# bluecher31/mlff-preconditioner

Hardware: AMD Instinct MI355X
Metric: CG iters/sec + GB/s on N×N fp64 kernel mat-vec; iters-to-1e-6 vs CPU ref (higher is better)
Workload: dtype f64

## Files before the change

### include/mlffpcg.h

```cpp
#ifndef MLFFPCG_H
#define MLFFPCG_H

#include <stdint.h>

#ifdef __cplusplus
extern "C" {
#endif

#define MLFF_OK 0
#define MLFF_ERR_ARG (-1)
#define MLFF_ERR_HIP (-2)
#define MLFF_ERR_NOT_PSD (-3)
#define MLFF_ERR_LINALG (-4)
#define MLFF_ERR_STATE (-5)
#define MLFF_ERR_COMM (-6)
#define MLFF_ERR_NOMEM (-7)

#define MLFF_PRECON_NONE 0
#define MLFF_PRECON_PIVCHOL 1
#define MLFF_PRECON_NYSTROM 2
#define MLFF_PRECON_NYSTROM_SB 3
#define MLFF_PRECON_LOWRANK 4
#define MLFF_PRECON_EIG 5

#define MLFF_STORAGE_DENSE 0
#define MLFF_STORAGE_SYMTILE 1
#define MLFF_STORAGE_AUTO 2
#define MLFF_STORAGE_MATFREE 3

#define MLFF_PCG_RUNNING 0
#define MLFF_PCG_CONVERGED 2
#define MLFF_PCG_MAXITER 3

typedef struct mlff_ctx mlff_ctx;

int mlff_version(void);
const char *mlff_build_hash(void);
int mlff_device_count(int *n_out);
int mlff_comm_unique_id(unsigned char id_out[128]);
int mlff_comm_selftest(int device, int64_t count, double *max_err_out);

int mlff_ctx_create(int device, int rank, int world, const unsigned char *comm_id,
                    int64_t n_global, mlff_ctx **ctx_out);
int mlff_ctx_destroy(mlff_ctx *ctx);
const char *mlff_last_error(mlff_ctx *ctx);
int mlff_shard_range(mlff_ctx *ctx, int64_t *row0_out, int64_t *nrows_out);
int mlff_comm_abort(mlff_ctx *ctx);
int mlff_matrix_ld(mlff_ctx *ctx, int64_t *ld_out);
int mlff_synchronize(mlff_ctx *ctx);
int mlff_stream(mlff_ctx *ctx, void **stream_out);

int mlff_set_matrix_host(mlff_ctx *ctx, const double *K_local, int64_t ld_host);
int mlff_get_matrix_rows(mlff_ctx *ctx, int64_t r0, int64_t nr, double *out, int64_t ld_out);
int mlff_gen_rbf(mlff_ctx *ctx, const double *X, int d, double length_scale, double jitter);
int mlff_assemble_sgdml(mlff_ctx *ctx, const double *R_desc, const double *R_d_desc,
                        int64_t M, int n_atoms, const int32_t *perms, int n_perms, double sig);
int mlff_sgdml_operator(mlff_ctx *ctx, const double *R_desc, const double *R_d_desc, int64_t M,
                        int n_atoms, const int32_t *perms, int n_perms, double sig);

int mlff_set_energy_constraints(mlff_ctx *ctx, int use_E_cstr);

int mlff_spectrum(mlff_ctx *ctx, int preconditioned, double *eig_out);

int mlff_test_gemm(mlff_ctx *ctx, int ta, int tb, int64_t M, int64_t N, int64_t K, double alpha,
                   const double *A, int64_t lda, const double *B, int64_t ldb, double beta,
                   double *C, int64_t ldc, int splits);
int mlff_dense_cho_solve(mlff_ctx *ctx, double sigma_K, double shift, const double *b,
                         double *x_out, double *seconds_out);
int mlff_test_potrf(mlff_ctx *ctx, const double *A, int64_t n, int variant, double *L_out,
                    double *seconds_out);
int mlff_test_gram(mlff_ctx *ctx, const double *W, int64_t k, int64_t ncols, int mode,
                   double *G_out);
int mlff_cho_factor_stable(mlff_ctx *ctx, const double *M, int64_t m, double *L_out,
                           double *lo_eig_out);
int mlff_sym_min_eig(mlff_ctx *ctx, const double *M, int64_t m, double *lo_eig_out,
                     double *d_out, double *e_out);
int mlff_sgdml_descriptors(const double *R, int64_t M, int n_atoms, double *R_desc_out,
                           double *R_d_desc_out);

int mlff_sgdml_energies(mlff_ctx *ctx, const double *alphas, double *E_out, int64_t *i0_out,
                        int64_t *ni_out);

int mlff_predict_set_model(mlff_ctx *ctx, const double *R_desc, const double *R_d_desc_alpha,
                           int64_t M, int n_atoms, const int32_t *perms, int n_perms, double sig,
                           double std, double c);
int mlff_predict(mlff_ctx *ctx, const double *R, int64_t Q, double *E_out, double *F_out);
int mlff_predict_info(mlff_ctx *ctx, int *form_out, int64_t *slab_out, double *flops_per_query_out,
                      double *bytes_per_query_out);

int mlff_set_operator(mlff_ctx *ctx, double sigma_K, double lam);
int mlff_matvec(mlff_ctx *ctx, const double *v_global, double *y_local);
int mlff_set_storage(mlff_ctx *ctx, int mode);
int mlff_storage_info(mlff_ctx *ctx, int *mode_out, double *bytes_per_matvec_out);
#define MLFF_MF_FORM_PAIR 0
#define MLFF_MF_FORM_REC 1
#define MLFF_MF_FORM_PTILE 2
int mlff_operator_form(mlff_ctx *ctx, int *form_out);
int mlff_get_diag(mlff_ctx *ctx, double *diag_local);

int mlff_precon_none(mlff_ctx *ctx);
int mlff_precon_pivchol(mlff_ctx *ctx, int64_t k, int build_woodbury, int64_t *index_columns_out,
                        double *seconds_out);
int mlff_pivchol_times(mlff_ctx *ctx, double *col_seconds_out, int64_t k,
                       double *woodbury_seconds_out);
int mlff_precon_nystrom(mlff_ctx *ctx, const int64_t *idx, int64_t k, int variant, double *seconds_out);
int mlff_precon_lowrank(mlff_ctx *ctx, const double *Lt_local, int64_t k);
int mlff_precon_eig(mlff_ctx *ctx, int64_t k, int mask_mode, int64_t dim_i, int build_woodbury,
                    double *evals_out, double *rowlev_out);
int mlff_precon_info(mlff_ctx *ctx, int *kind_out, int64_t *k_out);
int mlff_eig_info(mlff_ctx *ctx, int *converged_out, double *rel_resid_out);
int mlff_precon_apply(mlff_ctx *ctx, const double *r_local, double *z_local);
int mlff_precon_apply_traffic(mlff_ctx *ctx, int *one_pass_out, double *bytes_out);
int mlff_precon_get_panel(mlff_ctx *ctx, double *T_local, int64_t ld_out);

int mlff_lev_scores(mlff_ctx *ctx, const int64_t *idx, int64_t k, double lam, double *scores_out);

int mlff_pcg_start(mlff_ctx *ctx, const double *b_local, const double *x0_local, double tol,
                   int64_t maxiter, int *early_exit_out);
int mlff_pcg_run(mlff_ctx *ctx, int64_t n_iter, int64_t chunk, int *status_out);
int mlff_pcg_result(mlff_ctx *ctx, int64_t *iters_out, int *status_out, double *resid_out,
                    int *info_out);
int mlff_pcg_get_x(mlff_ctx *ctx, double *x_local);
int mlff_pcg_get_trace(mlff_ctx *ctx, double *trace_out, int64_t n);

int mlff_timing_enable(mlff_ctx *ctx, int on);
int mlff_timing_read(mlff_ctx *ctx, double *gemv_ms, int64_t *gemv_count, double *iter_ms,
                     int64_t *iter_count);
int mlff_timing_read_precon(mlff_ctx *ctx, double *ms, int64_t *count);
int mlff_timing_read_comm(mlff_ctx *ctx, double *ms, int64_t *count);
int mlff_timing_reset(mlff_ctx *ctx);
int mlff_device_memory(mlff_ctx *ctx, int64_t *free_out, int64_t *total_out);

#ifdef __cplusplus
}
#endif
#endif
```

### mlff-preconditioner_amd/csrc/api.hip

```cpp
#include "common.h"

#include <cstdlib>

#include <algorithm>
#include <chrono>
#include <cmath>
#include <condition_variable>
#include <cstring>
#include <limits>
#include <map>
#include <mutex>

using namespace mlff;

static thread_local std::string g_last_error;

namespace mlff {

int set_error(mlff_ctx *ctx, int code, const std::string &msg) {
  if (ctx != nullptr) ctx->err = msg;
  g_last_error = msg;
  return code;
}

// ... 1124 lines not shown
  if (hipDeviceSynchronize() != hipSuccess) return fail(set_error(nullptr, MLFF_ERR_HIP, "init sync failed"));
  *ctx_out = ctx;
  return MLFF_OK;
  MLFF_API_END(nullptr)
}

int mlff_ctx_destroy(mlff_ctx *ctx) {
  MLFF_API_BEGIN
  if (ctx == nullptr) return MLFF_OK;
  hipSetDevice(ctx->device);
  if (ctx->stream) hipStreamSynchronize(ctx->stream);
  for (void *p : {(void *)ctx->K, (void *)ctx->x, (void *)ctx->r, (void *)ctx->z, (void *)ctx->q,
                  (void *)ctx->b, (void *)ctx->p_full, (void *)ctx->xg, (void *)ctx->part,
                  (void *)ctx->st, (void *)ctx->trace, (void *)ctx->T, (void *)ctx->tpart_base,
                  (void *)ctx->perm, (void *)ctx->dwork, (void *)ctx->pivflag, (void *)ctx->prow, (void *)ctx->zpart, (void *)ctx->lr_zpart, (void *)ctx->lr_slots, (void *)ctx->lr_fault, (void *)ctx->gb})
    dev_free(p);
  for (const auto &c : ctx->scratch_chunks) dev_free(c.p);
  ctx->scratch_chunks.clear();
  sym_free(ctx->sym);
  mf_free(ctx->mf);
  pred_free(ctx->pred);
  rbf_free(ctx);
  if (ctx->h_st) hipHostFree(ctx->h_st);
  for (hipEvent_t e : ctx->timing.ev) hipEventDestroy(e);
  if (ctx->comm) ncclCommDestroy(ctx->comm);
  ctx->local.reset();
  if (ctx->stream) hipStreamDestroy(ctx->stream);
  delete ctx;
  return MLFF_OK;
  MLFF_API_END(ctx)
}

int mlff_comm_abort(mlff_ctx *ctx) {
  MLFF_API_BEGIN
  if (ctx == nullptr) return set_error(nullptr, MLFF_ERR_ARG, "null ctx");
  ctx->aborted = true;
  if (ctx->local) ctx->local->abort();
  if (ctx->comm != nullptr) {
    (void)hipSetDevice(ctx->device);
    ncclCommAbort(ctx->comm);
    ctx->comm = nullptr;
  }
  return MLFF_OK;
  MLFF_API_END(ctx)
}

int mlff_shard_range(mlff_ctx *ctx, int64_t *row0_out, int64_t *nrows_out) {
  MLFF_API_BEGIN
  MLFF_ENTER(ctx);
  if (row0_out) *row0_out = ctx->row0;
  if (nrows_out) *nrows_out = ctx->nrows;
  return MLFF_OK;
  MLFF_API_END(ctx)
}

int mlff_matrix_ld(mlff_ctx *ctx, int64_t *ld_out) {
  MLFF_API_BEGIN
  if (ctx == nullptr || ld_out == nullptr) return set_error(ctx, MLFF_ERR_ARG, "null pointer");
  *ld_out = ctx->ld;
  return MLFF_OK;
  MLFF_API_END(ctx)
}

int mlff_synchronize(mlff_ctx *ctx) {
  MLFF_API_BEGIN
  MLFF_ENTER(ctx);
  MLFF_HIP(ctx, hipStreamSynchronize(ctx->stream));
  return MLFF_OK;
  MLFF_API_END(ctx)
}

int mlff_stream(mlff_ctx *ctx, void **stream_out) {
  MLFF_API_BEGIN
  if (ctx == nullptr || stream_out == nullptr) return set_error(ctx, MLFF_ERR_ARG, "null pointer");
  *stream_out = (void *)ctx->stream;
  return MLFF_OK;
  MLFF_API_END(ctx)
}

int mlff_set_matrix_host(mlff_ctx *ctx, const double *K_local, int64_t ld_host) {
  MLFF_API_BEGIN
  MLFF_ENTER(ctx);
  if (K_local == nullptr && ctx->nrows > 0) return set_error(ctx, MLFF_ERR_ARG, "null K");
  if (ld_host < ctx->N) return set_error(ctx, MLFF_ERR_ARG, "ld_host < N");
  MLFF_TRY(ensure_matrix(ctx));
  MLFF_HIP(ctx, hipMemsetAsync(ctx->K, 0, sizeof(double) * ctx->blk * ctx->ld, ctx->stream));
  for (int r = 0; r < ctx->world && ctx->nrows > 0; ++r) {
    const int64_t g0 = (int64_t)r * ctx->rows_per;
    if (g0 >= ctx->N) break;
    const int64_t cnt = std::min<int64_t>(ctx->rows_per, ctx->N - g0);
    MLFF_HIP(ctx, hipMemcpy2DAsync(ctx->K + (int64_t)r * ctx->blk, sizeof(double) * ctx->ld,
                                   K_local + g0, sizeof(double) * ld_host, sizeof(double) * cnt,
                                   ctx->nrows, hipMemcpyHostToDevice, ctx->stream));
  }
  MLFF_HIP(ctx, hipStreamSynchronize(ctx->stream));
  ctx->has_matrix = true;
  ctx->K_symmetric = false;
  ctx->sym.ready = false;
  mf_free(ctx->mf);
  rbf_free(ctx);
  return MLFF_OK;
  MLFF_API_END(ctx)
}

int mlff_get_matrix_rows(mlff_ctx *ctx, int64_t r0, int64_t nr, double *out, int64_t ld_out) {
  MLFF_API_BEGIN
  MLFF_ENTER(ctx);
  if (out == nullptr) return set_error(ctx, MLFF_ERR_ARG, "null pointer");
  if (!ctx->has_matrix && !ctx->rbf.ready) return set_error(ctx, MLFF_ERR_STATE, "no kernel matrix set");
  if (r0 < 0 || nr < 0 || r0 + nr > ctx->nrows || ld_out < ctx->N)
    return set_error(ctx, MLFF_ERR_ARG, "row range / ld_out");
  ScratchScope scope(ctx);
  const int64_t chunk = ctx->has_matrix ? nr : std::max<int64_t>(1, std::min<int64_t>(nr, (int64_t)(256e6 / (8.0 * ctx->ld))));
  double *tmp = nullptr;
  if (!ctx->has_matrix) MLFF_TRY(scratch_alloc(ctx, &tmp, (size_t)chunk * ctx->ld));
  for (int64_t c0 = 0; c0 < nr; c0 += chunk) {
    const int64_t cn = std::min<int64_t>(chunk, nr - c0);
    const double *src = ctx->K + (r0 + c0) * ctx->ld;
    if (!ctx->has_matrix) {
      launch_gen_rbf(tmp, ctx->ld, cn, ctx->row0 + r0 + c0, ctx->rows_per, ctx->blk, ctx->N,
                     ctx->rbf.Xs, ctx->rbf.d, ctx->rbf.jitter, ctx->stream);
      MLFF_HIP(ctx, hipGetLastError());
      src = tmp;
    }
    for (int r = 0; r < ctx->world; ++r) {
      const int64_t g0 = (int64_t)r * ctx->rows_per;
      if (g0 >= ctx->N) break;
      const int64_t cnt = std::min<int64_t>(ctx->rows_per, ctx->N - g0);
      MLFF_HIP(ctx, hipMemcpy2DAsync(out + c0 * ld_out + g0, sizeof(double) * ld_out,
                                     src + (int64_t)r * ctx->blk, sizeof(double) * ctx->ld,
                                     sizeof(double) * cnt, cn, hipMemcpyDeviceToHost, ctx->stream));
    }
    MLFF_HIP(ctx, hipStreamSynchronize(ctx->stream));
  }
  return MLFF_OK;
  MLFF_API_END(ctx)
}

int mlff_gen_rbf(mlff_ctx *ctx, const double *X, int d, double length_scale, double jitter) {
  MLFF_API_BEGIN
  MLFF_ENTER(ctx);
  if (X == nullptr || d < 1 || d > 8 || !(length_scale > 0.0))
    return set_error(ctx, MLFF_ERR_ARG, "gen_rbf: need X, 1 <= d <= 8, length_scale > 0");
  std::vector<double> Xs((size_t)ctx->N * d);
  for (size_t i = 0; i < Xs.size(); ++i) Xs[i] = X[i] / length_scale;
  sym_free(ctx->sym);
  mf_free(ctx->mf);
  rbf_free(ctx);
  if (ctx->K != nullptr) {
    (void)hipFree(ctx->K);
    ctx->K = nullptr;
  }
  ctx->has_matrix = false;
  MLFF_HIP(ctx, hipMalloc(&ctx->rbf.Xs, sizeof(double) * Xs.size()));
  MLFF_HIP(ctx, hipMemcpy(ctx->rbf.Xs, Xs.data(), sizeof(double) * Xs.size(), hipMemcpyHostToDevice));
  ctx->rbf.d = d;
  ctx->rbf.jitter = jitter;
  ctx->rbf.ready = true;
  ctx->K_symmetric = true;
  return MLFF_OK;
  MLFF_API_END(ctx)
}

int mlff_assemble_sgdml(mlff_ctx *ctx, const double *R_desc, const double *R_d_desc, int64_t M,
                        int n_atoms, const int32_t *perms, int n_perms, double sig) {
  MLFF_API_BEGIN
  MLFF_ENTER(ctx);
  if (R_desc == nullptr || R_d_desc == nullptr || perms == nullptr || !(sig > 0.0))
    return set_error(ctx, MLFF_ERR_ARG, "assemble_sgdml: null input or sig <= 0");
  rbf_free(ctx);
  MLFF_TRY(ensure_matrix(ctx));
  MLFF_TRY(assemble_sgdml(ctx, R_desc, R_d_desc, M, n_atoms, perms, n_perms, sig));
  MLFF_TRY(mf_setup(ctx, R_desc, R_d_desc, M, n_atoms, perms, n_perms, sig));
  ctx->has_matrix = true;
  ctx->K_symmetric = true;
  ctx->sym.ready = false;
  return MLFF_OK;
  MLFF_API_END(ctx)
}

int mlff_sgdml_operator(mlff_ctx *ctx, const double *R_desc, const double *R_d_desc, int64_t M,
                        int n_atoms, const int32_t *perms, int n_perms, double sig) {
  MLFF_API_BEGIN
  MLFF_ENTER(ctx);
  if (R_desc == nullptr || R_d_desc == nullptr || perms == nullptr || !(sig > 0.0))
    return set_error(ctx, MLFF_ERR_ARG, "sgdml_operator: null input or sig <= 0");
  rbf_free(ctx);
  MLFF_TRY(mf_setup(ctx, R_desc, R_d_desc, M, n_atoms, perms, n_perms, sig));
  ctx->use_mf = false;
  ctx->has_matrix = false;
  ctx->sym.ready = false;
  return MLFF_OK;
  MLFF_API_END(ctx)
}

int mlff_test_gemm(mlff_ctx *ctx, int ta, int tb, int64_t M, int64_t N, int64_t K, double alpha,
                   const double *A, int64_t lda, const double *B, int64_t ldb, double beta,
                   double *C, int64_t ldc, int splits) {
  MLFF_API_BEGIN
  MLFF_ENTER(ctx);
  if (A == nullptr || B == nullptr || C == nullptr || M < 0 || N < 0 || K < 0 || splits < 1 ||
      lda < (ta ? M : K) || ldb < (tb ? K : N) || ldc < N)
    return set_error(ctx, MLFF_ERR_ARG, "test_gemm: bad arguments");
  return test_gemm(ctx, ta, tb, M, N, K, alpha, A, lda, B, ldb, beta, C, ldc, splits);
  MLFF_API_END(ctx)
}

int mlff_test_potrf(mlff_ctx *ctx, const double *A, int64_t n, int variant, double *L_out,
                    double *seconds_out) {
  MLFF_API_BEGIN
  MLFF_ENTER(ctx);
  if (A == nullptr || L_out == nullptr || n < 1 || variant < 0 || variant > 1)
    return set_error(ctx, MLFF_ERR_ARG, "test_potrf: bad arguments");
  return test_potrf(ctx, A, n, variant, L_out, seconds_out);
  MLFF_API_END(ctx)
}

int mlff_dense_cho_solve(mlff_ctx *ctx, double sigma_K, double shift, const double *b,
                         double *x_out, double *seconds_out) {
  MLFF_API_BEGIN
  MLFF_ENTER(ctx);
  if (b == nullptr || x_out == nullptr) return set_error(ctx, MLFF_ERR_ARG, "null pointer");
  if (ctx->world > 1)
    return set_error(ctx, MLFF_ERR_ARG, "dense_cho_solve: the closed-form solve runs on one rank");
  if (!ctx->has_matrix)
    return set_error(ctx, MLFF_ERR_STATE,
                     "dense_cho_solve: no dense kernel matrix (mlff_set_matrix_host / "
                     "mlff_assemble_sgdml); a matrix-free operator alone cannot be factored");
  return dense_cho_solve(ctx, sigma_K, shift, b, x_out, seconds_out);
  MLFF_API_END(ctx)
}

int mlff_test_gram(mlff_ctx *ctx, const double *W, int64_t k, int64_t ncols, int mode,
                   double *G_out) {
  MLFF_API_BEGIN
  MLFF_ENTER(ctx);
  if (W == nullptr || G_out == nullptr || k < 1 || ncols < 1 || mode < 0 || mode > 2)
    return set_error(ctx, MLFF_ERR_ARG, "test_gram: bad arguments");
  ScratchScope scope(ctx);
  double *dW = nullptr, *dG = nullptr;
  MLFF_TRY(scratch_alloc(ctx, &dW, (size_t)(k * ncols)));
  MLFF_TRY(scratch_alloc(ctx, &dG, (size_t)(k * k)));
  MLFF_HIP(ctx, hipMemcpyAsync(dW, W, sizeof(double) * k * ncols, hipMemcpyHostToDevice, ctx->stream));
  if (mode == 0)
    MLFF_TRY(syrk_wide(ctx, dW, k, ncols, ncols, dG));
  else
    MLFF_TRY(gram_wide_dd(ctx, dW, k, ncols, ncols, dG, mode == 2));
  MLFF_HIP(ctx, hipMemcpyAsync(G_out, dG, sizeof(double) * k * k, hipMemcpyDeviceToHost, ctx->stream));
  MLFF_HIP(ctx, hipStreamSynchronize(ctx->stream));
  return MLFF_OK;
  MLFF_API_END(ctx)
}

int mlff_sym_min_eig(mlff_ctx *ctx, const double *M, int64_t m, double *lo_eig_out,
                     double *d_out, double *e_out) {
  MLFF_API_BEGIN
  MLFF_ENTER(ctx);
  if (M == nullptr || m < 1 || lo_eig_out == nullptr)
    return set_error(ctx, MLFF_ERR_ARG, "sym_min_eig: bad arguments");
  ScratchScope scope(ctx);
  double *dM = nullptr;
  MLFF_TRY(scratch_alloc(ctx, &dM, (size_t)(m * m)));
  MLFF_HIP(ctx, hipMemcpyAsync(dM, M, sizeof(double) * m * m, hipMemcpyHostToDevice, ctx->stream));
  return sym_min_eig(ctx, dM, m, lo_eig_out, d_out, e_out);
  MLFF_API_END(ctx)
}

int mlff_cho_factor_stable(mlff_ctx *ctx, const double *M, int64_t m, double *L_out,
                           double *lo_eig_out) {
  MLFF_API_BEGIN
  MLFF_ENTER(ctx);
  if (M == nullptr || m < 1 || L_out == nullptr)
    return set_error(ctx, MLFF_ERR_ARG, "cho_factor_stable: bad arguments");
  ScratchScope scope(ctx);
  double *dM = nullptr;
  MLFF_TRY(scratch_alloc(ctx, &dM, (size_t)(m * m)));
  MLFF_HIP(ctx, hipMemcpyAsync(dM, M, sizeof(double) * m * m, hipMemcpyHostToDevice, ctx->stream));
  MLFF_TRY(cho_factor_stable(ctx, dM, m, lo_eig_out));
  MLFF_HIP(ctx, hipMemcpyAsync(L_out, dM, sizeof(double) * m * m, hipMemcpyDeviceToHost, ctx->stream));
  MLFF_HIP(ctx, hipStreamSynchronize(ctx->stream));
  return MLFF_OK;
  MLFF_API_END(ctx)
}

int mlff_spectrum(mlff_ctx *ctx, int preconditioned, double *eig_out) {
  MLFF_API_BEGIN
  MLFF_ENTER(ctx);
  if (eig_out == nullptr) return set_error(ctx, MLFF_ERR_ARG, "null pointer");
  MLFF_TRY(require_operator(ctx));
  return spectrum(ctx, preconditioned != 0, eig_out);
  MLFF_API_END(ctx)
}

int mlff_set_energy_constraints(mlff_ctx *ctx, int use_E_cstr) {
  MLFF_API_BEGIN
  MLFF_ENTER(ctx);
  if (use_E_cstr && ctx->world > 1)
    return set_error(ctx, MLFF_ERR_ARG, "use_E_cstr: energy constraints run on one rank");
  ctx->use_E_cstr = use_E_cstr != 0;
  return MLFF_OK;
  MLFF_API_END(ctx)
}

int mlff_sgdml_descriptors(const double *R, int64_t M, int n_atoms, double *R_desc_out,
                           double *R_d_desc_out) {
  MLFF_API_BEGIN
  if (R == nullptr || R_desc_out == nullptr || R_d_desc_out == nullptr || M < 1 || n_atoms < 2)
    return set_error(nullptr, MLFF_ERR_ARG, "sgdml_descriptors: bad arguments");
  const int rc = sgdml_descriptors(R, M, n_atoms, R_desc_out, R_d_desc_out);
  if (rc != MLFF_OK) return set_error(nullptr, rc, "sgdml_descriptors: HIP failure");
  return MLFF_OK;
  MLFF_API_END(nullptr)
}

int mlff_sgdml_energies(mlff_ctx *ctx, const double *alphas, double *E_out, int64_t *i0_out,
                        int64_t *ni_out) {
  MLFF_API_BEGIN
  MLFF_ENTER(ctx);
  if (alphas == nullptr || E_out == nullptr) return set_error(ctx, MLFF_ERR_ARG, "null pointer");
  if (!ctx->mf.ready) return set_error(ctx, MLFF_ERR_STATE, "no sGDML operator set");
  const MfData &mf = ctx->mf;
  const int64_t MP = mf.M * mf.n_perms;
  std::vector<double> pairs((size_t)std::max<int64_t>(mf.ni, 1) * MP);
  MLFF_TRY(mf_energies(ctx, alphas, pairs.data()));
  for (int64_t i = 0; i < mf.ni; ++i) {
    double e = 0.0;
    for (int64_t jp = 0; jp < MP; ++jp) e += pairs[(size_t)i * MP + jp];
    E_out[i] = e;
  }
  if (i0_out) *i0_out = mf.i0;
  if (ni_out) *ni_out = mf.ni;
  return MLFF_OK;
  MLFF_API_END(ctx)
}

int mlff_predict_set_model(mlff_ctx *ctx, const double *R_desc, const double *R_d_desc_alpha,
                           int64_t M, int n_atoms, const int32_t *perms, int n_perms, double sig,
                           double std, double c) {
  MLFF_API_BEGIN
  MLFF_ENTER(ctx);
  if (ctx->world > 1) return set_error(ctx, MLFF_ERR_ARG, "predict: runs on a one-rank context");
  if (R_desc == nullptr || R_d_desc_alpha == nullptr || perms == nullptr)
    return set_error(ctx, MLFF_ERR_ARG, "predict: null pointer");
  if (n_atoms < 2 || M < 1 || n_perms < 1 || n_perms > 1024)
    return set_error(ctx, MLFF_ERR_ARG, "predict: bad sizes");
  if (3 * (int64_t)n_atoms * M != ctx->N)
    return set_error(ctx, MLFF_ERR_ARG, "predict: N != 3 * n_atoms * M");
  if (!(sig > 0.0)) return set_error(ctx, MLFF_ERR_ARG, "predict: sig must be > 0");
  return pred_set_model(ctx, R_desc, R_d_desc_alpha, M, n_atoms, perms, n_perms, sig, std, c);
  MLFF_API_END(ctx)
}

int mlff_predict(mlff_ctx *ctx, const double *R, int64_t Q, double *E_out, double *F_out) {
  MLFF_API_BEGIN
  MLFF_ENTER(ctx);
  if (ctx->world > 1) return set_error(ctx, MLFF_ERR_ARG, "predict: runs on a one-rank context");
  if (!ctx->pred.ready) return set_error(ctx, MLFF_ERR_STATE, "predict: no model set (mlff_predict_set_model)");
  if (Q < 0) return set_error(ctx, MLFF_ERR_ARG, "predict: Q < 0");
  if (Q == 0) return MLFF_OK;
  if (R == nullptr || E_out == nullptr || F_out == nullptr)
    return set_error(ctx, MLFF_ERR_ARG, "predict: null pointer");
  return pred_run(ctx, R, Q, E_out, F_out);
  MLFF_API_END(ctx)
}

int mlff_predict_info(mlff_ctx *ctx, int *form_out, int64_t *slab_out, double *flops_per_query_out,
                      double *bytes_per_query_out) {
  MLFF_API_BEGIN
  MLFF_ENTER(ctx);
  if (!ctx->pred.ready) return set_error(ctx, MLFF_ERR_STATE, "predict: no model set (mlff_predict_set_model)");
  double fl = 0.0, by = 0.0;
  pred_work(ctx->pred, &fl, &by);
  if (form_out) *form_out = ctx->pred.form;
  if (slab_out) *slab_out = ctx->pred.slab;
  if (flops_per_query_out) *flops_per_query_out = fl;
  if (bytes_per_query_out) *bytes_per_query_out = by;
  return MLFF_OK;
  MLFF_API_END(ctx)
}

int mlff_set_operator(mlff_ctx *ctx, double sigma_K, double lam) {
  MLFF_API_BEGIN
  MLFF_ENTER(ctx);
  if (!(lam > 0.0)) return set_error(ctx, MLFF_ERR_ARG, "lam must be > 0");
  if (sigma_K != 1.0 && sigma_K != -1.0) return set_error(ctx, MLFF_ERR_ARG, "sigma_K must be +-1");
  ctx->sigma_K = sigma_K;
  ctx->lam = lam;
  ctx->has_operator = true;
  return MLFF_OK;
  MLFF_API_END(ctx)
}

int mlff_set_storage(mlff_ctx *ctx, int mode) {
  MLFF_API_BEGIN
  MLFF_ENTER(ctx);
  if (mode != MLFF_STORAGE_DENSE && mode != MLFF_STORAGE_SYMTILE && mode != MLFF_STORAGE_AUTO &&
      mode != MLFF_STORAGE_MATFREE)
    return set_error(ctx, MLFF_ERR_ARG, "bad storage mode");
  if (mode != ctx->storage) {
    ctx->storage = mode;
    ctx->use_sym = false;
    ctx->use_mf = false;
    if (mode == MLFF_STORAGE_DENSE || mode == MLFF_STORAGE_MATFREE) sym_free(ctx->sym);
  }
  return MLFF_OK;
  MLFF_API_END(ctx)
}

int mlff_operator_form(mlff_ctx *ctx, int *form_out) {
  MLFF_API_BEGIN
  MLFF_ENTER(ctx);
  if (form_out == nullptr) return set_error(ctx, MLFF_ERR_ARG, "null form_out");
  *form_out = ctx->mf.ready ? mf_form(ctx) : -1;
  return MLFF_OK;
  MLFF_API_END(ctx)
}

int mlff_storage_info(mlff_ctx *ctx, int *mode_out, double *bytes_per_matvec_out) {
  MLFF_API_BEGIN
  MLFF_ENTER(ctx);
  MLFF_TRY(require_operator(ctx));
  MLFF_TRY(resolve_storage(ctx));
  if (mode_out)
    *mode_out = ctx->use_mf ? MLFF_STORAGE_MATFREE
                            : (ctx->use_sym ? MLFF_STORAGE_SYMTILE : MLFF_STORAGE_DENSE);
  if (bytes_per_matvec_out) *bytes_per_matvec_out = operator_bytes(ctx);
  return MLFF_OK;
  MLFF_API_END(ctx)
}

int mlff_matvec(mlff_ctx *ctx, const double *v_global, double *y_local) {
  MLFF_API_BEGIN
  MLFF_ENTER(ctx);
  MLFF_TRY(require_operator(ctx));
  if (v_global == nullptr || (y_local == nullptr && ctx->nrows > 0)) return set_error(ctx, MLFF_ERR_ARG, "null vector");
  MLFF_TRY(resolve_storage(ctx));
  MLFF_TRY(scatter_global(ctx, v_global, ctx->xg));
  MLFF_TRY(launch_operator(ctx, ctx->xg, ctx->q, ctx->xg + (int64_t)ctx->rank * ctx->blk, nullptr));
  MLFF_HIP(ctx, hipGetLastError());
  if (ctx->nrows > 0)
    MLFF_HIP(ctx, hipMemcpyAsync(y_local, ctx->q, sizeof(double) * ctx->nrows, hipMemcpyDeviceToHost, ctx->stream));
  MLFF_HIP(ctx, hipStreamSynchronize(ctx->stream));
  return MLFF_OK;
  MLFF_API_END(ctx)
}

int mlff_get_diag(mlff_ctx *ctx, double *diag_local) {
  MLFF_API_BEGIN
  MLFF_ENTER(ctx);
  if (!ctx->has_matrix && !ctx->mf.ready && !ctx->rbf.ready)
    return set_error(ctx, MLFF_ERR_STATE, "no kernel matrix set");
  MLFF_TRY(operator_diag(ctx, ctx->dwork));
  if (ctx->nrows > 0)
    MLFF_HIP(ctx, hipMemcpyAsync(diag_local, ctx->dwork, sizeof(double) * ctx->nrows, hipMemcpyDeviceToHost, ctx->stream));
  MLFF_HIP(ctx, hipStreamSynchronize(ctx->stream));
  return MLFF_OK;
  MLFF_API_END(ctx)
}

int mlff_precon_none(mlff_ctx *ctx) {
  MLFF_API_BEGIN
  MLFF_ENTER(ctx);
  ctx->precon_kind = MLFF_PRECON_NONE;
  ctx->k = 0;
  return MLFF_OK;
  MLFF_API_END(ctx)
}

int mlff_precon_pivchol(mlff_ctx *ctx, int64_t k, int build_woodbury, int64_t *index_columns_out,
                        double *seconds_out) {
  MLFF_API_BEGIN
  MLFF_ENTER(ctx);
  MLFF_TRY(require_operator(ctx));
  if (k < 1 || k > ctx->N || k > 65536)
    return set_error(ctx, MLFF_ERR_ARG, "pivoted Cholesky rank k must satisfy 1 <= k <= min(N, 65536)");
  const auto t0 = std::chrono::steady_clock::now();
  ctx->precon_kind = MLFF_PRECON_NONE;
  MLFF_TRY(alloc_panel(ctx, k));
  if (ctx->prow) hipFree(ctx->prow);
  ctx->prow = nullptr;
  MLFF_HIP(ctx, hipMalloc(&ctx->prow, sizeof(double) * (k + 1)));
  MLFF_TRY(pivoted_cholesky(ctx, k, index_columns_out));
  ctx->k = k;
  ctx->piv_woodbury_s = 0.0;
  if (build_woodbury) {
    const auto tw = std::chrono::steady_clock::now();
    MLFF_TRY(woodbury_inplace(ctx, ctx->T, k));
    ctx->piv_woodbury_s = std::chrono::duration<double>(std::chrono::steady_clock::now() - tw).count();
    ctx->precon_kind = MLFF_PRECON_PIVCHOL;
    ctx->sigma_p = 1.0;
  }
  MLFF_HIP(ctx, hipStreamSynchronize(ctx->stream));
  if (seconds_out)
    *seconds_out = std::chrono::duration<double>(std::chrono::steady_clock::now() - t0).count();
  return MLFF_OK;
  MLFF_API_END(ctx)
}

int mlff_pivchol_times(mlff_ctx *ctx, double *col_seconds_out, int64_t k,
                       double *woodbury_seconds_out) {
  MLFF_API_BEGIN
  MLFF_ENTER(ctx);
  if (k < 0 || (k > 0 && col_seconds_out == nullptr)) return set_error(ctx, MLFF_ERR_ARG, "bad output");
  const int64_t n = std::min<int64_t>(k, (int64_t)ctx->piv_col_s.size());
  for (int64_t c = 0; c < n; ++c) col_seconds_out[c] = ctx->piv_col_s[c];
  for (int64_t c = n; c < k; ++c) col_seconds_out[c] = 0.0;
  if (woodbury_seconds_out) *woodbury_seconds_out = ctx->piv_woodbury_s;
  return MLFF_OK;
  MLFF_API_END(ctx)
}

int mlff_precon_nystrom(mlff_ctx *ctx, const int64_t *idx, int64_t k, int variant,
                        double *seconds_out) {
  MLFF_API_BEGIN
  MLFF_ENTER(ctx);
  MLFF_TRY(require_operator(ctx));
  if (variant != 0 && variant != 1) return set_error(ctx, MLFF_ERR_ARG, "variant must be 0 or 1");
  MLFF_TRY(check_idx(ctx, idx, k));
  const auto t0 = std::chrono::steady_clock::now();
  ctx->precon_kind = MLFF_PRECON_NONE;
  MLFF_TRY(alloc_panel(ctx, k));
  MLFF_TRY(nystrom_panel(ctx, idx, k, variant, ctx->lam, ctx->T));
  ctx->precon_kind = variant == 0 ? MLFF_PRECON_NYSTROM : MLFF_PRECON_NYSTROM_SB;
  ctx->k = k;
  ctx->sigma_p = -1.0;
  if (seconds_out)
    *seconds_out = std::chrono::duration<double>(std::chrono::steady_clock::now() - t0).count();
  return MLFF_OK;
  MLFF_API_END(ctx)
}

int mlff_precon_lowrank(mlff_ctx *ctx, const double *Lt_local, int64_t k) {
  MLFF_API_BEGIN
  MLFF_ENTER(ctx);
  MLFF_TRY(require_operator(ctx));
  if (k < 1 || k > ctx->N || (Lt_local == nullptr && ctx->nrows > 0))
    return set_error(ctx, MLFF_ERR_ARG, "lowrank: bad factor");
  ctx->precon_kind = MLFF_PRECON_NONE;
  MLFF_TRY(alloc_panel(ctx, k));
  if (ctx->nrows > 0)
    MLFF_HIP(ctx, hipMemcpy2DAsync(ctx->T, sizeof(double) * ctx->blk, Lt_local,
                                   sizeof(double) * ctx->nrows, sizeof(double) * ctx->nrows, k,
                                   hipMemcpyHostToDevice, ctx->stream));
  MLFF_TRY(woodbury_inplace(ctx, ctx->T, k));
  ctx->precon_kind = MLFF_PRECON_LOWRANK;
  ctx->k = k;
  ctx->sigma_p = 1.0;
  return MLFF_OK;
  MLFF_API_END(ctx)
}

int mlff_precon_eig(mlff_ctx *ctx, int64_t k, int mask_mode, int64_t dim_i, int build_woodbury,
                    double *evals_out, double *rowlev_out) {
  MLFF_API_BEGIN
  MLFF_ENTER(ctx);
  if (mask_mode < 0 || mask_mode > 2 || (mask_mode == 2 && (dim_i < 3 || dim_i % 3 != 0)))
    return set_error(ctx, MLFF_ERR_ARG, "eig: bad mask_mode / dim_i");
  if (mask_mode == 2) {
    MLFF_TRY(require_matrix(ctx));
  } else {
    MLFF_TRY(require_operator(ctx));
  }
  if (k < 1 || k > ctx->N) return set_error(ctx, MLFF_ERR_ARG, "eig: need 1 <= k <= N");
  ctx->precon_kind = MLFF_PRECON_NONE;
  MLFF_TRY(alloc_panel(ctx, k));
  MLFF_TRY(eig_lowrank(ctx, k, mask_mode, dim_i, ctx->T, evals_out, rowlev_out));
  if (build_woodbury) {
    MLFF_TRY(woodbury_inplace(ctx, ctx->T, k));
    ctx->precon_kind = MLFF_PRECON_EIG;
    ctx->k = k;
    ctx->sigma_p = 1.0;
  }
  return MLFF_OK;
  MLFF_API_END(ctx)
}

int mlff_eig_info(mlff_ctx *ctx, int *converged_out, double *rel_resid_out) {
  MLFF_API_BEGIN
  MLFF_ENTER(ctx);
  if (converged_out) *converged_out = ctx->eig_converged ? 1 : 0;
  if (rel_resid_out) *rel_resid_out = ctx->eig_rel_resid;
  return MLFF_OK;
  MLFF_API_END(ctx)
}

int mlff_precon_info(mlff_ctx *ctx, int *kind_out, int64_t *k_out) {
  MLFF_API_BEGIN
  MLFF_ENTER(ctx);
  if (kind_out) *kind_out = ctx->precon_kind;
  if (k_out) *k_out = ctx->k;
  return MLFF_OK;
  MLFF_API_END(ctx)
}

int mlff_precon_apply_traffic(mlff_ctx *ctx, int *one_pass_out, double *bytes_out) {
  MLFF_API_BEGIN
  MLFF_ENTER(ctx);
  const double N = (double)ctx->blk, n = (double)ctx->nrows, k = (double)ctx->k;
  const bool one = ctx->precon_kind != MLFF_PRECON_NONE && (ctx->lr_rows || ctx->lr_cluster);
  if (one_pass_out) *one_pass_out = one ? (ctx->lr_cluster ? 2 : 1) : 0;
  if (bytes_out) {
    if (ctx->precon_kind == MLFF_PRECON_NONE)
      *bytes_out = 0.0;
    else if (one)
      *bytes_out = 8.0 * k * N +
                   16.0 * (double)(ctx->lr_cluster ? ctx->lr_q : lr_rows_groups(ctx->k)) * N +
                   24.0 * n;
    else
      *bytes_out = 16.0 * k * N + 24.0 * n;
  }
  return MLFF_OK;
  MLFF_API_END(ctx)
}

int mlff_precon_apply(mlff_ctx *ctx, const double *r_local, double *z_local) {
  MLFF_API_BEGIN
  MLFF_ENTER(ctx);
  MLFF_TRY(require_operator(ctx));
  hipStream_t s = ctx->stream;
  ScratchScope scope(ctx);
  double *rd = nullptr, *zd = nullptr;
  MLFF_TRY(scratch_alloc(ctx, &rd, ctx->blk));
  MLFF_TRY(scratch_alloc(ctx, &zd, ctx->blk));
  MLFF_HIP(ctx, hipMemsetAsync(rd, 0, sizeof(double) * ctx->blk, s));
  if (ctx->nrows > 0)
    MLFF_HIP(ctx, hipMemcpyAsync(rd, r_local, sizeof(double) * ctx->nrows, hipMemcpyHostToDevice, s));
  if (ctx->precon_kind == MLFF_PRECON_NONE) {
    MLFF_HIP(ctx, hipMemcpyAsync(zd, rd, sizeof(double) * ctx->blk, hipMemcpyDeviceToDevice, s));
  } else {
    ctx->spec_t = false;
    if (ctx->exact_sums) {
      launch_dd_lowrank(ctx->T, ctx->blk, ctx->k, rd, zd, ctx->nrows, ctx->sigma_p, 1.0 / ctx->lam,
                        ctx->tpart, nullptr, s);
      MLFF_HIP(ctx, hipGetLastError());
      if (ctx->nrows > 0)
        MLFF_HIP(ctx, hipMemcpyAsync(z_local, zd, sizeof(double) * ctx->nrows, hipMemcpyDeviceToHost, s));
      MLFF_HIP(ctx, hipStreamSynchronize(s));
      return MLFF_OK;
    }
    if (ctx->lr_rows || ctx->lr_cluster) {
      if (ctx->lr_rows) {
        launch_lr_apply_rows(ctx->T, ctx->blk, ctx->k, rd, zd, ctx->nrows, ctx->sigma_p,
                             1.0 / ctx->lam, nullptr, nullptr, s, ctx->lr_zpart);
      } else {
        MLFF_HIP(ctx, hipMemsetAsync(ctx->lr_fault, 0, sizeof(int), s));
        launch_lr_apply_cluster(ctx->T, ctx->blk, ctx->k, ctx->lr_q, rd, zd, ctx->nrows,
                                ctx->sigma_p, 1.0 / ctx->lam, nullptr, nullptr, s, ctx->lr_zpart,
                                ctx->lr_slots, next_lr_epoch(ctx), ctx->lr_fault);
      }
      MLFF_HIP(ctx, hipGetLastError());
      if (ctx->lr_cluster) {
        int fault = 0;
        MLFF_HIP(ctx, hipMemcpyAsync(&fault, ctx->lr_fault, sizeof(int), hipMemcpyDeviceToHost, s));
        MLFF_HIP(ctx, hipStreamSynchronize(s));
        if (fault != 0) {
          ctx->lr_cluster = false;
          ctx->lr_fallbacks += 1;
          launch_gemv_split(ctx->T, ctx->blk, ctx->k, ctx->blk, ctx->tsplit, rd, ctx->tpart, nullptr, s);
          launch_precon_z(ctx->T, ctx->blk, ctx->k, ctx->tsplit, ctx->tpart, rd, zd, ctx->nrows,
                          ctx->sigma_p, 1.0 / ctx->lam, nullptr, nullptr, s, ctx->zpart, ctx->zsplit);
          MLFF_HIP(ctx, hipGetLastError());
        }
      }
      if (ctx->nrows > 0)
        MLFF_HIP(ctx, hipMemcpyAsync(z_local, zd, sizeof(double) * ctx->nrows, hipMemcpyDeviceToHost, s));
      MLFF_HIP(ctx, hipStreamSynchronize(s));
      return MLFF_OK;
    }
    launch_gemv_split(ctx->T, ctx->blk, ctx->k, ctx->blk, ctx->tsplit, rd, ctx->tpart, nullptr, s);
    MLFF_TRY(allreduce(ctx, ctx->tpart, (size_t)(ctx->k * ctx->tsplit)));
    launch_precon_z(ctx->T, ctx->blk, ctx->k, ctx->tsplit, ctx->tpart, rd, zd, ctx->nrows,
                    ctx->sigma_p, 1.0 / ctx->lam, nullptr, nullptr, s, ctx->zpart, ctx->zsplit);
  }
  MLFF_HIP(ctx, hipGetLastError());
  if (ctx->nrows > 0)
    MLFF_HIP(ctx, hipMemcpyAsync(z_local, zd, sizeof(double) * ctx->nrows, hipMemcpyDeviceToHost, s));
  MLFF_HIP(ctx, hipStreamSynchronize(s));
  return MLFF_OK;
  MLFF_API_END(ctx)
}

int mlff_precon_get_panel(mlff_ctx *ctx, double *T_local, int64_t ld_out) {
  MLFF_API_BEGIN
  MLFF_ENTER(ctx);
  if (ctx->T == nullptr || ctx->k < 1) return set_error(ctx, MLFF_ERR_STATE, "no low-rank panel");
  if (T_local == nullptr || ld_out < ctx->nrows) return set_error(ctx, MLFF_ERR_ARG, "bad output");
  if (ctx->nrows > 0)
    MLFF_HIP(ctx, hipMemcpy2DAsync(T_local, sizeof(double) * ld_out, ctx->T, sizeof(double) * ctx->blk,
                                   sizeof(double) * ctx->nrows, ctx->k, hipMemcpyDeviceToHost, ctx->stream));
  MLFF_HIP(ctx, hipStreamSynchronize(ctx->stream));
  return MLFF_OK;
  MLFF_API_END(ctx)
}

int mlff_lev_scores(mlff_ctx *ctx, const int64_t *idx, int64_t k, double lam, double *scores_out) {
  MLFF_API_BEGIN
  MLFF_ENTER(ctx);
  if (!ctx->has_matrix && !ctx->mf.ready && !ctx->rbf.ready)
    return set_error(ctx, MLFF_ERR_STATE, "no kernel matrix set");
  if (!(lam > 0.0) || scores_out == nullptr) return set_error(ctx, MLFF_ERR_ARG, "lev_scores: bad args");
  MLFF_TRY(check_idx(ctx, idx, k));
  hipStream_t s = ctx->stream;
  double *W = nullptr;
  MLFF_HIP(ctx, hipMalloc(&W, sizeof(double) * round_up(k, 8) * ctx->blk));
  MLFF_HIP(ctx, hipMemsetAsync(W, 0, sizeof(double) * round_up(k, 8) * ctx->blk, s));
  int rc = nystrom_panel(ctx, idx, k, 0, lam, W);
  if (rc != MLFF_OK) {
    hipFree(W);
    return rc;
  }
  MLFF_HIP(ctx, hipMemsetAsync(ctx->xg, 0, sizeof(double) * ctx->ld, s));
  launch_colsumsq(W, k, ctx->nrows, ctx->blk, ctx->xg + (int64_t)ctx->rank * ctx->blk, s);
  MLFF_TRY(allgather_blocks(ctx, ctx->xg));
  for (int r = 0; r < ctx->world; ++r) {
    const int64_t g0 = (int64_t)r * ctx->rows_per;
    if (g0 >= ctx->N) break;
    const int64_t cnt = std::min<int64_t>(ctx->rows_per, ctx->N - g0);
    MLFF_HIP(ctx, hipMemcpyAsync(scores_out + g0, ctx->xg + (int64_t)r * ctx->blk,
                                 sizeof(double) * cnt, hipMemcpyDeviceToHost, s));
  }
  MLFF_HIP(ctx, hipStreamSynchronize(s));
  hipFree(W);
  return MLFF_OK;
  MLFF_API_END(ctx)
}

int mlff_pcg_start(mlff_ctx *ctx, const double *b_local, const double *x0_local, double tol,
                   int64_t maxiter, int *early_exit_out) {
  MLFF_API_BEGIN
// ... 249 lines not shown
```

### mlff-preconditioner_amd/csrc/common.h

```cpp
#pragma once

#include <hip/hip_runtime.h>
#include <rccl/rccl.h>

#include <cstdint>
#include <memory>
#include <string>
#include <cstdlib>
#include <vector>

#include "../../include/mlffpcg.h"

namespace mlff {

constexpr int kWave = 64;
constexpr int kBlock = 256;
constexpr int kPad = 64;
constexpr int kMaxPart = 1024;
constexpr int kVecGrid = 512;
constexpr int kSymTile = 512;

__host__ __device__ inline int64_t round_up(int64_t a, int64_t b) { return (a + b - 1) / b * b; }

enum : int { ST_RUNNING = 0, ST_RECHECK = 1, ST_CONVERGED = 2, ST_MAXITER = 3, ST_FAULT = 4 };

struct DevState {
  double rho, rho1, alpha, pq, rr, resid, atol, pad0;
  long long iters;
  long long maxiter;
  int status;
  int linalg_err;
  int pivot_err;
  int pad1;
  long long m_pi;
  double sqrt_piv;
  double best_val;
  long long best_pos;
  double rho_new;
};

constexpr int kSymGenMaxD = 3;
constexpr double kSymStreamRate = 4990.0;
constexpr double kSymGenRate = 4990.0;
struct SymGen {
  const double *Xs = nullptr;
  int d = 0;
  double jitter = 0.0;
  int64_t N = 0, rows_per = 0, blk = 0;
  int n_s = 0;
  int qmode = 0;
  int roles = 0;
  int pool_first = 0;
};
enum SymRoles : int { kSymRolesCu = 0, kSymRolesIndex = 1, kSymRolesStream = 2, kSymRolesGen = 3 };
constexpr int kSymCuWords = 4096;

struct SymPack {
  bool ready = false;
  double *tiles = nullptr;
  int2 *list = nullptr;
  int64_t ntiles = 0;
  int64_t Np = 0;
  int64_t nb = 0;
  int64_t tiles_per_rank = 0;
  double *P = nullptr;
  int64_t nwhole = 0;
  int lsub = 2;
  int64_t pq_planes = 0;
  double *Pq = nullptr;
  unsigned char *split = nullptr;
  int *own = nullptr;
  int *plist = nullptr;
  int64_t pstride = 0;
  int pmax = 0;
  bool pq_ordered = false;
  int64_t t_split = 0;
  int64_t dyn = 0;
  unsigned long long *ticket = nullptr;
  bool gen = false;
  SymGen gsrc;
  double *yg = nullptr;
  double *yr = nullptr;
  int64_t ystride = 0;
};

constexpr int kSymOwnSplit = 1 << 24;
constexpr int kSymPlistSlotBits = 16;
constexpr int kSymPlistMaxSlots = (1 << kSymPlistSlotBits) - 1;
__host__ __device__ inline int sym_own_entry(int slot, bool split) {
  return slot | (split ? kSymOwnSplit : 0);
}
__host__ __device__ inline int sym_own_slot(int e) { return e & (kSymOwnSplit - 1); }
__host__ __device__ inline bool sym_own_split(int e) { return (e & kSymOwnSplit) != 0; }
__host__ __device__ inline int sym_plist_entry(int slot, int plane) {
  return slot | (plane << kSymPlistSlotBits);
}
__host__ __device__ inline int sym_plist_slot(int e) { return e & kSymPlistMaxSlots; }
__host__ __device__ inline int sym_plist_plane(int e) { return e >> kSymPlistSlotBits; }

struct MfData {
  bool ready = false;
  int64_t M = 0, D = 0;
  int n = 0, n_perms = 0;
  double sig = 0.0;
  int64_t i0 = 0, ni = 0;
  double *Rd = nullptr, *Rdd = nullptr;
  double *Rt = nullptr, *Zt = nullptr;
  int32_t *Pt = nullptr, *ps = nullptr, *pt = nullptr;
  bool ident = false;
  double *m5 = nullptr, *w = nullptr;
  double *c = nullptr, *F = nullptr;
  double *part = nullptr;
  double *ypart = nullptr;
  double *xc = nullptr;
  int nz = 1;
  int64_t dslice = 0;
  std::vector<int32_t> perms, piinv;
  double *uvk = nullptr;
  int32_t *pi_d = nullptr, *piinv_d = nullptr;
  bool rec = false;
  int rec_rg = 8;
  bool rec_wc16 = true;
  int rblk = 0;
  int64_t ldw = 0;
  double *wt = nullptr, *sv = nullptr, *rpart = nullptr;
  bool ptile = false;
  int pt_S = 1;
  double *ptpart = nullptr;
  bool E = false;
  int64_t nF = 0;
  double *kee = nullptr;
  double *eterm = nullptr;
};

struct PredData {
  bool ready = false;
  int64_t M = 0, D = 0, MP = 0;
  int n = 0, n_perms = 0;
  double sig = 0.0, std = 1.0, c = 0.0;
  int form = 0;
  int S = 1;
  int G = 1;
  int64_t slab = 0;
  int64_t PS = 0, ecol = 0;
  double *Rt = nullptr, *Zt = nullptr;
  double *Rq = nullptr;
  double *Rdq = nullptr, *Rddq = nullptr;
  double *part = nullptr;
  double *Fd = nullptr;
  double *EF = nullptr;
  double *h_in = nullptr, *h_out = nullptr;
};

struct RbfData {
  bool ready = false;
  double *Xs = nullptr;
  int d = 0;
  double jitter = 0.0;
};

__device__ __forceinline__ double rbf_sqdist_step(double s, double df, bool first) {
  return first ? __dmul_rn(df, df) : fma(df, df, s);
}
__device__ __forceinline__ double rbf_of_sqdist(double s) { return exp(-0.5 * s); }
__device__ __forceinline__ double rbf_value(const double (&xi)[8], const double *__restrict__ Xs,
                                            int64_t g, int d) {
  double s = 0.0;
#pragma unroll
  for (int t = 0; t < 8; ++t)
    if (t < d) s = rbf_sqdist_step(s, __dsub_rn(xi[t], Xs[g * d + t]), t == 0);
  return rbf_of_sqdist(s);
}

struct StopFold {
  const double *rr_part = nullptr;
  DevState *st = nullptr;
  double *trace = nullptr;
  long long it = 0;
};

struct XrFold {
  double *x = nullptr;
  double *r = nullptr;
  const double *p = nullptr;
  const double *q = nullptr;
  const double *pq_part = nullptr;
  double *rr_part = nullptr;
  DevState *st = nullptr;
};

inline unsigned timing_event_flags() {
  static const unsigned f = std::getenv("MLFF_EVENT_FENCE") ? hipEventDefault
                                                            : hipEventDisableSystemFence;
  return f;
}

struct Timing {
  bool on = false;
  int every = 1;
  bool sample = true;
  std::vector<hipEvent_t> ev;
  size_t used = 0;
  double gemv_ms = 0.0;
  int64_t gemv_count = 0;
  double pre_ms = 0.0;
  int64_t pre_count = 0;
  double iter_ms = 0.0;
  int64_t iter_count = 0;
  double comm_ms = 0.0;
  int64_t comm_count = 0;
};


__device__ __forceinline__ double fused_p(double pold, double z, double beta, bool first) {
  return first ? z : fma(beta, pold, z);
}

__device__ __forceinline__ double wave_sum(double v) {
#pragma unroll
  for (int o = 32; o > 0; o >>= 1) v += __shfl_down(v, o, 64);
  return v;
}

template <int CTRL>
__device__ __forceinline__ double dpp_f64(double v) {
  const int lo = __builtin_amdgcn_update_dpp(0, __double2loint(v), CTRL, 0xF, 0xF, false);
  const int hi = __builtin_amdgcn_update_dpp(0, __double2hiint(v), CTRL, 0xF, 0xF, false);
  return __hiloint2double(hi, lo);
}
template <int L>
__device__ __forceinline__ double group_sum(double v) {
  static_assert(L == 1 || L == 2 || L == 4 || L == 8, "DPP butterfly for L <= 8");
  if (L >= 2) v += dpp_f64<0xB1>(v);
  if (L >= 4) v += dpp_f64<0x4E>(v);
  if (L >= 8) v += dpp_f64<0x141>(v);
  return v;
}

__device__ __forceinline__ double block_sum256(double v, double *sh) {
  v = wave_sum(v);
  const int lane = threadIdx.x & 63, w = threadIdx.x >> 6;
  __syncthreads();
  if (lane == 0) sh[w] = v;
  __syncthreads();
  double t = 0.0;
  if (threadIdx.x == 0) t = (sh[0] + sh[1]) + (sh[2] + sh[3]);
  return t;
}

__device__ __forceinline__ void block_sum256_pair(double &a, double &b, double *sh) {
  a = wave_sum(a);
  b = wave_sum(b);
  const int lane = threadIdx.x & 63, w = threadIdx.x >> 6;
  __syncthreads();
  if (lane == 0) {
    sh[w] = a;
    sh[4 + w] = b;
  }
  __syncthreads();
  a = (sh[0] + sh[1]) + (sh[2] + sh[3]);
  b = (sh[4] + sh[5]) + (sh[6] + sh[7]);
}

__device__ __forceinline__ double reduce_parts_bcast(const double *__restrict__ part, int np,
                                                     double *sh) {
  double v = 0.0;
  for (int i = threadIdx.x; i < np; i += 256) v += part[i];
  v = block_sum256(v, sh);
  __syncthreads();
  if (threadIdx.x == 0) sh[4] = v;
  __syncthreads();
  return sh[4];
}

__device__ __forceinline__ bool stop_decide(const StopFold &f, double rr) {
  const double resid = sqrt(rr);
  DevState *st = f.st;
  int dec = ST_RUNNING;
  if (resid <= st->atol)
    dec = f.it > 1 ? ST_RECHECK : ST_CONVERGED;
  else if (f.it >= st->maxiter)
    dec = ST_MAXITER;
  if (blockIdx.x == 0 && blockIdx.y == 0 && threadIdx.x == 0) {
    st->rr = rr;
    st->resid = resid;
    st->iters = f.it;
    f.trace[f.it] = resid;
    if (dec != ST_RUNNING)
      st->status = dec;
    else
      st->rho1 = st->rho;
  }
  return dec == ST_RUNNING;
}

__device__ __forceinline__ double reduce_parts_bcast_wide(const double *__restrict__ part, int np,
                                                          double *sh) {
  double v = 0.0;
  if (threadIdx.x < 256)
    for (int i = threadIdx.x; i < np; i += 256) v += part[i];
  v = wave_sum(v);
  const int lane = threadIdx.x & 63, w = threadIdx.x >> 6;
  __syncthreads();
  if (lane == 0 && w < 4) sh[w] = v;
  __syncthreads();
  const double t = (sh[0] + sh[1]) + (sh[2] + sh[3]);
  __syncthreads();
  return t;
}

__device__ __forceinline__ double parts_thread_sum(const double *__restrict__ part, int np) {
  double v = 0.0;
  for (int i = threadIdx.x; i < np; i += 256) v += part[i];
  return v;
}
__device__ __forceinline__ double parts_bcast(double v, double *sh) {
  v = block_sum256(v, sh);
  __syncthreads();
  if (threadIdx.x == 0) sh[4] = v;
  __syncthreads();
  return sh[4];
}

}

namespace mlff {
struct LocalGroup;
}

struct mlff_ctx {
  int device = 0, rank = 0, world = 1;
  int64_t N = 0;
  int64_t rows_per = 0;
  int64_t row0 = 0, nrows = 0;
  int64_t blk = 0;
  int64_t ld = 0;
  hipStream_t stream = nullptr;
  ncclComm_t comm = nullptr;
  std::shared_ptr<mlff::LocalGroup> local;
  bool solo = false;

  double *K = nullptr;
  bool has_matrix = false;
  double sigma_K = 1.0, lam = 0.0;
  bool has_operator = false;
  bool K_symmetric = false;
  bool use_E_cstr = false;
  int storage = MLFF_STORAGE_AUTO;
  bool use_sym = false;
  bool use_mf = false;
  mlff::SymPack sym;
  mlff::MfData mf;
  mlff::RbfData rbf;
  mlff::PredData pred;

  double *x = nullptr, *r = nullptr, *z = nullptr, *q = nullptr, *b = nullptr;
  double *p_full = nullptr, *xg = nullptr;
  double *gb = nullptr;
  int64_t gstride = 0;
  double *part = nullptr;
  mlff::DevState *st = nullptr;
  mlff::DevState *h_st = nullptr;
  double *trace = nullptr;
  int64_t trace_cap = 0;
  bool pcg_active = false;
  int64_t pcg_done = 0;
  double tol = 0.0, bnorm = 0.0;

  int precon_kind = MLFF_PRECON_NONE;
  int64_t k = 0;
  double *T = nullptr;
  double sigma_p = 1.0;
  int tsplit = 1;
  int zsplit = 1;
  double *zpart = nullptr;
  bool lr_rows = false;
  bool fuse_p = true, fuse_xr = true;
  bool cho_fast = true;
  bool fuse_xr_ranks = false;
  bool pq_publish = false;
  bool piv_persist_off = false;
  int wb_refine = 0;
  int wb_gram_dd = 1;
  bool nys_refine = false;
  bool exact_sums = false;
  bool lr_cluster = false;
  int lr_q = 0;
  double *lr_zpart = nullptr;
  unsigned long long *lr_slots = nullptr;
  unsigned lr_epoch = 0;
  int *lr_fault = nullptr;
  int lr_fallbacks = 0;
  double last_lo_eig = 0.0;
  bool cho_flipped = false;
  bool eig_converged = true;
  double eig_rel_resid = 0.0;
  double *tpart = nullptr;
  double *tpart_base = nullptr;
  bool spec_t = false;

  int64_t *perm = nullptr;
  double *dwork = nullptr;
  int *pivflag = nullptr;
  double *prow = nullptr;
  std::vector<double> piv_col_s;
  double piv_woodbury_s = 0.0;

  mlff::Timing timing;
  std::string err;
  bool aborted = false;

  struct ScratchChunk {
    char *p;
    size_t size;
  };
  std::vector<ScratchChunk> scratch_chunks;
  size_t scratch_cur = 0, scratch_off = 0;
  int scratch_depth = 0;
};

namespace mlff {

int set_error(mlff_ctx *ctx, int code, const std::string &msg);
int hip_check(mlff_ctx *ctx, hipError_t e, const char *what);
int nccl_check(mlff_ctx *ctx, ncclResult_t e, const char *what);

#define MLFF_HIP(ctx, call)                                   \
  do {                                                        \
    hipError_t e__ = (call);                                  \
    if (e__ != hipSuccess) return mlff::hip_check(ctx, e__, #call); \
  } while (0)
#define MLFF_NCCL(ctx, call)                                  \
  do {                                                        \
    ncclResult_t e__ = (call);                                \
    if (e__ != ncclSuccess) return mlff::nccl_check(ctx, e__, #call); \
  } while (0)
#define MLFF_ENTER(ctx)                                                        \
  do {                                                                         \
    if ((ctx) == nullptr) return mlff::set_error(nullptr, MLFF_ERR_ARG, "null ctx"); \
    if ((ctx)->aborted)                                                        \
      return mlff::set_error((ctx), MLFF_ERR_COMM, "communicator aborted (mlff_comm_abort)"); \
    (void)hipSetDevice((ctx)->device);                                         \
  } while (0)
#define MLFF_TRY(x)             \
  do {                          \
    int rc__ = (x);             \
    if (rc__ != MLFF_OK) return rc__; \
  } while (0)

int api_exception(mlff_ctx *ctx, int code, const char *what);
#define MLFF_API_BEGIN try {
#define MLFF_API_END(ctx)                                                             \
  }                                                                                   \
  catch (const std::bad_alloc &) {                                                    \
    return mlff::api_exception((ctx), MLFF_ERR_NOMEM, "host allocation failed");      \
  }                                                                                   \
  catch (const std::exception &e__) {                                                 \
    return mlff::api_exception((ctx), MLFF_ERR_HIP, e__.what());                      \
  }                                                                                   \
  catch (...) {                                                                       \
    return mlff::api_exception((ctx), MLFF_ERR_HIP, "unknown C++ exception");         \
  }

struct ScratchScope {
  mlff_ctx *ctx;
  size_t chunk, off;
  explicit ScratchScope(mlff_ctx *c);
  ~ScratchScope();
  ScratchScope(const ScratchScope &) = delete;
  ScratchScope &operator=(const ScratchScope &) = delete;
};
int scratch_get(mlff_ctx *ctx, size_t bytes, void **out);
template <typename T>
int scratch_alloc(mlff_ctx *ctx, T **out, size_t count) {
  return scratch_get(ctx, sizeof(T) * (count > 0 ? count : 1), reinterpret_cast<void **>(out));
}

int comm_allreduce(mlff_ctx *ctx, double *buf, size_t n);
int comm_allgather(mlff_ctx *ctx, const double *send, double *recv, size_t count);

void launch_gemv_rows(const double *M, int64_t ld, int64_t rows, const double *v, double *y,
                      double sigma, double lam, const double *vloc, const int *status,
                      hipStream_t s);
void launch_gemv_split(const double *T, int64_t ldt, int64_t k, int64_t ncols, int splits,
                       const double *r, double *tpart, const int *status, hipStream_t s,
                       StopFold fold = StopFold{});
int choose_tsplit(int64_t k, int64_t ncols);
int choose_zsplit(int64_t k, int64_t ncols);
void launch_precon_z(const double *T, int64_t ldt, int64_t k, int splits, const double *tpart,
                     const double *r, double *z, int64_t n, double sigma_p, double lam_inv,
                     double *rho_part, const int *status, hipStream_t s, double *zpart,
                     int zsplit, StopFold fold = StopFold{});
bool lr_rows_fits(int64_t ldt);
int lr_rows_groups(int64_t k);
void launch_lr_apply_rows(const double *T, int64_t ldt, int64_t k, const double *r, double *z,
                          int64_t n, double sigma_p, double lam_inv, double *rho_part,
                          const int *status, hipStream_t s, double *zpart,
                          StopFold fold = StopFold{}, XrFold xf = XrFold{});
bool lr_cluster_fits(int64_t ldt);
int lr_cluster_members(int64_t ldt);
int lr_cluster_count(int64_t ldt, int device);
void launch_lr_apply_cluster(const double *T, int64_t ldt, int64_t k, int Q, const double *r,
                             double *z, int64_t n, double sigma_p, double lam_inv,
                             double *rho_part, const int *status, hipStream_t s, double *zpart,
                             unsigned long long *slots, unsigned epoch, int *fault,
                             StopFold fold = StopFold{});
void launch_colgemv_part(const double *W, int64_t ldw, int64_t k, const double *tsrc,
                         int tsplits, int64_t tstride, int ksplit, double *part,
                         const int *status, hipStream_t s, StopFold fold = StopFold{},
                         int64_t cached_rows = 0, const long long *tcol = nullptr,
                         const int *spec_hit = nullptr, int64_t spec_m0 = 0);
int gemm_splitk(mlff_ctx *ctx, bool ta, bool tb, int64_t M, int64_t N, int64_t K, const double *A,
                int64_t lda, const double *B, int64_t ldb, double *C, int64_t ldc);
int choose_ksplit(int64_t k, int64_t ncols);
int64_t panel_cached_rows(int64_t k, int64_t ldt);
void launch_dot_part(const double *a, const double *b, int64_t n, double *part,
                     const int *status, hipStream_t s, StopFold fold = StopFold{});
void launch_update_p(const double *z, double *p, int64_t n, const double *rho_part,
                     DevState *st, long long it, const int *status, hipStream_t s);
void launch_copy_dot(const double *r, int64_t n, double *dst, double *part, const int *status,
                     hipStream_t s, StopFold fold = StopFold{});
void launch_update_p_gathered(const double *gb, int64_t gstride, int64_t blk, int world,
                              double *p_full, DevState *st, long long it, const int *status,
                              hipStream_t s);
void launch_update_xr_shares(double *x, double *r, const double *p, const double *y,
                             const double *shares, int world, int64_t n, double sigma, double lam,
                             double *rr_part, DevState *st, const int *status, hipStream_t s);
bool xr_fold_fits(int64_t ncols, int splits, int64_t n);
void launch_dd_gemv_rows(const double *M, int64_t ld, int64_t rows, int64_t ncols, const double *v,
                         double *y, double sigma, double lam, const double *vloc, const int *status,
                         hipStream_t s);
void launch_dd_lowrank(const double *T, int64_t ldt, int64_t k, const double *r, double *z, int64_t n,
                       double sigma_p, double lam_inv, double *t, const int *status, hipStream_t s);
int gram_wide_dd(mlff_ctx *ctx, const double *W, int64_t k, int64_t ncols, int64_t ldw, double *G,
                 bool exact_products);
void launch_gemv_xr(const double *T, int64_t ldt, int64_t k, int64_t ncols, int splits,
                    const double *r, double *r_out, double *x, const double *p, const double *y,
                    const double *shares, int world, int64_t n, double sigma, double lam,
                    double *rr_part, DevState *st, double *tpart, const int *status,
                    hipStream_t s);
void launch_update_xr(double *x, double *r, const double *p, const double *q, int64_t n,
                      const double *pq_part, double *rr_part, DevState *st, const int *status,
                      hipStream_t s);
void launch_stoptest(const double *rr_part, DevState *st, double *trace, long long it,
                     hipStream_t s);
void launch_residual(const double *b, const double *q, double *r, int64_t n, double *rr_part,
                     hipStream_t s);
void launch_recheck_finish(const double *rr_part, DevState *st, double *trace, hipStream_t s);
void launch_reduce_to(const double *part, int np, double *out, hipStream_t s);
void launch_scale_copy(const double *a, double *y, int64_t n, double alpha, hipStream_t s);

void launch_gemm(bool ta, bool tb, int64_t M, int64_t Nc, int64_t Kd, double alpha,
                 const double *A, int64_t lda, const double *B, int64_t ldb, double beta,
                 double *C, int64_t ldc, hipStream_t s);
int syrk_wide(mlff_ctx *ctx, const double *W, int64_t k, int64_t ncols, int64_t ldw, double *G);
int gram_wide(mlff_ctx *ctx, const double *A, const double *B, int64_t k, int64_t ncols,
              int64_t ldw, double *G);
int potrf_lower(mlff_ctx *ctx, double *A, int64_t k, bool *ok_out = nullptr);
int sym_min_eig(mlff_ctx *ctx, const double *M, int64_t m, double *lo_eig, double *d_host,
                double *e_host);
int trsm_lower_wide(mlff_ctx *ctx, const double *L, int64_t k, double *W, int64_t ncols,
                    int64_t ldw);
void launch_add_diag(double *A, int64_t k, double v, hipStream_t s);
void launch_zero_upper(double *A, int64_t k, hipStream_t s);
void launch_potrf_diag_wave(double *A, int64_t lda, int64_t j0, int jb, int *err, hipStream_t s);
void launch_trsm_panel(double *A, int64_t lda, int64_t k, int64_t j0, int jb, hipStream_t s);
void launch_gemm_tri(bool ta, bool tb, int64_t M, int64_t Nc, int64_t Kd, double alpha,
                     const double *A, int64_t lda, const double *B, int64_t ldb, double beta,
                     double *C, int64_t ldc, hipStream_t s);

int potrf_lower_blocked(mlff_ctx *ctx, double *A, int64_t n, bool *ok_out = nullptr);
int trsv_lower_fwd(mlff_ctx *ctx, const double *L, int64_t n, double *x);
int trsv_lower_bwd(mlff_ctx *ctx, const double *L, int64_t n, double *x);
int dense_cho_solve(mlff_ctx *ctx, double sigma_K, double shift, const double *b_host,
                    double *x_host, double *seconds_out);
int test_potrf(mlff_ctx *ctx, const double *A_host, int64_t n, int variant, double *L_host,
               double *seconds_out);
void launch_colsumsq(const double *W, int64_t k, int64_t ncols, int64_t ldw, double *out,
                     hipStream_t s);

void launch_gen_rbf(double *K, int64_t ld, int64_t nrows, int64_t row0, int64_t rows_per,
                    int64_t blk, int64_t N, const double *Xs, int d, double jitter,
                    hipStream_t s);
void launch_diag_of(const double *K, int64_t ld, int64_t nrows, int64_t row0, int64_t rows_per,
                    int64_t blk, double sigma, double *out, hipStream_t s);
void launch_gather_cols(const double *K, int64_t ld, int64_t nrows, const int64_t *idx,
                        int64_t k, int64_t rows_per, int64_t blk, double sigma, double *W,
                        int64_t ldw, hipStream_t s);
void launch_gather_mm(const double *W, int64_t ldw, const int64_t *idx, int64_t k,
                      int64_t row0, int64_t nrows, double *Smm, hipStream_t s);
void launch_rbf_cols(const RbfData &rbf, int64_t N, int64_t row0, int64_t nrows,
                     const int64_t *cols, int64_t ncols, const DevState *st, double sigma,
                     double *out, int64_t ldo, hipStream_t s);
void launch_fill(double *y, int64_t n, double v, hipStream_t s);
int assemble_sgdml(mlff_ctx *ctx, const double *R_desc, const double *R_d_desc, int64_t M,
                   int n_atoms, const int32_t *perms, int n_perms, double sig);
int sgdml_descriptors(const double *R, int64_t M, int n_atoms, double *R_desc,
                      double *R_d_desc);
void launch_sgdml_kee(const double *Rd, int64_t M, int64_t D, int64_t i0, int64_t ni,
                      const int32_t *Pt, int n_perms, double sig, double *kee, hipStream_t s);
void launch_sgdml_records(const double *Rd, const double *Rdd, int64_t M, int n, int64_t D,
                          int64_t i0, int64_t ni, const int32_t *Pt, const int32_t *piinv,
                          int n_perms, double sig, double *uvk, hipStream_t s);
void launch_sgdml_columns(const double *Rdd, int64_t M, int n, int64_t D, int64_t i0,
                          const int32_t *pi, const int32_t *piinv, int n_perms,
                          const double *uvk, int64_t row0, int64_t nrows, const int64_t *cols,
                          int64_t ncols, const DevState *st, double sigma, double *out,
                          int64_t ldo, hipStream_t s);

int sym_build(mlff_ctx *ctx, bool check_symmetry, bool *symmetric_out);
void sym_free(SymPack &sp);
struct PGather {
  const double *gb = nullptr;
  int64_t gstride = 0, blk = 0;
  int world = 1;
  DevState *st = nullptr;
  long long it = 0;
};
void launch_symv(const SymPack &sp, const double *v_full, double *P, const int *status,
                 hipStream_t s, PGather pg = PGather{});
void launch_sym_reduce(const SymPack &sp, int64_t n_out, double *y, bool epilogue, double sigma,
                       double lam, const double *vloc, const int *status, hipStream_t s);
void launch_sym_reduce_pq(const SymPack &sp, int64_t n_out, double *y, double sigma, double lam,
                          const double *p, double *pq_part, const int *status, hipStream_t s,
                          PGather pg = PGather{});
void launch_sym_reduce_ranks(const SymPack &sp, int rank, int world, int64_t blk,
                             const double *p_full, double *pq_part, double *pp_part,
                             double sigma, double lam, const int *status, hipStream_t s,
                             PGather pg = PGather{}, bool separate_publish = false);
void launch_axpby_loc(const double *src, double *y, int64_t n, double sigma, double lam,
                      const double *vloc, const int *status, hipStream_t s);
int comm_reduce_scatter(mlff_ctx *ctx, const double *send, double *recv, size_t count);

int mf_setup(mlff_ctx *ctx, const double *R_desc, const double *R_d_desc, int64_t M, int n_atoms,
             const int32_t *perms, int n_perms, double sig);
struct PFuse {
  const double *z;
  const double *rho_part;
  DevState *st;
  long long it;
  StopFold sf;
};
bool mf_can_fuse_p(const mlff_ctx *ctx);
void launch_mf_operator(const mlff_ctx *ctx, const double *x_full, double *y_loc,
                        const double *x_loc, const int *status, double sigma, double lam,
                        double *pq_part = nullptr, const PFuse *pf = nullptr);
int mf_diag(mlff_ctx *ctx, double *out);
void launch_mf_zt(const MfData &mf, const double *xc, const int *status, hipStream_t s,
                  const PFuse *pf = nullptr);
bool pt_supported(int64_t D);
int pt_chunks(int64_t D, int64_t ni, int64_t MP);
int64_t pt_padded_d(int64_t D);
void launch_pt_operator(const MfData &mf, const double *Rt, const double *xc, int64_t row0,
                        int64_t nrows, const double *x_loc, double *y_loc, const int *status,
                        double sigma, double lam, double *pq_part, hipStream_t s,
                        const PFuse *pf = nullptr);
int mf_form(const mlff_ctx *ctx);
bool mf_columns(const mlff_ctx *ctx, const int64_t *cols, int64_t ncols, double sigma,
                double *out, int64_t ldo);
int mf_energies(mlff_ctx *ctx, const double *alphas, double *E_pairs_host);
int operator_diag(mlff_ctx *ctx, double *out);
int sgdml_diag(mlff_ctx *ctx, const double *dRd, const double *dRdd, int64_t M, int n,
               const int32_t *dP, const int32_t *perms_host, const int32_t *piinv_host,
               int n_perms, double sig, double *diag_out);
double mf_bytes(const mlff_ctx *ctx);
double mf_seconds(const mlff_ctx *ctx);
void mf_free(MfData &mf);
int desc_perm_tables(mlff_ctx *ctx, const int32_t *perms, int n, int n_perms,
                     std::vector<int32_t> &Pt, std::vector<int32_t> &piinv);

int pred_set_model(mlff_ctx *ctx, const double *R_desc, const double *R_d_desc_alpha, int64_t M,
                   int n_atoms, const int32_t *perms, int n_perms, double sig, double std, double c);
int pred_run(mlff_ctx *ctx, const double *R, int64_t Q, double *E_out, double *F_out);
bool pred_tile_supported(int64_t D);
void pred_work(const PredData &pd, double *flops_per_query, double *bytes_per_query);
void pred_free(PredData &pd);

int operator_prepare(mlff_ctx *ctx);
int operator_apply_local(mlff_ctx *ctx, const double *x_loc, double *y_loc);

int eig_lowrank(mlff_ctx *ctx, int64_t k, int mask_mode, int64_t dim_i, double *Lt_out,
                double *evals_out, double *rowlev_out);
int spectrum(mlff_ctx *ctx, bool preconditioned, double *eig_out);
int test_gemm(mlff_ctx *ctx, int ta, int tb, int64_t M, int64_t Nc, int64_t Kd, double alpha,
              const double *A, int64_t lda, const double *B, int64_t ldb, double beta, double *C,
              int64_t ldc, int splits);

int pivoted_cholesky(mlff_ctx *ctx, int64_t k, int64_t *index_columns_out);

}
```

### mlff-preconditioner_amd/csrc/kernels_sym.hip

```cpp
#include "common.h"

#include <algorithm>
#include <cstdlib>
#include <cstring>

namespace mlff {

typedef double d2 __attribute__((ext_vector_type(2)));

namespace {

constexpr int B = kSymTile;
constexpr int kRB = 8;
constexpr int kBatches = B / kRB;
constexpr int kTileRed = 6 * B;
constexpr int kTileLds = kTileRed + 4 * kRB * 64;

__device__ __forceinline__ void decode_unit(long long u, int nwhole, int lsub, int &tile, int &h,
                                            int &gb0, int &gb1) {
  if (u < nwhole) {
    tile = (int)u;
    h = 0;
    gb0 = 0;
    gb1 = kBatches;
  } else {
    const long long q = u - nwhole;
    tile = nwhole + (int)(q >> lsub);
    h = (int)(q & ((1 << lsub) - 1));
    gb0 = h * (kBatches >> lsub);
    gb1 = gb0 + (kBatches >> lsub);
  }
}

__device__ __forceinline__ double gathered_rho(const PGather &pg, double *sh) {
  double v = 0.0;
  const int np = pg.world * kVecGrid;
  int f = threadIdx.x;
  for (; f + 7 * 256 < np; f += 8 * 256) {
    double t[8];
#pragma unroll
    for (int u = 0; u < 8; ++u) {
      const int g = f + u * 256;
      t[u] = pg.gb[(int64_t)(g / kVecGrid) * pg.gstride + pg.blk + (g % kVecGrid)];
    }
#pragma unroll
    for (int u = 0; u < 8; ++u) v += t[u];
  }
  for (; f < np; f += 256) v += pg.gb[(int64_t)(f / kVecGrid) * pg.gstride + pg.blk + (f % kVecGrid)];
  v = block_sum256(v, sh);
  __syncthreads();
  if (threadIdx.x == 0) sh[4] = v;
  __syncthreads();
  const double rho = sh[4];
  __syncthreads();
  return rho;
}

__device__ __forceinline__ double pg_z(const PGather &pg, int64_t i) {
  const int64_t rk = i / pg.blk;
  return rk < pg.world ? pg.gb[rk * pg.gstride + i % pg.blk] : 0.0;
}
__device__ __forceinline__ double pg_val(const PGather &pg, const double *v, int64_t i, double beta) {
  return pg.it > 1 ? fma(beta, v[i], pg_z(pg, i)) : pg_z(pg, i);
}
__device__ __forceinline__ d2 pg_val2(const PGather &pg, const double *v, int64_t i, double beta) {
  if (pg.gb == nullptr) return *reinterpret_cast<const d2 *>(v + i);
  const int64_t rk = i / pg.blk;
  const d2 z = rk < pg.world ? *reinterpret_cast<const d2 *>(pg.gb + rk * pg.gstride + i % pg.blk)
                             : d2{0.0, 0.0};
  if (pg.it <= 1) return z;
  const d2 po = *reinterpret_cast<const d2 *>(v + i);
  return d2{fma(beta, po.x, z.x), fma(beta, po.y, z.y)};
}

__device__ __forceinline__ double fused_p_beta(const PGather &pg, double rho, double *publish) {
  const double beta = pg.it > 1 ? rho / pg.st->rho1 : 0.0;
  if (blockIdx.x == 0 && threadIdx.x == 0) *publish = rho;
  return beta;
}

constexpr int kTicketWords = 4;
__device__ __forceinline__ void reset_work_counters(unsigned long long *ticket) {
  ticket[0] = 0ull;
  ticket[2] = 0ull;
  ticket[3] = 0ull;
}

struct UnitQueue {
  unsigned long long *c0, *c1, *c2;
  long long base0, hi0, base1, hi1, base2, hi2;
  int stage;
};
__device__ __forceinline__ bool take_unit(unsigned long long *c, long long base, long long hi,
                                          long long &u) {
  if (base >= hi) return false;
  u = base + (long long)atomicAdd(c, 1ull);
  return u < hi;
}
__device__ __forceinline__ long long next_unit(UnitQueue &q, long long nunits) {
  long long u;
  if (q.stage == 0) {
    if (take_unit(q.c0, q.base0, q.hi0, u)) return u;
    q.stage = 1;
  }
  if (q.stage == 1) {
    if (take_unit(q.c1, q.base1, q.hi1, u)) return u;
    q.stage = 2;
  }
  if (q.stage == 2) {
    if (take_unit(q.c2, q.base2, q.hi2, u)) return u;
    q.stage = 3;
  }
  return nunits;
}

__device__ __forceinline__ bool gen_index(const SymGen &gs, int64_t pos, int64_t &g) {
  const int64_t off = pos % gs.blk;
  g = (pos / gs.blk) * gs.rows_per + off;
  return off < gs.rows_per && g < gs.N;
}

struct GenCols {
  double x[8][kSymGenMaxD];
  unsigned valid;
};
__device__ __forceinline__ void gen_load_cols(const SymGen &gs, int J, int lane, GenCols &gc) {
  gc.valid = 0u;
#pragma unroll
  for (int j = 0; j < 8; ++j) {
    int64_t g;
    const bool ok = gen_index(gs, (int64_t)J * B + 2 * (lane + 64 * (j >> 1)) + (j & 1), g);
    if (ok) gc.valid |= 1u << j;
#pragma unroll
    for (int t = 0; t < kSymGenMaxD; ++t) gc.x[j][t] = (ok && t < gs.d) ? gs.Xs[g * gs.d + t] : 0.0;
  }
}
__device__ __forceinline__ void gen_stage_rows(const SymGen &gs, int I, int r0, int nr,
                                               double *__restrict__ xrow) {
  for (int i = threadIdx.x; i < nr; i += 256) {
    int64_t g;
    const bool ok = gen_index(gs, (int64_t)I * B + r0 + i, g);
#pragma unroll
    for (int t = 0; t < kSymGenMaxD; ++t)
      xrow[4 * (r0 + i) + t] = (ok && t < gs.d) ? gs.Xs[g * gs.d + t] : 0.0;
    xrow[4 * (r0 + i) + 3] = ok ? 1.0 : 0.0;
  }
}
__device__ __forceinline__ bool gen_block_full(const SymGen &gs, int Jb) {
  int64_t g;
  const int64_t p0 = (int64_t)Jb * B, p1 = p0 + B - 1;
  return p0 / gs.blk == p1 / gs.blk && gen_index(gs, p0, g) && gen_index(gs, p1, g);
}
__device__ __forceinline__ void gen_row(const SymGen &gs, const GenCols &gc,
                                        const double *__restrict__ xrow, int r, int lane, bool plain,
                                        bool diag, d2 (&ar)[4]) {
  const double *xr = xrow + 4 * r;
  double x[kSymGenMaxD];
#pragma unroll
  for (int t = 0; t < kSymGenMaxD; ++t) x[t] = xr[t];
  double v[8];
#pragma unroll
  for (int j = 0; j < 8; ++j) {
    double s = 0.0;
#pragma unroll
    for (int t = 0; t < kSymGenMaxD; ++t) s = rbf_sqdist_step(s, __dsub_rn(gc.x[j][t], x[t]), t == 0);
    v[j] = rbf_of_sqdist(s);
  }
  if (!plain) {
    const bool rv = xr[3] != 0.0;
#pragma unroll
    for (int j = 0; j < 8; ++j) {
      const int c = 2 * (lane + 64 * (j >> 1)) + (j & 1);
      if (diag && c == r) v[j] = 1.0 + gs.jitter;
      if (!(rv && ((gc.valid >> j) & 1u))) v[j] = 0.0;
    }
  }
#pragma unroll
  for (int q = 0; q < 4; ++q) ar[q] = d2{v[2 * q], v[2 * q + 1]};
}


__device__ __forceinline__ void tile_load_batch(const double *A, int64_t rbase, int lane,
                                                d2 (&a)[kRB][4]) {
  const d2 *rowp = reinterpret_cast<const d2 *>(A + rbase * B) + lane;
#pragma unroll
  for (int rr = 0; rr < kRB; ++rr)
#pragma unroll
    for (int q = 0; q < 4; ++q) a[rr][q] = __builtin_nontemporal_load(rowp + rr * (B / 2) + 64 * q);
}

template <bool GEN>
__device__ __forceinline__ void tile_batch(const d2 (&a)[GEN ? 1 : kRB][4], const SymGen &gs,
                                           const GenCols &gc, const double *xrow,
                                           bool plain, bool diag, const d2 (&pc)[4],
                                           const double *vrow, int rbase, int lane,
                                           double *red, double *rows,
                                           d2 (&acc)[4]) {
#pragma unroll(GEN ? 2 : kRB)
  for (int rr = 0; rr < kRB; ++rr) {
    d2 ar[4];
    if constexpr (GEN) {
      gen_row(gs, gc, xrow, rbase + rr, lane, plain, diag, ar);
    } else {
#pragma unroll
      for (int q = 0; q < 4; ++q) ar[q] = a[rr][q];
    }
    double s0 = ar[0].x * pc[0].x;
    double s1 = ar[0].y * pc[0].y;
#pragma unroll
    for (int q = 1; q < 4; ++q) {
      s0 = fma(ar[q].x, pc[q].x, s0);
      s1 = fma(ar[q].y, pc[q].y, s1);
    }
    red[rr * 64 + lane] = s0 + s1;
    if (!diag) {
      const double pr = vrow[rbase + rr];
#pragma unroll
      for (int q = 0; q < 4; ++q) {
        acc[q].x = fma(ar[q].x, pr, acc[q].x);
        acc[q].y = fma(ar[q].y, pr, acc[q].y);
      }
    }
  }
  __builtin_amdgcn_fence(__ATOMIC_RELEASE, "wavefront");
  __builtin_amdgcn_wave_barrier();
  __builtin_amdgcn_fence(__ATOMIC_ACQUIRE, "wavefront");
  const d2 *rp = reinterpret_cast<const d2 *>(red + (lane >> 3) * 64 + (lane & 7) * 8);
  const d2 t0 = rp[0], t1 = rp[1], t2 = rp[2], t3 = rp[3];
  double tt = ((t0.x + t0.y) + (t1.x + t1.y)) + ((t2.x + t2.y) + (t3.x + t3.y));
  tt += __shfl_xor(tt, 1, 64);
  tt += __shfl_xor(tt, 2, 64);
  tt += __shfl_xor(tt, 4, 64);
  if ((lane & 7) == 0) rows[rbase + (lane >> 3)] = tt;
  __builtin_amdgcn_fence(__ATOMIC_RELEASE, "wavefront");
  __builtin_amdgcn_wave_barrier();
  __builtin_amdgcn_fence(__ATOMIC_ACQUIRE, "wavefront");
}

__device__ __forceinline__ void tile_stage_cols(const d2 (&acc)[4], double *cs, int w, int lane) {
  d2 *cs2 = reinterpret_cast<d2 *>(cs);
#pragma unroll
  for (int q = 0; q < 4; ++q) cs2[w * (B / 2) + lane + 64 * q] = acc[q];
}

__device__ __forceinline__ void tile_store_slots(double *P, double *Pq,
                                                 int64_t Np, int nb, int2 t, int h, int gb0, int gb1,
                                                 bool diag, const double *sh) {
  const double *rows = sh + B, *cs = sh + 2 * B;
  const int row0 = gb0 * kRB, nr = (gb1 - gb0) * kRB;
  double *Prow = P + (int64_t)t.y * Np + (int64_t)t.x * B + row0;
  for (int c = threadIdx.x; c < nr; c += 256) __builtin_nontemporal_store(rows[row0 + c], Prow + c);
  if (!diag) {
    double *Pc = h == 0 ? P : Pq + (int64_t)(h - 1) * nb * Np;
    double *Pcol = Pc + (int64_t)t.x * Np + (int64_t)t.y * B;
    for (int c = threadIdx.x; c < B; c += 256)
      __builtin_nontemporal_store((cs[c] + cs[B + c]) + (cs[2 * B + c] + cs[3 * B + c]), Pcol + c);
  }
}

__global__ __launch_bounds__(256) void k_symv_tiles(const double *__restrict__ tiles,
                                                    const int2 *__restrict__ list,
                                                    const double *__restrict__ v,
                                                    double *__restrict__ P,
                                                    double *__restrict__ Pq, int64_t Np,
                                                    int nwhole, int nb, int lsub,
                                                    const int *__restrict__ status) {
  if (status != nullptr && *status != ST_RUNNING) return;
  __shared__ double sh[kTileLds];
  const int lane = threadIdx.x & 63, w = threadIdx.x >> 6;
  int tile, h, gb0, gb1;
  decode_unit(blockIdx.x, nwhole, lsub, tile, h, gb0, gb1);
  const int2 t = list[tile];
  const double *A = tiles + (int64_t)tile * B * B;
  d2 pc[4], a[kRB][4];
#pragma unroll
  for (int q = 0; q < 4; ++q)
    pc[q] = *reinterpret_cast<const d2 *>(v + (int64_t)t.y * B + 2 * (lane + 64 * q));
  tile_load_batch(A, (int64_t)(gb0 + w) * kRB, lane, a);
  for (int i = gb0 * kRB + threadIdx.x; i < gb1 * kRB; i += 256) sh[i] = v[(int64_t)t.x * B + i];
  __syncthreads();
  const bool diag = t.x == t.y;
  const GenCols none{};
  d2 acc[4];
#pragma unroll
  for (int q = 0; q < 4; ++q) acc[q] = d2{0.0, 0.0};
#pragma unroll 1
  for (int g = gb0 + w; g < gb1; g += 4) {
    if (g != gb0 + w) tile_load_batch(A, g * kRB, lane, a);
    tile_batch<false>(a, SymGen{}, none, nullptr, false, diag, pc, sh, g * kRB, lane,
                      sh + kTileRed + w * kRB * 64, sh + B, acc);
  }
  if (!diag) tile_stage_cols(acc, sh + 2 * B, w, lane);
  __syncthreads();
  tile_store_slots(P, Pq, Np, nb, t, h, gb0, gb1, diag, sh);
}

struct SymvArgs {
  const double *tiles;
  const int2 *list;
  const double *v;
  double *P, *Pq;
  int64_t Np;
  int nwhole;
  long long nunits;
  int nb, lsub;
  PGather pg;
  double beta;
};

template <bool GEN>
__device__ __forceinline__ long long symv_units(const SymvArgs &k, const SymGen &gs, long long u,
                                                UnitQueue q, double *__restrict__ sh,
                                                long long *s_next) {
  const int lane = threadIdx.x & 63, w = threadIdx.x >> 6;
  double *vrow = sh, *rows = sh + B, *cs = sh + 2 * B;
  double *red = sh + kTileRed + w * kRB * 64;
  double *xrow = sh + kTileLds;
  const PGather &pg = k.pg;
  const double *v = k.v;
  const double beta = k.beta;
  long long units_done = 0;
  int tile, h, gb0, gb1;
  decode_unit(u, k.nwhole, k.lsub, tile, h, gb0, gb1);
  int2 t = k.list[tile];
  const double *A = k.tiles + (int64_t)tile * B * B;
  d2 pc[4], a[GEN ? 1 : kRB][4];
  GenCols gc;
#pragma unroll
  for (int q = 0; q < 4; ++q) pc[q] = pg_val2(pg, v, (int64_t)t.y * B + 2 * (lane + 64 * q), beta);
  if constexpr (!GEN) tile_load_batch(A, (int64_t)(gb0 + w) * kRB, lane, a);
  if (threadIdx.x == 0) *s_next = next_unit(q, k.nunits);
  for (int i = threadIdx.x; i < (gb1 - gb0) * kRB; i += 256) {
    const int64_t gi = (int64_t)t.x * B + gb0 * kRB + i;
    vrow[gb0 * kRB + i] = pg.gb != nullptr ? pg_val(pg, v, gi, beta) : v[gi];
  }
  if (GEN) {
    gen_stage_rows(gs, t.x, gb0 * kRB, (gb1 - gb0) * kRB, xrow);
    gen_load_cols(gs, t.y, lane, gc);
  }
  __syncthreads();
  while (true) {
    const bool diag = t.x == t.y;
    const bool plain = GEN && !diag && gen_block_full(gs, t.x) && gen_block_full(gs, t.y);
    d2 acc[4];
#pragma unroll
    for (int q = 0; q < 4; ++q) acc[q] = d2{0.0, 0.0};
#pragma unroll 1
    for (int g = gb0 + w; g < gb1; g += 4) {
      if constexpr (!GEN)
        if (g != gb0 + w) tile_load_batch(A, g * kRB, lane, a);
      tile_batch<GEN>(a, gs, gc, xrow, plain, diag, pc, vrow, g * kRB, lane, red, rows, acc);
    }
    if (!diag) tile_stage_cols(acc, cs, w, lane);
    __syncthreads();
    const long long un = *s_next;
    int tile2 = 0, h2 = 0, gb02 = 0, gb12 = 0;
    int2 t2 = t;
    const double *A2 = A;
    if (un < k.nunits) {
      decode_unit(un, k.nwhole, k.lsub, tile2, h2, gb02, gb12);
      t2 = k.list[tile2];
      A2 = k.tiles + (int64_t)tile2 * B * B;
#pragma unroll
      for (int q = 0; q < 4; ++q)
        pc[q] = pg_val2(pg, v, (int64_t)t2.y * B + 2 * (lane + 64 * q), beta);
      if constexpr (GEN)
        gen_load_cols(gs, t2.y, lane, gc);
      else
        tile_load_batch(A2, (int64_t)(gb02 + w) * kRB, lane, a);
    }
    tile_store_slots(k.P, k.Pq, k.Np, k.nb, t, h, gb0, gb1, diag, sh);
    __syncthreads();
    ++units_done;
    if (un >= k.nunits) break;
    if (threadIdx.x == 0) *s_next = next_unit(q, k.nunits);
    tile = tile2;
    h = h2;
    gb0 = gb02;
    gb1 = gb12;
    t = t2;
    A = A2;
    for (int i = threadIdx.x; i < (gb1 - gb0) * kRB; i += 256) {
      const int64_t gi = (int64_t)t.x * B + gb0 * kRB + i;
      vrow[gb0 * kRB + i] = pg.gb != nullptr ? pg_val(pg, v, gi, beta) : v[gi];
    }
    if (GEN) gen_stage_rows(gs, t.x, gb0 * kRB, (gb1 - gb0) * kRB, xrow);
    __syncthreads();
  }
  return units_done;
}

__device__ __forceinline__ unsigned cu_key() {
  unsigned xcc = 0, hw = 0;
  asm volatile("s_getreg_b32 %0, hwreg(HW_REG_XCC_ID)" : "=s"(xcc));
  asm volatile("s_getreg_b32 %0, hwreg(HW_REG_HW_ID)" : "=s"(hw));
  return ((xcc & 0xfu) << 8) | ((hw >> 8) & 0xffu);
}

constexpr int kTraceWords = 4;

template <bool ROLES>
__global__ __launch_bounds__(256) void k_symv_dyn(const double *__restrict__ tiles,
                                                  const int2 *__restrict__ list,
                                                  const double *__restrict__ v,
                                                  double *__restrict__ P,
                                                  double *__restrict__ Pq, int64_t Np,
                                                  int nwhole, long long nunits, int nb,
                                                  int lsub,
                                                  unsigned long long *__restrict__ ticket,
                                                  const int *__restrict__ status, PGather pg,
                                                  SymGen gs,
                                                  unsigned long long *wgtrace = nullptr) {
  if (status != nullptr && *status != ST_RUNNING) return;
  unsigned long long *tr = wgtrace != nullptr ? wgtrace + kTraceWords * blockIdx.x : nullptr;
  if (tr != nullptr && threadIdx.x == 0) tr[0] = wall_clock64();
  __shared__ double sh[kTileLds + (ROLES ? 4 * B : 0)];
  __shared__ long long s_next;
  __shared__ int s_role;
  if (!ROLES && (long long)blockIdx.x >= nunits) return;
  if (ROLES && threadIdx.x == 0) {
    int r = gs.roles == kSymRolesGen ? 1 : 0;
    if (gs.roles == kSymRolesIndex) r = (int)(blockIdx.x & 1u);
    if (gs.roles == kSymRolesCu) r = (int)(atomicAdd(ticket + kTicketWords + cu_key(), 1ull) & 1ull);
    s_role = r;
  }
  if (!ROLES && tr != nullptr && threadIdx.x == 0) tr[3] = 1ull | (unsigned long long)cu_key() << 2;
  const double beta = pg.gb != nullptr ? fused_p_beta(pg, gathered_rho(pg, sh), &pg.st->rho_new) : 0.0;
  UnitQueue q{ticket, ticket, ticket, (long long)gridDim.x, nunits, 0, 0, 0, 0, 0};
  long long u = blockIdx.x;
  bool gen = false;
  if (ROLES) {
    __syncthreads();
    gen = __builtin_amdgcn_readfirstlane(s_role) != 0;
    const bool pool_first = gs.pool_first != 0 && gs.qmode != (gen ? 1 : 2);
    unsigned long long *cs = ticket, *cg = ticket + 2, *cq = ticket + 3;
    const long long ns = gs.n_s;
    q.c0 = gen ? cg : cs;
    q.base0 = gen ? ns : 0;
    q.hi0 = gen ? nwhole : ns;
    unsigned long long *co = gen ? cs : cg;
    const long long olo = gen ? 0 : ns, ohi = gen ? ns : nwhole;
    q.c1 = pool_first ? cq : co;
    q.base1 = pool_first ? nwhole : olo;
    q.hi1 = pool_first ? nunits : ohi;
    q.c2 = pool_first ? co : cq;
    q.base2 = pool_first ? olo : nwhole;
    q.hi2 = pool_first ? ohi : nunits;
    if (threadIdx.x == 0) {
      s_next = next_unit(q, nunits);
      if (tr != nullptr) tr[3] = 1ull | (gen ? 2ull : 0ull) | (unsigned long long)cu_key() << 2;
    }
    __syncthreads();
    u = s_next;
    __syncthreads();
    if (u >= nunits) {
      if (tr != nullptr && threadIdx.x == 0) tr[1] = wall_clock64();
      return;
    }
  }
  const SymvArgs k{tiles, list, v, P, Pq, Np, nwhole, nunits, nb, lsub, pg, beta};
  long long units_done;
  if constexpr (ROLES) {
    if (gen)
      units_done = symv_units<true>(k, gs, u, q, sh, &s_next);
    else
      units_done = symv_units<false>(k, gs, u, q, sh, &s_next);
  } else {
    units_done = symv_units<false>(k, gs, u, q, sh, &s_next);
  }
  if (tr != nullptr && threadIdx.x == 0) {
    tr[1] = wall_clock64();
    tr[2] = (unsigned long long)units_done;
  }
}

template <bool EPI, bool PQ>
__global__ __launch_bounds__(256) void k_sym_reduce(const double *__restrict__ P,
                                                    const double *__restrict__ Pq,
                                                    const unsigned char *__restrict__ split,
                                                    int t_split, int64_t Np, int nb, int nq,
                                                    int64_t n_out, double *__restrict__ y,
                                                    double sigma, double lam,
                                                    const double *__restrict__ vloc,
                                                    double *__restrict__ pq_part,
                                                    unsigned long long *__restrict__ ticket,
                                                    const int *__restrict__ status,
                                                    PGather pg = PGather{},
                                                    double *pw = nullptr) {
  if (status != nullptr && *status != ST_RUNNING) return;
  if (blockIdx.x == 0 && threadIdx.x == 0) reset_work_counters(ticket);
  double apq = 0.0;
  const double beta = PQ && pg.gb != nullptr ? fused_p_beta(pg, pg.st->rho_new, &pg.st->rho) : 0.0;
  const int64_t pl = (int64_t)nb * Np;
  for (int64_t i = (int64_t)blockIdx.x * 256 + threadIdx.x; i < n_out;
       i += (int64_t)gridDim.x * 256) {
    const int bi = (int)(i / B);
    double s = 0.0;
    const int tend = t_split > bi ? t_split : bi + 1;
    const int t8 = tend < nb ? tend : nb;
    int t = 0;
    for (; t + 15 < t8; t += 16) {
      double v[16];
#pragma unroll
      for (int u = 0; u < 16; ++u) v[u] = __builtin_nontemporal_load(P + (int64_t)(t + u) * Np + i);
#pragma unroll
      for (int u = 0; u < 16; ++u) s += v[u];
    }
    for (; t + 7 < t8; t += 8) {
      double v[8];
#pragma unroll
      for (int u = 0; u < 8; ++u) v[u] = __builtin_nontemporal_load(P + (int64_t)(t + u) * Np + i);
#pragma unroll
      for (int u = 0; u < 8; ++u) s += v[u];
    }
    for (; t < nb; t += 8) {
      double v[8];
#pragma unroll
      for (int u = 0; u < 8; ++u) {
        v[u] = 0.0;
        const int tu = t + u;
        if (tu < nb) {
          v[u] = P[(int64_t)tu * Np + i];
          if (tu > bi && split[(int64_t)tu * nb + bi])
            for (int hq = 0; hq < nq; ++hq) v[u] += Pq[hq * pl + (int64_t)tu * Np + i];
        }
      }
#pragma unroll
      for (int u = 0; u < 8; ++u)
        if (t + u < nb) s += v[u];
    }
    if (EPI) {
      double pv = 0.0;
      if (PQ && pg.gb != nullptr) {
        pv = pg_val(pg, pw, i, beta);
        pw[i] = pv;
      } else if (vloc != nullptr) {
        pv = vloc[i];
      }
      double yv = sigma * s;
      if (vloc != nullptr) yv += lam * pv;
      y[i] = yv;
      if (PQ) apq = fma(pv, yv, apq);
    } else {
      y[i] = s;
    }
  }
  if (PQ) {
    __shared__ double sh[4];
    apq = block_sum256(apq, sh);
    if (threadIdx.x == 0) pq_part[blockIdx.x] = apq;
  }
}

struct PqPublish {
  double sigma = 0.0, lam = 0.0;
  int world = 0;
  bool ordered = true;
};

template <bool ORDERED>
__device__ __forceinline__ void pq_put(double *p, double v) {
  if (ORDERED)
    *p = v;
  else
    __hip_atomic_store(reinterpret_cast<unsigned long long *>(p), __builtin_bit_cast(unsigned long long, v),
                       __ATOMIC_RELAXED, __HIP_MEMORY_SCOPE_AGENT);
}
template <bool ORDERED>
__device__ __forceinline__ double pq_get(const double *p) {
  if (ORDERED) return *p;
  return __builtin_bit_cast(double, __hip_atomic_load(reinterpret_cast<const unsigned long long *>(p),
                                                      __ATOMIC_RELAXED, __HIP_MEMORY_SCOPE_AGENT));
}

template <bool ORDERED = true>
__device__ __forceinline__ void pq_publish_share(const double *pq_part, const double *pp_part, int np,
                                                 double sigma, double lam, int rank, int world,
                                                 int64_t blk, int64_t bstride, double *yg, double *sh) {
  double a = 0.0, b = 0.0;
  for (int i = threadIdx.x; i < np; i += 256) {
    a += pq_get<ORDERED>(pq_part + i);
    b += pq_get<ORDERED>(pp_part + i);
  }
  block_sum256_pair(a, b, sh);
  const double share = sigma * a + lam * b;
  for (int g = threadIdx.x; g < world; g += 256) yg[(int64_t)g * bstride + blk + rank] = share;
}

template <bool ORDERED>
__device__ __forceinline__ bool pq_arrive(double a, double b, double *pq_part, double *pp_part,
                                          unsigned long long *ticket, int *s_last) {
  if (threadIdx.x == 0) {
    pq_put<ORDERED>(pq_part + blockIdx.x, a);
    pq_put<ORDERED>(pp_part + blockIdx.x, b);
    if (ORDERED)
      __builtin_amdgcn_fence(__ATOMIC_RELEASE, "agent");
    else
      asm volatile("s_waitcnt vmcnt(0)" ::: "memory");
    const bool last = __hip_atomic_fetch_add(ticket + 1, 1ull, __ATOMIC_RELAXED, __HIP_MEMORY_SCOPE_AGENT) ==
                      (unsigned long long)(gridDim.x - 1);
    if (last) __hip_atomic_store(ticket + 1, 0ull, __ATOMIC_RELAXED, __HIP_MEMORY_SCOPE_AGENT);
    *s_last = last;
  }
  __syncthreads();
  if (!*s_last) return false;
  if (ORDERED)
    __builtin_amdgcn_fence(__ATOMIC_ACQUIRE, "agent");
  else
    __builtin_amdgcn_fence(__ATOMIC_ACQUIRE, "wavefront");
  return true;
}

template <bool ORDERED>
__device__ __forceinline__ void pq_tail(double apq, double app, double *pq_part, double *pp_part,
                                        unsigned long long *ticket, const PqPublish &pub, int rank,
                                        int64_t blk, int64_t bstride, double *yg, double *sh,
                                        int *s_last) {
  block_sum256_pair(apq, app, sh);
  if (pub.world == 0) {
    if (threadIdx.x == 0) {
      pq_part[blockIdx.x] = apq;
      pp_part[blockIdx.x] = app;
    }
    return;
  }
  if (!pq_arrive<ORDERED>(apq, app, pq_part, pp_part, ticket, s_last)) return;
  pq_publish_share<ORDERED>(pq_part, pp_part, (int)gridDim.x, pub.sigma, pub.lam, rank, pub.world, blk,
                            bstride, yg, sh);
}

template <bool PQ>
__global__ __launch_bounds__(256) void k_sym_reduce_w(const double *__restrict__ P,
                                                      const double *__restrict__ Pq,
                                                      const unsigned char *__restrict__ split,
                                                      int64_t Np, int nq,
                                                      int nb, int rank,
                                                      const int *__restrict__ own,
                                                      int64_t ld, int64_t blk, int64_t bstride,
                                                      double *__restrict__ yg,
                                                      double *p,
                                                      double *__restrict__ pq_part,
                                                      double *__restrict__ pp_part,
                                                      unsigned long long *__restrict__ ticket,
                                                      const int *__restrict__ status,
                                                      PGather pg, PqPublish pub) {
  if (status != nullptr && *status != ST_RUNNING) return;
  if (blockIdx.x == 0 && threadIdx.x == 0) reset_work_counters(ticket);
  __shared__ double sh[8];
  __shared__ int s_last;
  double apq = 0.0, app = 0.0;
  const double beta = PQ && pg.gb != nullptr ? fused_p_beta(pg, pg.st->rho_new, &pg.st->rho) : 0.0;
  const int64_t lo = (int64_t)rank * blk, hi = lo + blk;
  for (int64_t i = (int64_t)blockIdx.x * 256 + threadIdx.x; i < ld;
       i += (int64_t)gridDim.x * 256) {
    const int bi = __builtin_amdgcn_readfirstlane((int)(i / B));
    double s = 0.0;
    const int *ol = own + (int64_t)bi * nb;
    const int cnt = own[(int64_t)nb * nb + bi];
    const int64_t pl = (int64_t)nb * Np;
    for (int c = 0; c < cnt; c += 16) {
      double v[16];
#pragma unroll
      for (int u = 0; u < 16; ++u) {
        v[u] = 0.0;
        if (c + u < cnt) {
          const int e = ol[c + u];
          const int64_t at = (int64_t)sym_own_slot(e) * Np + i;
          v[u] = P[at];
          if (sym_own_split(e))
            for (int hq = 0; hq < nq; ++hq) v[u] += Pq[hq * pl + at];
        }
      }
#pragma unroll
      for (int u = 0; u < 16; ++u)
        if (c + u < cnt) s += v[u];
    }
    yg[(i / blk) * bstride + i % blk] = s;
    if (PQ) {
      double pv;
      if (pg.gb != nullptr) {
        pv = pg_val(pg, p, i, beta);
        p[i] = pv;
      } else {
        pv = p[i];
      }
      apq = fma(pv, s, apq);
      if (i >= lo && i < hi) app = fma(pv, pv, app);
    }
  }
  if (PQ) pq_tail<true>(apq, app, pq_part, pp_part, ticket, pub, rank, blk, bstride, yg, sh, &s_last);
}

constexpr int kRwBatch = 32;
constexpr int kRwMaxList = 2048;

template <bool PQ>
__global__ __launch_bounds__(256) void k_sym_reduce_wl(const double *__restrict__ P,
                                                       const double *__restrict__ Pq,
                                                       int64_t Np, int nb,
                                                       const int *__restrict__ plist,
                                                       int64_t pstride, int rank,
                                                       int64_t ld, int64_t blk, int64_t bstride,
                                                       double *__restrict__ yg, double *p,
                                                       double *__restrict__ pq_part,
                                                       double *__restrict__ pp_part,
                                                       unsigned long long *__restrict__ ticket,
                                                       const int *__restrict__ status,
                                                       PGather pg, PqPublish pub) {
  if (status != nullptr && *status != ST_RUNNING) return;
  if (blockIdx.x == 0 && threadIdx.x == 0) reset_work_counters(ticket);
  __shared__ double sh[8];
  __shared__ int s_last;
  __shared__ int sl[kRwMaxList];
  double apq = 0.0, app = 0.0;
  const double beta = PQ && pg.gb != nullptr ? fused_p_beta(pg, pg.st->rho_new, &pg.st->rho) : 0.0;
  const int64_t lo = (int64_t)rank * blk, hi = lo + blk;
  const int64_t plane = (int64_t)nb * Np;
  for (int64_t c0 = (int64_t)blockIdx.x * 256; c0 < ld; c0 += (int64_t)gridDim.x * 256) {
    const int64_t i = c0 + threadIdx.x;
    const int bi = (int)(c0 / B);
    const int cnt = plist[(int64_t)nb * pstride + bi];
    int le[kRwMaxList / 256];
#pragma unroll
    for (int q = 0; q < kRwMaxList / 256; ++q) {
      const int e = threadIdx.x + 256 * q;
      le[q] = e < pstride ? plist[(int64_t)bi * pstride + e] : 0;
    }
    double pz = 0.0, pold = 0.0;
    if (PQ && i < ld) {
      if (pg.gb != nullptr) {
        pz = pg_z(pg, i);
        if (pg.it > 1) pold = p[i];
      } else {
        pold = p[i];
      }
    }
    __syncthreads();
#pragma unroll
    for (int q = 0; q < kRwMaxList / 256; ++q)
      if (threadIdx.x + 256 * q < pstride) sl[threadIdx.x + 256 * q] = le[q];
    __syncthreads();
    const int lane32 = (int)(threadIdx.x & 31);
    auto entries = [&](int e0) { return sl[e0 + lane32 < cnt ? e0 + lane32 : cnt - 1]; };
    auto load = [&](int ent, int u) {
      const int x = __builtin_amdgcn_readlane(ent, u);
      const int h = sym_plist_plane(x);
      const double *base = h == 0 ? P : Pq + (int64_t)(h - 1) * plane;
      return base[(int64_t)sym_plist_slot(x) * Np + i];
    };
    double s = 0.0, cur = 0.0;
    if (cnt > 0 && i < ld) {
      double v[kRwBatch];
      int ev = entries(0);
#pragma unroll
      for (int u = 0; u < kRwBatch; ++u) v[u] = load(ev, u);
      for (int e0 = 0; e0 < cnt; e0 += kRwBatch) {
        double w[kRwBatch];
        const int ew = entries(e0 + kRwBatch < cnt ? e0 + kRwBatch : e0);
        if (e0 + kRwBatch < cnt) {
#pragma unroll
          for (int u = 0; u < kRwBatch; ++u) w[u] = load(ew, u);
        } else {
#pragma unroll
          for (int u = 0; u < kRwBatch; ++u) w[u] = 0.0;
        }
#pragma unroll
        for (int u = 0; u < kRwBatch; ++u) {
          if (e0 + u < cnt) {
            if (sym_plist_plane(__builtin_amdgcn_readlane(ev, u))) {
              cur += v[u];
            } else {
              s += cur;
              cur = v[u];
            }
          }
        }
#pragma unroll
        for (int u = 0; u < kRwBatch; ++u) v[u] = w[u];
        ev = ew;
      }
    }
    s += cur;
    if (i >= ld) continue;
    yg[(i / blk) * bstride + i % blk] = s;
    if (PQ) {
      double pv;
      if (pg.gb != nullptr) {
        pv = pg.it > 1 ? fma(beta, pold, pz) : pz;
        p[i] = pv;
      } else {
        pv = pold;
      }
      apq = fma(pv, s, apq);
      if (i >= lo && i < hi) app = fma(pv, pv, app);
    }
  }
  if (PQ) {
    if (pub.ordered)
      pq_tail<true>(apq, app, pq_part, pp_part, ticket, pub, rank, blk, bstride, yg, sh, &s_last);
    else
      pq_tail<false>(apq, app, pq_part, pp_part, ticket, pub, rank, blk, bstride, yg, sh, &s_last);
  }
}

__global__ __launch_bounds__(256) void k_pq_publish(const double *__restrict__ pq_part,
                                                    const double *__restrict__ pp_part, int np,
                                                    double sigma, double lam, int rank, int world,
                                                    int64_t blk, int64_t bstride,
                                                    double *__restrict__ yg,
                                                    const int *__restrict__ status) {
  if (status != nullptr && *status != ST_RUNNING) return;
  __shared__ double sh[8];
  pq_publish_share(pq_part, pp_part, np, sigma, lam, rank, world, blk, bstride, yg, sh);
}

__global__ __launch_bounds__(256) void k_axpby_loc(const double *__restrict__ src, double *y,
                                                   int64_t n, double sigma, double lam,
                                                   const double *__restrict__ vloc,
                                                   const int *__restrict__ status) {
  if (status != nullptr && *status != ST_RUNNING) return;
  const int64_t i = (int64_t)blockIdx.x * 256 + threadIdx.x;
  if (i >= n) return;
  double yv = sigma * src[i];
  if (vloc != nullptr) yv += lam * vloc[i];
  y[i] = yv;
}

template <bool COMPARE>
__global__ __launch_bounds__(256) void k_sym_pack(const double *__restrict__ K, int64_t ld,
                                                  int64_t rowbase, int64_t nloc, const int2 *__restrict__ list,
                                                  const unsigned char *__restrict__ trans,
                                                  double *__restrict__ tiles,
                                                  int *__restrict__ mismatch) {
  __shared__ double S[64][65];
  const int2 t = list[blockIdx.x];
  const bool tr = trans[blockIdx.x] != 0;
  double *T = tiles + (int64_t)blockIdx.x * B * B;
  const int tx = threadIdx.x & 63, ty = threadIdx.x >> 6;
  int bad = 0;
  for (int sb = 0; sb < (B / 64) * (B / 64); ++sb) {
    const int br = (sb / (B / 64)) * 64, bc = (sb % (B / 64)) * 64;
    const int64_t srow = tr ? (int64_t)t.y * B + bc : (int64_t)t.x * B + br;
    const int64_t scol = tr ? (int64_t)t.x * B + br : (int64_t)t.y * B + bc;
    __syncthreads();
    for (int a = ty; a < 64; a += 4) {
      const int64_t lr = srow + a - rowbase, c = scol + tx;
      S[a][tx] = (lr >= 0 && lr < nloc && c < ld) ? K[lr * ld + c] : 0.0;
    }
    __syncthreads();
    for (int a = ty; a < 64; a += 4) {
      const double val = tr ? S[tx][a] : S[a][tx];
      double *dst = T + (int64_t)(br + a) * B + bc + tx;
      if (COMPARE) {
        if (*dst != val) bad = 1;
      } else {
        *dst = val;
      }
    }
  }
  if (COMPARE && bad) atomicOr(mismatch, 1);
}

__global__ __launch_bounds__(256) void k_sym_gen_rbf(const int2 *__restrict__ list,
                                                     const double *__restrict__ Xs, int d,
                                                     double jitter, int64_t N, int64_t rows_per,
                                                     int64_t blk, double *__restrict__ tiles) {
  const int2 t = list[blockIdx.x];
  double *T = tiles + (int64_t)blockIdx.x * B * B;
  double xc[2][8];
  int64_t gc[2];
  bool vc[2];
#pragma unroll
  for (int h = 0; h < 2; ++h) {
    const int64_t pos = (int64_t)t.y * B + threadIdx.x + 256 * h;
    const int64_t off = pos % blk;
    gc[h] = (pos / blk) * rows_per + off;
    vc[h] = off < rows_per && gc[h] < N;
#pragma unroll
    for (int u = 0; u < 8; ++u) xc[h][u] = (vc[h] && u < d) ? Xs[gc[h] * d + u] : 0.0;
  }
  for (int r = 0; r < B; ++r) {
    const int64_t pos = (int64_t)t.x * B + r;
    const int64_t off = pos % blk;
    const int64_t gr = (pos / blk) * rows_per + off;
    const bool vr = off < rows_per && gr < N;
#pragma unroll
    for (int h = 0; h < 2; ++h) {
      double val = 0.0;
      if (vr && vc[h]) val = (gr == gc[h]) ? 1.0 + jitter : rbf_value(xc[h], Xs, gr, d);
      __builtin_nontemporal_store(val, T + (int64_t)r * B + threadIdx.x + 256 * h);
    }
  }
}

}

struct SymKnobs {
  int64_t whole_rounds = -1;
  int lsub = 2;
  bool dynamic = true;
  bool gen = true;
  int64_t gen_tiles = -1;
  int gen_quarters = 0;
  int roles = kSymRolesCu;
  int pool_first = 0;
  bool reduce_list = true;
  bool pq_ordered = false;
  long long trace_at = 0;
};

static SymKnobs sym_knobs() {
  SymKnobs k;
  if (const char *e = std::getenv("MLFF_SYM_WHOLE_ROUNDS")) k.whole_rounds = std::max<int64_t>(0, std::atoll(e));
  if (const char *e = std::getenv("MLFF_SYM_LSUB")) {
    const int v = std::atoi(e);
    if (v >= 1 && v <= 4) k.lsub = v;
  }
  if (const char *e = std::getenv("MLFF_SYM_SCHED")) k.dynamic = std::strcmp(e, "static") != 0;
  if (const char *e = std::getenv("MLFF_SYM_GEN")) k.gen = std::atoi(e) != 0;
  if (const char *e = std::getenv("MLFF_SYM_GEN_TILES")) k.gen_tiles = std::max<int64_t>(0, std::atoll(e));
  if (const char *e = std::getenv("MLFF_SYM_GEN_QUARTERS")) {
    const int v = std::atoi(e);
    if (v >= 0 && v <= 2) k.gen_quarters = v;
  }
  if (const char *e = std::getenv("MLFF_SYM_ROLES")) {
    if (std::strcmp(e, "index") == 0) k.roles = kSymRolesIndex;
    if (std::strcmp(e, "stream") == 0) k.roles = kSymRolesStream;
    if (std::strcmp(e, "gen") == 0) k.roles = kSymRolesGen;
  }
  if (const char *e = std::getenv("MLFF_SYM_STEAL")) k.pool_first = std::strcmp(e, "pool") == 0;
  if (const char *e = std::getenv("MLFF_SYM_REDUCE_LIST")) k.reduce_list = std::atoi(e) != 0;
  if (const char *e = std::getenv("MLFF_SYM_PQ_ORDERED")) k.pq_ordered = std::atoi(e) != 0;
  if (const char *e = std::getenv("MLFF_SYM_TRACE")) k.trace_at = std::atoll(e);
  return k;
}

static void print_symv_trace(const unsigned long long *tr, unsigned G, int64_t units, hipStream_t s) {
  std::vector<unsigned long long> h((size_t)kTraceWords * G);
  if (hipStreamSynchronize(s) != hipSuccess ||
      hipMemcpy(h.data(), tr, sizeof(unsigned long long) * h.size(), hipMemcpyDeviceToHost) != hipSuccess)
    return;
  unsigned long long t0 = ~0ull, t1 = 0;
  std::vector<double> st, en, un;
  for (unsigned g = 0; g < G; ++g) {
    const unsigned long long *r = &h[(size_t)kTraceWords * g];
    if (r[0] == 0) continue;
    t0 = std::min(t0, r[0]);
    t1 = std::max(t1, r[1]);
  }
  double idle = 0.0;
  std::vector<int> cu_s(kSymCuWords, 0), cu_g(kSymCuWords, 0);
  int xs[16] = {0}, xg[16] = {0};
  double un_s = 0.0, un_g = 0.0;
  for (unsigned g = 0; g < G; ++g) {
    const unsigned long long *r = &h[(size_t)kTraceWords * g];
    if (r[0] == 0) continue;
    st.push_back(10.0 * (double)(r[0] - t0));
    en.push_back(10.0 * (double)(r[1] - t0));
    un.push_back((double)r[2]);
    idle += 10.0 * (double)(t1 - r[1]) + 10.0 * (double)(r[0] - t0);
    if (!(r[3] & 1ull)) continue;
    const bool gen = (r[3] & 2ull) != 0;
    const unsigned key = (unsigned)(r[3] >> 2) & (kSymCuWords - 1);
    ++(gen ? cu_g : cu_s)[key];
    ++(gen ? xg : xs)[key >> 8];
    (gen ? un_g : un_s) += (double)r[2];
  }
  auto q = [](std::vector<double> v, double f) {
    std::sort(v.begin(), v.end());
    return v.empty() ? 0.0 : v[(size_t)(f * (double)(v.size() - 1))];
  };
  const double span = 10.0 * (double)(t1 - t0);
  std::fprintf(stderr,
               "[sym trace] units %lld on %zu workgroups (units per wg p0/p50/p100 %.0f/%.0f/%.0f); "
               "span %.1f us; starts p50/p100 %.1f/%.1f us; ends p0/p10/p50/p90/p100 "
               "%.1f/%.1f/%.1f/%.1f/%.1f us; idle (ramp + tail) %.1f %% of wg-time\n",
               (long long)units, st.size(), q(un, 0.0), q(un, 0.5), q(un, 1.0), 1e-3 * span,
               1e-3 * q(st, 0.5), 1e-3 * q(st, 1.0), 1e-3 * q(en, 0.0), 1e-3 * q(en, 0.1),
               1e-3 * q(en, 0.5), 1e-3 * q(en, 0.9), 1e-3 * q(en, 1.0),
               100.0 * idle / (span * (double)st.size()));
  int cus = 0, paired = 0, two_s = 0, two_g = 0, other = 0;
  for (int k = 0; k < kSymCuWords; ++k) {
    if (cu_s[k] + cu_g[k] == 0) continue;
    ++cus;
    if (cu_s[k] == 1 && cu_g[k] == 1)
      ++paired;
    else if (cu_s[k] == 2 && cu_g[k] == 0)
      ++two_s;
    else if (cu_s[k] == 0 && cu_g[k] == 2)
      ++two_g;
    else
      ++other;
  }
  std::string per_xcc;
  for (int x = 0; x < 16; ++x)
    if (xs[x] + xg[x] > 0)
      per_xcc += " " + std::to_string(x) + ":" + std::to_string(xs[x]) + "s+" + std::to_string(xg[x]) + "g";
  std::fprintf(stderr,
               "[sym trace] roles: %d distinct CU keys; CUs holding {stream + gen} %d, {2 stream} %d, "
               "{2 gen} %d, other %d; units taken stream / gen %.0f / %.0f; per XCC id%s\n",
               cus, paired, two_s, two_g, other, un_s, un_g, per_xcc.c_str());
}

void launch_symv(const SymPack &sp, const double *v_full, double *P, const int *status,
                 hipStream_t s, PGather pg) {
  if (sp.ntiles == 0) return;
  const int64_t grid = sp.nwhole + ((sp.ntiles - sp.nwhole) << sp.lsub);
  if (sp.dyn == 0) {
    hipLaunchKernelGGL(k_symv_tiles, dim3((unsigned)grid), dim3(256), 0, s, sp.tiles, sp.list, v_full,
                       P, sp.Pq, sp.Np, (int)sp.nwhole, (int)sp.nb, sp.lsub, status);
    return;
  }
  const unsigned G = (unsigned)std::min<int64_t>(sp.dyn, grid);
  static const long long trace_at = sym_knobs().trace_at;
  static long long launches = 0;
  unsigned long long *tr = nullptr;
  if (trace_at > 0 && ++launches == trace_at &&
      hipMalloc(&tr, sizeof(unsigned long long) * kTraceWords * G) == hipSuccess)
    (void)hipMemsetAsync(tr, 0, sizeof(unsigned long long) * kTraceWords * G, s);
  if (sp.gen)
    hipLaunchKernelGGL(k_symv_dyn<true>, dim3(G), dim3(256), 0, s,
                       sp.tiles, sp.list, v_full, P, sp.Pq, sp.Np, (int)sp.nwhole, (long long)grid,
                       (int)sp.nb, sp.lsub, sp.ticket, status, pg, sp.gsrc, tr);
  else
    hipLaunchKernelGGL(k_symv_dyn<false>, dim3(G), dim3(256), 0, s,
                       sp.tiles, sp.list, v_full, P, sp.Pq, sp.Np, (int)sp.nwhole, (long long)grid,
                       (int)sp.nb, sp.lsub, sp.ticket, status, pg, SymGen{}, tr);
  if (tr != nullptr) {
    print_symv_trace(tr, G, grid, s);
    (void)hipFree(tr);
  }
}

void launch_sym_reduce(const SymPack &sp, int64_t n_out, double *y, bool epilogue, double sigma,
                       double lam, const double *vloc, const int *status, hipStream_t s) {
  if (n_out <= 0) return;
  const dim3 grid((unsigned)((n_out + 255) / 256));
  if (epilogue)
    hipLaunchKernelGGL((k_sym_reduce<true, false>), grid, dim3(256), 0, s, sp.P, sp.Pq, sp.split,
                       (int)sp.t_split, sp.Np, (int)sp.nb, (1 << sp.lsub) - 1, n_out, y, sigma, lam, vloc,
                       (double *)nullptr, sp.ticket, status);
  else
    hipLaunchKernelGGL((k_sym_reduce<false, false>), grid, dim3(256), 0, s, sp.P, sp.Pq, sp.split,
                       (int)sp.t_split, sp.Np, (int)sp.nb, (1 << sp.lsub) - 1, n_out, y, sigma, lam, vloc,
                       (double *)nullptr, sp.ticket, status);
}

void launch_sym_reduce_pq(const SymPack &sp, int64_t n_out, double *y, double sigma, double lam,
                          const double *p, double *pq_part, const int *status, hipStream_t s,
                          PGather pg) {
  hipLaunchKernelGGL((k_sym_reduce<true, true>), dim3(kVecGrid), dim3(256), 0, s, sp.P, sp.Pq,
                     sp.split, (int)sp.t_split, sp.Np, (int)sp.nb, (1 << sp.lsub) - 1, n_out, y, sigma,
                     lam, p, pq_part,
                     sp.ticket, status, pg, pg.gb != nullptr ? const_cast<double *>(p) : nullptr);
}

static bool sym_reduce_list(const SymPack &sp) {
  return sp.plist != nullptr && sp.pstride <= kRwMaxList && sp.nb <= kSymPlistMaxSlots;
}

void launch_sym_reduce_ranks(const SymPack &sp, int rank, int world, int64_t blk,
                             const double *p_full, double *pq_part, double *pp_part,
                             double sigma, double lam, const int *status, hipStream_t s,
                             PGather pg, bool separate_publish) {
  const int64_t ld = (int64_t)world * blk;
  const dim3 grid(kVecGrid);
  double *pw = const_cast<double *>(p_full);
  const PqPublish pub = p_full == nullptr
                            ? PqPublish{}
                            : PqPublish{sigma, lam, separate_publish ? 0 : world, sp.pq_ordered};
  const PGather pgu = p_full == nullptr ? PGather{} : pg;
  if (sym_reduce_list(sp)) {
    if (p_full == nullptr)
      hipLaunchKernelGGL((k_sym_reduce_wl<false>), grid, dim3(256), 0, s, sp.P, sp.Pq, sp.Np,
                         (int)sp.nb, sp.plist, sp.pstride, rank, ld, blk, sp.ystride, sp.yg, pw,
                         pq_part, pp_part, sp.ticket, status, pgu, pub);
    else
      hipLaunchKernelGGL((k_sym_reduce_wl<true>), grid, dim3(256), 0, s, sp.P, sp.Pq, sp.Np,
                         (int)sp.nb, sp.plist, sp.pstride, rank, ld, blk, sp.ystride, sp.yg, pw,
                         pq_part, pp_part, sp.ticket, status, pgu, pub);
  } else if (p_full == nullptr) {
    hipLaunchKernelGGL((k_sym_reduce_w<false>), grid, dim3(256), 0, s, sp.P, sp.Pq, sp.split, sp.Np,
                       (1 << sp.lsub) - 1, (int)sp.nb, rank,
                       sp.own, ld, blk, sp.ystride, sp.yg, pw, pq_part, pp_part,
                       sp.ticket, status, pgu, pub);
  } else {
    hipLaunchKernelGGL((k_sym_reduce_w<true>), grid, dim3(256), 0, s, sp.P, sp.Pq, sp.split, sp.Np,
                       (1 << sp.lsub) - 1, (int)sp.nb, rank,
                       sp.own, ld, blk, sp.ystride, sp.yg, pw, pq_part, pp_part,
                       sp.ticket, status, pgu, pub);
  }
  if (p_full != nullptr && separate_publish)
    hipLaunchKernelGGL(k_pq_publish, dim3(1), dim3(256), 0, s, pq_part, pp_part, kVecGrid, sigma, lam,
                       rank, world, blk, sp.ystride, sp.yg, status);
}

void launch_axpby_loc(const double *src, double *y, int64_t n, double sigma, double lam,
                      const double *vloc, const int *status, hipStream_t s) {
  if (n <= 0) return;
  hipLaunchKernelGGL(k_axpby_loc, dim3((unsigned)((n + 255) / 256)), dim3(256), 0, s, src, y, n,
                     sigma, lam, vloc, status);
}

static int owner_host(int I, int J, int tpr) {
  const int a = I / tpr, c = J / tpr;
  if (a == c) return a;
  return ((I + J) & 1) ? a : c;
}


struct SymPlan {
  int64_t Np = 0;
  int nb = 0, tpr = 0;
  std::vector<int2> list;
  std::vector<unsigned char> trans;
  int64_t nt = 0, nwhole = 0;
  int lsub = 2;
  int64_t nq = 3;
  int64_t dyn = 0;
  bool gen = false;
  SymGen gsrc;
};

static SymPlan sym_plan(const mlff_ctx *ctx, const SymKnobs &kn) {
  SymPlan pl;
  pl.Np = round_up(ctx->ld, B);
  pl.nb = (int)(pl.Np / B);
  pl.tpr = ctx->world > 1 ? (int)(ctx->blk / B) : pl.nb;
  for (int I = 0; I < pl.nb; ++I)
    for (int J = 0; J <= I; ++J) {
      if (owner_host(I, J, pl.tpr) != ctx->rank) continue;
      pl.list.push_back(make_int2(I, J));
      pl.trans.push_back(ctx->world > 1 && (I / pl.tpr) != ctx->rank ? 1 : 0);
    }
  pl.nt = (int64_t)pl.list.size();
  int cus = 0;
  if (hipDeviceGetAttribute(&cus, hipDeviceAttributeMultiprocessorCount, ctx->device) != hipSuccess ||
      cus < 1)
    cus = 256;
  const int64_t C = 2 * (int64_t)cus;
  pl.nwhole = (pl.nt / C) * C;
  if (kn.whole_rounds >= 0) pl.nwhole = std::min<int64_t>(pl.nwhole, kn.whole_rounds * C);
  pl.lsub = kn.lsub;
  pl.nq = ((int64_t)1 << pl.lsub) - 1;
  pl.dyn = kn.dynamic ? C : 0;
  if (pl.dyn > 0 && pl.nt > 0 && !ctx->has_matrix && ctx->rbf.ready && ctx->rbf.d >= 1 &&
      ctx->rbf.d <= kSymGenMaxD) {
    int64_t n_s = (int64_t)((double)pl.nwhole * kSymStreamRate / (kSymStreamRate + kSymGenRate) + 0.5);
    if (kn.gen_tiles >= 0) n_s = pl.nwhole - std::min<int64_t>(pl.nwhole, kn.gen_tiles);
    const int qmode = kn.gen_quarters;
    bool on = kn.gen;
    if (pl.nwhole == pl.nt && n_s == pl.nwhole) on = false;
    if (n_s == pl.nwhole && qmode == 1) on = false;
    if (on) {
      pl.gen = true;
      pl.gsrc = SymGen{ctx->rbf.Xs, ctx->rbf.d, ctx->rbf.jitter, ctx->N, ctx->rows_per, ctx->blk,
                       (int)n_s, qmode, kn.roles, kn.pool_first};
    }
  }
  return pl;
}

static int sym_alloc(mlff_ctx *ctx, const SymPlan &pl, const SymKnobs &kn) {
  SymPack &sp = ctx->sym;
  hipStream_t s = ctx->stream;
  const int64_t nt = pl.nt, nb = pl.nb, Np = pl.Np, nq = pl.nq;
  if (sp.tiles == nullptr || sp.ntiles != nt || sp.Np != Np || sp.pq_planes != nq) {
    sym_free(sp);
    if (nt > 0) {
      MLFF_HIP(ctx, hipMalloc(&sp.tiles, sizeof(double) * nt * B * B));
      MLFF_HIP(ctx, hipMalloc(&sp.list, sizeof(int2) * nt));
    }
    MLFF_HIP(ctx, hipMalloc(&sp.P, sizeof(double) * nb * Np));
    MLFF_HIP(ctx, hipMemsetAsync(sp.P, 0, sizeof(double) * nb * Np, s));
    MLFF_HIP(ctx, hipMalloc(&sp.Pq, sizeof(double) * nq * nb * Np));
    MLFF_HIP(ctx, hipMemsetAsync(sp.Pq, 0, sizeof(double) * nq * nb * Np, s));
    sp.pq_planes = nq;
    MLFF_HIP(ctx, hipMalloc(&sp.split, (size_t)nb * nb));
    MLFF_HIP(ctx, hipMalloc(&sp.own, sizeof(int) * (size_t)nb * (nb + 1)));
    const size_t tw = (kTicketWords + kSymCuWords) * sizeof(unsigned long long);
    MLFF_HIP(ctx, hipMalloc(&sp.ticket, tw));
    MLFF_HIP(ctx, hipMemsetAsync(sp.ticket, 0, tw, s));
    if (ctx->world > 1) {
      sp.ystride = ctx->blk + round_up(ctx->world, kPad);
      const int64_t ny = (int64_t)ctx->world * sp.ystride;
      MLFF_HIP(ctx, hipMalloc(&sp.yg, sizeof(double) * ny));
      MLFF_HIP(ctx, hipMalloc(&sp.yr, sizeof(double) * sp.ystride));
      MLFF_HIP(ctx, hipMemsetAsync(sp.yg, 0, sizeof(double) * ny, s));
      MLFF_HIP(ctx, hipMemsetAsync(sp.yr, 0, sizeof(double) * sp.ystride, s));
    }
  }
  sp.ntiles = nt;
  sp.Np = Np;
  sp.nb = nb;
  sp.tiles_per_rank = pl.tpr;
  sp.nwhole = pl.nwhole;
  sp.lsub = pl.lsub;
  sp.dyn = pl.dyn;
  sp.gen = pl.gen;
  sp.gsrc = pl.gsrc;
  sp.pq_ordered = kn.pq_ordered;
  return MLFF_OK;
}

static int sym_slot_tables(mlff_ctx *ctx, const SymPlan &pl, const SymKnobs &kn) {
  SymPack &sp = ctx->sym;
  hipStream_t s = ctx->stream;
  const int nb = pl.nb;
  std::vector<unsigned char> split((size_t)nb * nb, 0);
  sp.t_split = nb;
  for (int64_t t = pl.nwhole; t < pl.nt; ++t) {
    split[(size_t)pl.list[t].x * nb + pl.list[t].y] = 1;
    sp.t_split = std::min<int64_t>(sp.t_split, pl.list[t].x);
  }
  MLFF_HIP(ctx, hipMemcpyAsync(sp.split, split.data(), split.size(), hipMemcpyHostToDevice, s));
  std::vector<int> own((size_t)nb * (nb + 1), 0);
  for (int bi = 0; bi < nb; ++bi) {
    int c = 0;
    for (int t = 0; t < nb; ++t)
      if (owner_host(std::max(bi, t), std::min(bi, t), pl.tpr) == ctx->rank)
        own[(size_t)bi * nb + c++] = sym_own_entry(t, t > bi && split[(size_t)t * nb + bi]);
    own[(size_t)nb * nb + bi] = c;
  }
  MLFF_HIP(ctx, hipMemcpyAsync(sp.own, own.data(), sizeof(int) * own.size(), hipMemcpyHostToDevice, s));
  std::vector<std::vector<int>> lists((size_t)nb);
  sp.pmax = 0;
  for (int bi = 0; bi < nb; ++bi) {
    for (int j = 0; j < own[(size_t)nb * nb + bi]; ++j) {
      const int e = own[(size_t)bi * nb + j];
      for (int h = 0; h <= (sym_own_split(e) ? pl.nq : 0); ++h)
        lists[bi].push_back(sym_plist_entry(sym_own_slot(e), h));
    }
    sp.pmax = std::max(sp.pmax, (int)lists[bi].size());
  }
  sp.pstride = round_up(std::max(sp.pmax, 1), 64);
  std::vector<int> plist((size_t)nb * (sp.pstride + 1), 0);
  for (int bi = 0; bi < nb; ++bi) {
    std::copy(lists[bi].begin(), lists[bi].end(), plist.begin() + (size_t)bi * sp.pstride);
    plist[(size_t)nb * sp.pstride + bi] = (int)lists[bi].size();
  }
  if (sp.plist != nullptr) (void)hipFree(sp.plist);
  sp.plist = nullptr;
  if (ctx->world > 1 && kn.reduce_list) {
    MLFF_HIP(ctx, hipMalloc(&sp.plist, sizeof(int) * plist.size()));
    MLFF_HIP(ctx, hipMemcpyAsync(sp.plist, plist.data(), sizeof(int) * plist.size(),
                                 hipMemcpyHostToDevice, s));
  }
  MLFF_HIP(ctx, hipStreamSynchronize(s));
  return MLFF_OK;
}

static int sym_fill(mlff_ctx *ctx, const SymPlan &pl, bool check_symmetry, bool *symmetric_out) {
  SymPack &sp = ctx->sym;
  hipStream_t s = ctx->stream;
  const int64_t nt = pl.nt;
  if (symmetric_out) *symmetric_out = true;
  if (nt == 0) return MLFF_OK;
  MLFF_HIP(ctx, hipMemcpyAsync(sp.list, pl.list.data(), sizeof(int2) * nt, hipMemcpyHostToDevice, s));
  if (!ctx->has_matrix && ctx->rbf.ready) {
    hipLaunchKernelGGL(k_sym_gen_rbf, dim3((unsigned)nt), dim3(256), 0, s, sp.list, ctx->rbf.Xs,
                       ctx->rbf.d, ctx->rbf.jitter, ctx->N, ctx->rows_per, ctx->blk, sp.tiles);
    MLFF_HIP(ctx, hipGetLastError());
    MLFF_HIP(ctx, hipStreamSynchronize(s));
    return MLFF_OK;
  }
  unsigned char *dtrans = nullptr;
  int *dflag = nullptr;
  MLFF_HIP(ctx, hipMalloc(&dtrans, nt));
  MLFF_HIP(ctx, hipMalloc(&dflag, sizeof(int)));
  MLFF_HIP(ctx, hipMemcpyAsync(dtrans, pl.trans.data(), nt, hipMemcpyHostToDevice, s));
  MLFF_HIP(ctx, hipMemsetAsync(dflag, 0, sizeof(int), s));
  const int64_t rowbase = (int64_t)ctx->rank * ctx->blk;
  hipLaunchKernelGGL(k_sym_pack<false>, dim3((unsigned)nt), dim3(256), 0, s, ctx->K, ctx->ld, rowbase,
                     ctx->blk, sp.list, dtrans, sp.tiles, dflag);
  int mism = 0;
  if (check_symmetry) {
    MLFF_HIP(ctx, hipMemsetAsync(dtrans, 1, nt, s));
    hipLaunchKernelGGL(k_sym_pack<true>, dim3((unsigned)nt), dim3(256), 0, s, ctx->K, ctx->ld, rowbase,
                       ctx->blk, sp.list, dtrans, sp.tiles, dflag);
    MLFF_HIP(ctx, hipMemcpyAsync(&mism, dflag, sizeof(int), hipMemcpyDeviceToHost, s));
  }
  MLFF_HIP(ctx, hipGetLastError());
  MLFF_HIP(ctx, hipStreamSynchronize(s));
  (void)hipFree(dtrans);
  (void)hipFree(dflag);
  if (symmetric_out) *symmetric_out = (mism == 0);
  return MLFF_OK;
}

int sym_build(mlff_ctx *ctx, bool check_symmetry, bool *symmetric_out) {
  const SymKnobs kn = sym_knobs();
  const SymPlan pl = sym_plan(ctx, kn);
  if (int rc = sym_alloc(ctx, pl, kn); rc != MLFF_OK) return rc;
  if (int rc = sym_slot_tables(ctx, pl, kn); rc != MLFF_OK) return rc;
  if (int rc = sym_fill(ctx, pl, check_symmetry, symmetric_out); rc != MLFF_OK) return rc;
  ctx->sym.ready = true;
  return MLFF_OK;
}

void sym_free(SymPack &sp) {
  for (void *p : {(void *)sp.tiles, (void *)sp.list, (void *)sp.P, (void *)sp.yg, (void *)sp.yr,
                  (void *)sp.Pq, (void *)sp.split, (void *)sp.ticket, (void *)sp.own,
                  (void *)sp.plist})
    if (p) (void)hipFree(p);
  sp = SymPack{};
}

}
```

### mlff-preconditioner_amd/sgdml_amd/_native.py

```python
from __future__ import annotations

import ctypes
import os
from pathlib import Path

import numpy as np

PKG_ROOT = Path(__file__).resolve().parent.parent
LIB_PATH = Path(os.environ.get("MLFF_PCG_LIB", PKG_ROOT / "lib" / "libmlffpcg.so"))

MLFF_OK = 0
MLFF_ERR_ARG = -1
MLFF_ERR_HIP = -2
MLFF_ERR_NOT_PSD = -3
MLFF_ERR_LINALG = -4
MLFF_ERR_STATE = -5
MLFF_ERR_COMM = -6
MLFF_ERR_NOMEM = -7

PRECON_NONE, PRECON_PIVCHOL, PRECON_NYSTROM, PRECON_NYSTROM_SB, PRECON_LOWRANK, PRECON_EIG = range(6)
PCG_RUNNING, PCG_CONVERGED, PCG_MAXITER = 0, 2, 3
STORAGE_DENSE, STORAGE_SYMTILE, STORAGE_AUTO, STORAGE_MATFREE = 0, 1, 2, 3

_c_ctx = ctypes.c_void_p
_p_dbl = ctypes.POINTER(ctypes.c_double)
_p_i64 = ctypes.POINTER(ctypes.c_int64)
_p_i32 = ctypes.POINTER(ctypes.c_int32)
_p_int = ctypes.POINTER(ctypes.c_int)
_i64 = ctypes.c_int64
_int = ctypes.c_int
_dbl = ctypes.c_double

SIGNATURES = {
    "mlff_version": (_int, []),
    "mlff_build_hash": (ctypes.c_char_p, []),
    "mlff_device_count": (_int, [_p_int]),
    "mlff_comm_unique_id": (_int, [ctypes.c_char_p]),
    "mlff_comm_selftest": (_int, [_int, _i64, ctypes.POINTER(ctypes.c_double)]),
    "mlff_ctx_create": (_int, [_int, _int, _int, ctypes.c_char_p, _i64, ctypes.POINTER(_c_ctx)]),
    "mlff_ctx_destroy": (_int, [_c_ctx]),
    "mlff_last_error": (ctypes.c_char_p, [_c_ctx]),
    "mlff_shard_range": (_int, [_c_ctx, _p_i64, _p_i64]),
    "mlff_comm_abort": (_int, [_c_ctx]),
    "mlff_matrix_ld": (_int, [_c_ctx, _p_i64]),
    "mlff_synchronize": (_int, [_c_ctx]),
    "mlff_stream": (_int, [_c_ctx, ctypes.POINTER(ctypes.c_void_p)]),
    "mlff_set_matrix_host": (_int, [_c_ctx, _p_dbl, _i64]),
    "mlff_get_matrix_rows": (_int, [_c_ctx, _i64, _i64, _p_dbl, _i64]),
    "mlff_gen_rbf": (_int, [_c_ctx, _p_dbl, _int, _dbl, _dbl]),
    "mlff_assemble_sgdml": (_int, [_c_ctx, _p_dbl, _p_dbl, _i64, _int, _p_i32, _int, _dbl]),
    "mlff_sgdml_operator": (_int, [_c_ctx, _p_dbl, _p_dbl, _i64, _int, _p_i32, _int, _dbl]),
    "mlff_set_energy_constraints": (_int, [_c_ctx, _int]),
    "mlff_spectrum": (_int, [_c_ctx, _int, _p_dbl]),
    "mlff_test_gemm": (_int, [_c_ctx, _int, _int, _i64, _i64, _i64, _dbl, _p_dbl, _i64, _p_dbl,
                              _i64, _dbl, _p_dbl, _i64, _int]),
    "mlff_dense_cho_solve": (_int, [_c_ctx, _dbl, _dbl, _p_dbl, _p_dbl, _p_dbl]),
    "mlff_test_potrf": (_int, [_c_ctx, _p_dbl, _i64, _int, _p_dbl, _p_dbl]),
    "mlff_test_gram": (_int, [_c_ctx, _p_dbl, _i64, _i64, _int, _p_dbl]),
    "mlff_sgdml_energies": (_int, [_c_ctx, _p_dbl, _p_dbl, _p_i64, _p_i64]),
    "mlff_sgdml_descriptors": (_int, [_p_dbl, _i64, _int, _p_dbl, _p_dbl]),
    "mlff_predict_set_model": (_int, [_c_ctx, _p_dbl, _p_dbl, _i64, _int, _p_i32, _int, _dbl, _dbl,
                                      _dbl]),
    "mlff_predict": (_int, [_c_ctx, _p_dbl, _i64, _p_dbl, _p_dbl]),
    "mlff_predict_info": (_int, [_c_ctx, _p_int, _p_i64, _p_dbl, _p_dbl]),
    "mlff_set_operator": (_int, [_c_ctx, _dbl, _dbl]),
    "mlff_matvec": (_int, [_c_ctx, _p_dbl, _p_dbl]),
    "mlff_get_diag": (_int, [_c_ctx, _p_dbl]),
    "mlff_set_storage": (_int, [_c_ctx, _int]),
    "mlff_storage_info": (_int, [_c_ctx, _p_int, _p_dbl]),
    "mlff_operator_form": (_int, [_c_ctx, _p_int]),
    "mlff_precon_none": (_int, [_c_ctx]),
    "mlff_precon_pivchol": (_int, [_c_ctx, _i64, _int, _p_i64, _p_dbl]),
    "mlff_precon_nystrom": (_int, [_c_ctx, _p_i64, _i64, _int, _p_dbl]),
    "mlff_pivchol_times": (_int, [_c_ctx, _p_dbl, _i64, _p_dbl]),
    "mlff_precon_lowrank": (_int, [_c_ctx, _p_dbl, _i64]),
    "mlff_precon_eig": (_int, [_c_ctx, _i64, _int, _i64, _int, _p_dbl, _p_dbl]),
    "mlff_precon_info": (_int, [_c_ctx, _p_int, _p_i64]),
    "mlff_precon_apply_traffic": (_int, [_c_ctx, _p_int, _p_dbl]),
    "mlff_precon_apply": (_int, [_c_ctx, _p_dbl, _p_dbl]),
    "mlff_precon_get_panel": (_int, [_c_ctx, _p_dbl, _i64]),
    "mlff_lev_scores": (_int, [_c_ctx, _p_i64, _i64, _dbl, _p_dbl]),
    "mlff_eig_info": (_int, [_c_ctx, _p_int, _p_dbl]),
    "mlff_cho_factor_stable": (_int, [_c_ctx, _p_dbl, _i64, _p_dbl, _p_dbl]),
    "mlff_sym_min_eig": (_int, [_c_ctx, _p_dbl, _i64, _p_dbl, _p_dbl, _p_dbl]),
    "mlff_pcg_start": (_int, [_c_ctx, _p_dbl, _p_dbl, _dbl, _i64, _p_int]),
    "mlff_pcg_run": (_int, [_c_ctx, _i64, _i64, _p_int]),
    "mlff_pcg_result": (_int, [_c_ctx, _p_i64, _p_int, _p_dbl, _p_int]),
    "mlff_pcg_get_x": (_int, [_c_ctx, _p_dbl]),
    "mlff_pcg_get_trace": (_int, [_c_ctx, _p_dbl, _i64]),
    "mlff_timing_enable": (_int, [_c_ctx, _int]),
    "mlff_timing_read": (_int, [_c_ctx, _p_dbl, _p_i64, _p_dbl, _p_i64]),
    "mlff_timing_reset": (_int, [_c_ctx]),
    "mlff_timing_read_precon": (_int, [_c_ctx, _p_dbl, _p_i64]),
    "mlff_timing_read_comm": (_int, [_c_ctx, _p_dbl, _p_i64]),
    "mlff_device_memory": (_int, [_c_ctx, _p_i64, _p_i64]),
}

_lib = None


def load_library(path: str | os.PathLike | None = None):
    global _lib
    if _lib is not None:
        return _lib
    try:
        import torch
    except Exception:
        pass
    p = Path(path) if path is not None else Path(os.environ.get("MLFF_LIB") or LIB_PATH)
    if not p.exists():
        raise ImportError(
            f"libmlffpcg.so not found at {p}: build it with "
            "`python mlff-preconditioner_amd/build_native.py` (no CPU fallback exists)")
    lib = ctypes.CDLL(str(p))
    for name, (res, args) in SIGNATURES.items():
        fn = getattr(lib, name)
        fn.restype = res
        fn.argtypes = args
    _lib = lib
    return lib


def last_error(ctx=None) -> str:
    lib = load_library()
    msg = lib.mlff_last_error(ctx)
    return msg.decode() if msg else ""


def check(rc: int, ctx=None, what: str = ""):
    if rc == MLFF_OK:
        return
    msg = f"{what}: {last_error(ctx)}" if what else last_error(ctx)
    if rc == MLFF_ERR_NOT_PSD:
        raise AssertionError(msg)
    if rc == MLFF_ERR_LINALG:
        raise np.linalg.LinAlgError(msg)
    if rc == MLFF_ERR_ARG:
        raise ValueError(msg)
    raise RuntimeError(f"libmlffpcg error {rc}: {msg}")


def dptr(a: np.ndarray | None):
    if a is None:
        return None
    assert a.dtype == np.float64 and a.flags.c_contiguous
    return a.ctypes.data_as(_p_dbl)


def i64ptr(a: np.ndarray | None):
    if a is None:
        return None
    assert a.dtype == np.int64 and a.flags.c_contiguous
    return a.ctypes.data_as(_p_i64)


def i32ptr(a: np.ndarray):
    assert a.dtype == np.int32 and a.flags.c_contiguous
    return a.ctypes.data_as(_p_i32)


def build_hash() -> str:
    return load_library().mlff_build_hash().decode()


def device_count() -> int:
    lib = load_library()
    n = ctypes.c_int(0)
    rc = lib.mlff_device_count(ctypes.byref(n))
    return n.value if rc == MLFF_OK else 0


def comm_unique_id() -> bytes:
    lib = load_library()
    buf = ctypes.create_string_buffer(128)
    check(lib.mlff_comm_unique_id(buf), None, "mlff_comm_unique_id")
    return buf.raw


def comm_selftest(device: int = 0, count: int = 1 << 20) -> float:
    lib = load_library()
    err = ctypes.c_double(-1.0)
    check(lib.mlff_comm_selftest(int(device), int(count), ctypes.byref(err)), None, "mlff_comm_selftest")
    return err.value
```

### mlff-preconditioner_amd/sgdml_amd/solver.py

```python
from __future__ import annotations

import ctypes
import threading
from dataclasses import dataclass, field

import numpy as np

from . import _native as nat


@dataclass
class PCGResult:
    x: np.ndarray
    info: int
    iters: int
    resid: float
    trace: np.ndarray
    early_exit: bool = False
    callbacks: int = 0
    extra: dict = field(default_factory=dict)


class KernelSolver:
    def __init__(self, n: int, device: int | None = None, rank: int = 0, world: int = 1,
                 comm_id: bytes | None = None):
        self._lib = nat.load_library()
        self._close_lock = threading.Lock()
        self.n = int(n)
        self.rank, self.world = int(rank), int(world)
        if device is None:
            ndev = nat.device_count()
            device = rank % max(ndev, 1)
        self.device = int(device)
        ctx = ctypes.c_void_p()
        cid = None if comm_id is None else ctypes.c_char_p(bytes(comm_id))
        nat.check(self._lib.mlff_ctx_create(self.device, self.rank, self.world, cid, self.n,
                                            ctypes.byref(ctx)), None, "mlff_ctx_create")
        self._ctx = ctx
        r0, nr = ctypes.c_int64(), ctypes.c_int64()
        self._call("mlff_shard_range", ctypes.byref(r0), ctypes.byref(nr))
        self.row0, self.nrows = r0.value, nr.value

    def _call(self, name, *args):
        rc = getattr(self._lib, name)(self._ctx, *args)
        if rc != nat.MLFF_OK and self.world > 1 and rc not in (nat.MLFF_ERR_NOT_PSD,
                                                                nat.MLFF_ERR_LINALG):
            try:
                nat.check(rc, self._ctx, name)
            finally:
                self._lib.mlff_comm_abort(self._ctx)
        nat.check(rc, self._ctx, name)

    def close(self):
        lock = getattr(self, "_close_lock", None)
        if lock is None:
            return
        with lock:
            ctx = getattr(self, "_ctx", None)
            self._ctx = None
            if ctx is not None and ctx.value is not None:
                self._lib.mlff_ctx_destroy(ctx)

    def __del__(self):
        try:
            self.close()
        except Exception:
            pass

    def __enter__(self):
        return self

    def __exit__(self, *exc):
        self.close()

    def row_range(self) -> tuple[int, int]:
        return self.row0, self.row0 + self.nrows

    def synchronize(self):
        self._call("mlff_synchronize")

    def stream_handle(self) -> int:
        p = ctypes.c_void_p()
        self._call("mlff_stream", ctypes.byref(p))
        return p.value or 0

    def set_matrix(self, K_local: np.ndarray):
        K_local = np.ascontiguousarray(K_local, dtype=np.float64)
        if K_local.shape != (self.nrows, self.n):
            raise ValueError(f"K_local must have shape {(self.nrows, self.n)}, got {K_local.shape}")
        self._call("mlff_set_matrix_host", nat.dptr(K_local), self.n)

    def get_matrix_rows(self, r0: int = 0, nr: int | None = None) -> np.ndarray:
        nr = self.nrows - r0 if nr is None else nr
        out = np.empty((nr, self.n))
        self._call("mlff_get_matrix_rows", int(r0), int(nr), nat.dptr(out), self.n)
        return out

    def gen_rbf(self, X: np.ndarray, length_scale: float = 1.0, jitter: float = 0.0):
        X = np.ascontiguousarray(X, dtype=np.float64)
        if X.ndim != 2 or X.shape[0] != self.n:
            raise ValueError("X must be N x d")
        self._call("mlff_gen_rbf", nat.dptr(X), int(X.shape[1]), float(length_scale), float(jitter))

    def sgdml_operator(self, R_desc: np.ndarray, R_d_desc: np.ndarray, perms: np.ndarray,
                       sig: float, use_E_cstr: bool = False):
        self._call("mlff_set_energy_constraints", int(bool(use_E_cstr)))
        R_desc = np.ascontiguousarray(R_desc, dtype=np.float64)
        R_d_desc = np.ascontiguousarray(R_d_desc, dtype=np.float64)
        perms = np.ascontiguousarray(np.atleast_2d(perms), dtype=np.int32)
        M, D = R_desc.shape
        n_atoms = perms.shape[1]
        if R_d_desc.shape != (M, D, 3) or D != n_atoms * (n_atoms - 1) // 2:
            raise ValueError("R_desc / R_d_desc / perms shapes do not match")
        self._call("mlff_sgdml_operator", nat.dptr(R_desc), nat.dptr(R_d_desc), M, n_atoms,
                   nat.i32ptr(perms), perms.shape[0], float(sig))

    def assemble_sgdml(self, R_desc: np.ndarray, R_d_desc: np.ndarray, perms: np.ndarray,
                       sig: float, use_E_cstr: bool = False):
        self._call("mlff_set_energy_constraints", int(bool(use_E_cstr)))
        R_desc = np.ascontiguousarray(R_desc, dtype=np.float64)
        R_d_desc = np.ascontiguousarray(R_d_desc, dtype=np.float64)
        perms = np.ascontiguousarray(np.atleast_2d(perms), dtype=np.int32)
        M, D = R_desc.shape
        n_atoms = perms.shape[1]
        if R_d_desc.shape != (M, D, 3) or D != n_atoms * (n_atoms - 1) // 2:
            raise ValueError("R_desc / R_d_desc / perms shapes are inconsistent")
        self._call("mlff_assemble_sgdml", nat.dptr(R_desc), nat.dptr(R_d_desc), int(M),
                   int(n_atoms), nat.i32ptr(perms), int(perms.shape[0]), float(sig))

    def sgdml_energies(self, alphas: np.ndarray) -> tuple[int, np.ndarray]:
        alphas = np.ascontiguousarray(alphas, dtype=np.float64)
        if alphas.shape != (self.n,):
            raise ValueError("alphas must have N entries")
        E = np.empty(self.n)
        i0, ni = ctypes.c_int64(), ctypes.c_int64()
        self._call("mlff_sgdml_energies", nat.dptr(alphas), nat.dptr(E), ctypes.byref(i0),
                   ctypes.byref(ni))
        return i0.value, E[: ni.value].copy()

    def predict_set_model(self, R_desc: np.ndarray, R_d_desc_alpha: np.ndarray, perms: np.ndarray,
                          sig: float, std: float = 1.0, c: float = 0.0):
        R_desc = np.ascontiguousarray(R_desc, dtype=np.float64)
        Rda = np.ascontiguousarray(R_d_desc_alpha, dtype=np.float64)
        perms = np.ascontiguousarray(np.atleast_2d(perms), dtype=np.int32)
        if R_desc.ndim != 2:
            raise ValueError("R_desc must be M x D")
        M, D = R_desc.shape
        n_atoms = perms.shape[1]
        if Rda.shape != (M, D) or D != n_atoms * (n_atoms - 1) // 2:
            raise ValueError("R_desc / R_d_desc_alpha / perms shapes do not match")
        self._call("mlff_predict_set_model", nat.dptr(R_desc), nat.dptr(Rda), int(M), int(n_atoms),
                   nat.i32ptr(perms), int(perms.shape[0]), float(sig), float(std), float(c))
        self._pred_n_atoms = n_atoms

    def predict(self, R: np.ndarray) -> tuple[np.ndarray, np.ndarray]:
        R = np.ascontiguousarray(R, dtype=np.float64)
        n = getattr(self, "_pred_n_atoms", None)
        if n is not None and (R.ndim != 3 or R.shape[1:] != (n, 3)):
            raise ValueError(f"R must be Q x {n} x 3, got {R.shape}")
        if n is None and (R.ndim != 3 or R.shape[2] != 3):
            raise ValueError("R must be Q x n_atoms x 3")
        Q, n = R.shape[0], R.shape[1]
        E = np.empty(Q)
        F = np.empty((Q, 3 * n))
        self._call("mlff_predict", nat.dptr(R), int(Q), nat.dptr(E), nat.dptr(F))
        return E, F

    def predict_info(self) -> tuple[str, int, float, float]:
        form, slab = ctypes.c_int(), ctypes.c_int64()
        fl, by = ctypes.c_double(), ctypes.c_double()
        self._call("mlff_predict_info", ctypes.byref(form), ctypes.byref(slab), ctypes.byref(fl),
                   ctypes.byref(by))
        return {0: "tile", 1: "stream"}[form.value], slab.value, fl.value, by.value

    def set_operator(self, sigma_K: float, lam: float):
        self._call("mlff_set_operator", float(sigma_K), float(lam))

    def set_storage(self, mode: str):
        code = {"dense": nat.STORAGE_DENSE, "sym": nat.STORAGE_SYMTILE,
                "auto": nat.STORAGE_AUTO, "matfree": nat.STORAGE_MATFREE}[mode]
        self._call("mlff_set_storage", code)

    def storage_info(self) -> tuple[str, float]:
        mode = ctypes.c_int()
        nbytes = ctypes.c_double()
        self._call("mlff_storage_info", ctypes.byref(mode), ctypes.byref(nbytes))
        name = {nat.STORAGE_SYMTILE: "sym", nat.STORAGE_MATFREE: "matfree"}.get(mode.value,
                                                                                "dense")
        return name, nbytes.value

    def operator_form(self) -> str | None:
        f = ctypes.c_int()
        self._call("mlff_operator_form", ctypes.byref(f))
        return {0: "pair", 1: "rec", 2: "pt"}.get(f.value)

    def matvec(self, v: np.ndarray) -> np.ndarray:
        v = np.ascontiguousarray(v, dtype=np.float64)
        if v.shape != (self.n,):
            raise ValueError("v must have N entries")
        y = np.empty(self.nrows)
        self._call("mlff_matvec", nat.dptr(v), nat.dptr(y))
        return y

    def spectrum(self, preconditioned: bool = True) -> np.ndarray:
        out = np.empty(self.n)
        self._call("mlff_spectrum", int(bool(preconditioned)), nat.dptr(out))
        return out

    def dense_cho_solve(self, b: np.ndarray, sigma_K: float = -1.0, shift: float = 1e-10,
                        want_seconds: bool = False):
        b = np.ascontiguousarray(b, dtype=np.float64)
        if b.shape != (self.n,):
            raise ValueError("b must have N entries")
        x = np.empty(self.n)
        sec = np.zeros(3)
        self._call("mlff_dense_cho_solve", float(sigma_K), float(shift), nat.dptr(b), nat.dptr(x),
                   nat.dptr(sec))
        return (x, sec) if want_seconds else x

    def test_potrf(self, A: np.ndarray, variant: int = 1, want_seconds: bool = False):
        A = np.ascontiguousarray(A, dtype=np.float64)
        if A.ndim != 2 or A.shape[0] != A.shape[1]:
            raise ValueError("A must be square")
        L = np.empty_like(A)
        sec = ctypes.c_double()
        self._call("mlff_test_potrf", nat.dptr(A), A.shape[0], int(variant), nat.dptr(L),
                   ctypes.byref(sec))
        return (L, sec.value) if want_seconds else L

    def diag(self) -> np.ndarray:
        d = np.empty(self.nrows)
        self._call("mlff_get_diag", nat.dptr(d))
        return d

    def precon_none(self):
        self._call("mlff_precon_none")

    def precon_pivchol(self, k: int, build_woodbury: bool = True):
        idx = np.empty(self.n, dtype=np.int64)
        sec = ctypes.c_double()
        self._call("mlff_precon_pivchol", int(k), int(bool(build_woodbury)), nat.i64ptr(idx),
                   ctypes.byref(sec))
        return idx, sec.value

    def pivchol_times(self, k: int) -> tuple[np.ndarray, float]:
        t = np.empty(int(k))
        w = ctypes.c_double()
        self._call("mlff_pivchol_times", nat.dptr(t), int(k), ctypes.byref(w))
        return t, w.value

    def precon_nystrom(self, idx: np.ndarray, variant: int = 0) -> float:
        idx = np.ascontiguousarray(idx, dtype=np.int64)
        sec = ctypes.c_double()
        self._call("mlff_precon_nystrom", nat.i64ptr(idx), int(idx.size), int(variant),
                   ctypes.byref(sec))
        return sec.value

    def precon_lowrank(self, Lt_local: np.ndarray):
        Lt_local = np.ascontiguousarray(Lt_local, dtype=np.float64)
        k = Lt_local.shape[0]
        if Lt_local.shape != (k, self.nrows):
            raise ValueError("Lt_local must be k x nrows")
        self._call("mlff_precon_lowrank", nat.dptr(Lt_local), int(k))

    def precon_eig(self, k: int, mask_mode: int = 0, dim_i: int = 0, build_woodbury: bool = True,
                   want_evals: bool = False, want_rowlev: bool = False):
        ev = np.empty(int(k)) if want_evals else None
        rl = np.empty(self.n) if want_rowlev else None
        self._call("mlff_precon_eig", int(k), int(mask_mode), int(dim_i), int(bool(build_woodbury)),
                   nat.dptr(ev), nat.dptr(rl))
        return ev, rl

    def eig_info(self) -> tuple[bool, float]:
        c, r = ctypes.c_int(), ctypes.c_double()
        self._call("mlff_eig_info", ctypes.byref(c), ctypes.byref(r))
        return bool(c.value), r.value

    def precon_info(self) -> tuple[int, int]:
        kind, k = ctypes.c_int(), ctypes.c_int64()
        self._call("mlff_precon_info", ctypes.byref(kind), ctypes.byref(k))
        return kind.value, k.value

    def precon_apply_traffic(self) -> tuple[int, float]:
        one, b = ctypes.c_int(), ctypes.c_double()
        self._call("mlff_precon_apply_traffic", ctypes.byref(one), ctypes.byref(b))
        return one.value, b.value

    def precon_apply(self, r_local: np.ndarray) -> np.ndarray:
        r_local = np.ascontiguousarray(r_local, dtype=np.float64)
        z = np.empty(self.nrows)
        self._call("mlff_precon_apply", nat.dptr(r_local), nat.dptr(z))
        return z

    def precon_panel(self) -> np.ndarray:
        _, k = self.precon_info()
        T = np.empty((k, self.nrows))
        self._call("mlff_precon_get_panel", nat.dptr(T), self.nrows)
        return T

    def cho_factor_stable(self, M: np.ndarray) -> tuple[np.ndarray, float]:
        M = np.ascontiguousarray(M, dtype=np.float64)
        if M.ndim != 2 or M.shape[0] != M.shape[1]:
            raise ValueError("M must be square")
        L = np.empty_like(M)
        lo = ctypes.c_double()
        self._call("mlff_cho_factor_stable", nat.dptr(M), M.shape[0], nat.dptr(L), ctypes.byref(lo))
        return L, lo.value

    def sym_min_eig(self, M: np.ndarray, want_tridiag: bool = False):
        M = np.ascontiguousarray(M, dtype=np.float64)
        if M.ndim != 2 or M.shape[0] != M.shape[1]:
            raise ValueError("M must be square")
        m = M.shape[0]
        lo = ctypes.c_double()
        d = np.empty(m) if want_tridiag else None
        e = np.empty(max(m - 1, 1)) if want_tridiag else None
        self._call("mlff_sym_min_eig", nat.dptr(M), m, ctypes.byref(lo), nat.dptr(d), nat.dptr(e))
        return (lo.value, d, e[: m - 1]) if want_tridiag else lo.value

    def lev_scores(self, idx: np.ndarray, lam: float) -> np.ndarray:
        idx = np.ascontiguousarray(idx, dtype=np.int64)
        out = np.empty(self.n)
        self._call("mlff_lev_scores", nat.i64ptr(idx), int(idx.size), float(lam), nat.dptr(out))
        return out

    def pcg_start(self, b_local: np.ndarray, x0_local: np.ndarray | None = None,
                  tol: float = 1e-5, maxiter: int | None = None) -> bool:
        b_local = np.ascontiguousarray(b_local, dtype=np.float64)
        if b_local.shape != (self.nrows,):
            raise ValueError("b_local must have nrows entries")
        x0p = None
        if x0_local is not None:
            x0_local = np.ascontiguousarray(x0_local, dtype=np.float64)
            if x0_local.shape != (self.nrows,):
                raise ValueError("x0_local must have nrows entries")
            x0p = nat.dptr(x0_local)
        maxiter = 10 * self.n if maxiter is None else int(maxiter)
        early = ctypes.c_int()
        self._call("mlff_pcg_start", nat.dptr(b_local), x0p, float(tol), maxiter,
                   ctypes.byref(early))
        self._maxiter = maxiter
        return bool(early.value)

    def pcg_run(self, n_iter: int, chunk: int = 0) -> int:
        st = ctypes.c_int()
        self._call("mlff_pcg_run", int(n_iter), int(chunk), ctypes.byref(st))
        return st.value

    def pcg_result(self) -> tuple[int, int, float, int]:
        it, st, res, info = ctypes.c_int64(), ctypes.c_int(), ctypes.c_double(), ctypes.c_int()
        self._call("mlff_pcg_result", ctypes.byref(it), ctypes.byref(st), ctypes.byref(res),
                   ctypes.byref(info))
        return it.value, st.value, res.value, info.value

    def pcg_x(self) -> np.ndarray:
        x = np.empty(self.nrows)
        self._call("mlff_pcg_get_x", nat.dptr(x))
        return x

    def pcg_trace(self) -> np.ndarray:
        it = self.pcg_result()[0]
        t = np.empty(it + 1)
        self._call("mlff_pcg_get_trace", nat.dptr(t), it + 1)
        return t

    def pcg(self, b_local: np.ndarray, x0_local: np.ndarray | None = None, tol: float = 1e-5,
            maxiter: int | None = None, callback=None, cb_every: int = 0,
            chunk: int = 0) -> PCGResult:
        early = self.pcg_start(b_local, x0_local, tol, maxiter)
        status = self.pcg_result()[1]
        step = int(cb_every) if cb_every and cb_every > 0 else self._maxiter
        while status == nat.PCG_RUNNING:
            status = self.pcg_run(step, chunk)
            if callback is not None and status == nat.PCG_RUNNING:
                it, _, res, _ = self.pcg_result()
                callback(self.pcg_x(), it, res)
        it, status, resid, info = self.pcg_result()
        x = self.pcg_x()
        trace = self.pcg_trace()
        callbacks = 0 if early else max(it, 1)
        return PCGResult(x=x, info=info, iters=it, resid=resid, trace=trace,
                         early_exit=early, callbacks=callbacks)

    def timing(self, on: bool | int = True):
        self._call("mlff_timing_enable", int(on) if not isinstance(on, bool) else int(on))

    def timing_reset(self):
        self._call("mlff_timing_reset")

    def timing_read(self) -> dict:
        gm, gc, im, ic = ctypes.c_double(), ctypes.c_int64(), ctypes.c_double(), ctypes.c_int64()
        self._call("mlff_timing_read", ctypes.byref(gm), ctypes.byref(gc), ctypes.byref(im),
                   ctypes.byref(ic))
        pm, pc = ctypes.c_double(), ctypes.c_int64()
        self._call("mlff_timing_read_precon", ctypes.byref(pm), ctypes.byref(pc))
        cm, cc = ctypes.c_double(), ctypes.c_int64()
        self._call("mlff_timing_read_comm", ctypes.byref(cm), ctypes.byref(cc))
        return {"gemv_ms": gm.value, "gemv_count": gc.value, "iter_ms": im.value,
                "iter_count": ic.value, "precon_ms": pm.value, "precon_count": pc.value,
                "comm_ms": cm.value, "comm_count": cc.value}

    def device_memory(self) -> tuple[int, int]:
        fr, tot = ctypes.c_int64(), ctypes.c_int64()
        self._call("mlff_device_memory", ctypes.byref(fr), ctypes.byref(tot))
        return fr.value, tot.value


def host_descriptors(R: np.ndarray) -> tuple[np.ndarray, np.ndarray]:
    R = np.asarray(R, dtype=np.float64)
    a, b = np.tril_indices(R.shape[1], k=-1)
    diff = R[:, a, :] - R[:, b, :]
    r = np.sqrt(np.sum(diff ** 2, axis=2))
    return 1.0 / r, diff / (r ** 3)[:, :, None]


def sgdml_descriptors(R: np.ndarray) -> tuple[np.ndarray, np.ndarray]:
    lib = nat.load_library()
    R = np.ascontiguousarray(R, dtype=np.float64)
    M, n = R.shape[0], R.shape[1]
    D = n * (n - 1) // 2
    Rd = np.empty((M, D))
    Rdd = np.empty((M, D, 3))
    nat.check(lib.mlff_sgdml_descriptors(nat.dptr(R), M, n, nat.dptr(Rd), nat.dptr(Rdd)), None,
              "mlff_sgdml_descriptors")
    return Rd, Rdd
```

Measured before the change: 557.4.

## Add three-workgroup-per-CU symmetric gen path with lean exp and compile-time tile variants

```diff
diff --git a/include/mlffpcg.h b/include/mlffpcg.h
--- a/include/mlffpcg.h
+++ b/include/mlffpcg.h
@@ -77,6 +77,7 @@
                      double *d_out, double *e_out);
 int mlff_sgdml_descriptors(const double *R, int64_t M, int n_atoms, double *R_desc_out,
                            double *R_d_desc_out);
+int mlff_test_rbf_exp(mlff_ctx *ctx, const double *s, int64_t n, double *lib_out, double *lean_out);
 
 int mlff_sgdml_energies(mlff_ctx *ctx, const double *alphas, double *E_out, int64_t *i0_out,
                         int64_t *ni_out);
@@ -92,6 +93,7 @@
 int mlff_matvec(mlff_ctx *ctx, const double *v_global, double *y_local);
 int mlff_set_storage(mlff_ctx *ctx, int mode);
 int mlff_storage_info(mlff_ctx *ctx, int *mode_out, double *bytes_per_matvec_out);
+int mlff_sym_launch_info(mlff_ctx *ctx, int *wgs_per_cu_out, int64_t *grid_out);
 #define MLFF_MF_FORM_PAIR 0
 #define MLFF_MF_FORM_REC 1
 #define MLFF_MF_FORM_PTILE 2
diff --git a/mlff-preconditioner_amd/csrc/api.hip b/mlff-preconditioner_amd/csrc/api.hip
--- a/mlff-preconditioner_amd/csrc/api.hip
+++ b/mlff-preconditioner_amd/csrc/api.hip
@@ -1450,6 +1450,26 @@
   MLFF_API_END(ctx)
 }
 
+int mlff_test_rbf_exp(mlff_ctx *ctx, const double *s, int64_t n, double *lib_out, double *lean_out) {
+  MLFF_API_BEGIN
+  MLFF_ENTER(ctx);
+  if (s == nullptr || lib_out == nullptr || lean_out == nullptr || n < 1)
+    return set_error(ctx, MLFF_ERR_ARG, "test_rbf_exp: bad arguments");
+  ScratchScope scope(ctx);
+  double *ds = nullptr, *da = nullptr, *db = nullptr;
+  MLFF_TRY(scratch_alloc(ctx, &ds, (size_t)n));
+  MLFF_TRY(scratch_alloc(ctx, &da, (size_t)n));
+  MLFF_TRY(scratch_alloc(ctx, &db, (size_t)n));
+  MLFF_HIP(ctx, hipMemcpyAsync(ds, s, sizeof(double) * n, hipMemcpyHostToDevice, ctx->stream));
+  launch_rbf_exp_probe(ds, n, da, db, ctx->stream);
+  MLFF_HIP(ctx, hipGetLastError());
+  MLFF_HIP(ctx, hipMemcpyAsync(lib_out, da, sizeof(double) * n, hipMemcpyDeviceToHost, ctx->stream));
+  MLFF_HIP(ctx, hipMemcpyAsync(lean_out, db, sizeof(double) * n, hipMemcpyDeviceToHost, ctx->stream));
+  MLFF_HIP(ctx, hipStreamSynchronize(ctx->stream));
+  return MLFF_OK;
+  MLFF_API_END(ctx)
+}
+
 int mlff_sgdml_descriptors(const double *R, int64_t M, int n_atoms, double *R_desc_out,
                            double *R_d_desc_out) {
   MLFF_API_BEGIN
@@ -1573,6 +1593,18 @@
     *mode_out = ctx->use_mf ? MLFF_STORAGE_MATFREE
                             : (ctx->use_sym ? MLFF_STORAGE_SYMTILE : MLFF_STORAGE_DENSE);
   if (bytes_per_matvec_out) *bytes_per_matvec_out = operator_bytes(ctx);
+  return MLFF_OK;
+  MLFF_API_END(ctx)
+}
+
+int mlff_sym_launch_info(mlff_ctx *ctx, int *wgs_per_cu_out, int64_t *grid_out) {
+  MLFF_API_BEGIN
+  MLFF_ENTER(ctx);
+  MLFF_TRY(require_operator(ctx));
+  MLFF_TRY(resolve_storage(ctx));
+  if (!ctx->use_sym || !ctx->sym.ready) return set_error(ctx, MLFF_ERR_STATE, "no symmetric tile operator");
+  if (wgs_per_cu_out) *wgs_per_cu_out = ctx->sym.wgs;
+  if (grid_out) *grid_out = ctx->sym.dyn;
   return MLFF_OK;
   MLFF_API_END(ctx)
 }
diff --git a/mlff-preconditioner_amd/csrc/common.h b/mlff-preconditioner_amd/csrc/common.h
--- a/mlff-preconditioner_amd/csrc/common.h
+++ b/mlff-preconditioner_amd/csrc/common.h
@@ -40,8 +40,9 @@
 };
 
 constexpr int kSymGenMaxD = 3;
-constexpr double kSymStreamRate = 4990.0;
-constexpr double kSymGenRate = 4990.0;
+constexpr double kSymStreamRate = 5600.0;
+constexpr double kSymGenRate = 5600.0;
+constexpr int kSymThreeWgMinUnits = 2;
 struct SymGen {
   const double *Xs = nullptr;
   int d = 0;
@@ -51,6 +52,7 @@
   int qmode = 0;
   int roles = 0;
   int pool_first = 0;
+  int wgs = 2;
 };
 enum SymRoles : int { kSymRolesCu = 0, kSymRolesIndex = 1, kSymRolesStream = 2, kSymRolesGen = 3 };
 constexpr int kSymCuWords = 4096;
@@ -76,6 +78,8 @@
   bool pq_ordered = false;
   int64_t t_split = 0;
   int64_t dyn = 0;
+  int wgs = 0;
+  bool rb4 = false;
   unsigned long long *ticket = nullptr;
   bool gen = false;
   SymGen gsrc;
@@ -163,6 +167,27 @@
   return first ? __dmul_rn(df, df) : fma(df, df, s);
 }
 __device__ __forceinline__ double rbf_of_sqdist(double s) { return exp(-0.5 * s); }
+__device__ __forceinline__ double rbf_exp_c(unsigned long long bits) {
+  return __builtin_bit_cast(double, bits);
+}
+__device__ __forceinline__ double rbf_of_sqdist_lean(double s) {
+  const double x = __builtin_fmax(-0.5 * s, -1075.0);
+  const double n = __builtin_rint(__dmul_rn(x, rbf_exp_c(0x3FF71547652B82FEull)));
+  double r = fma(-n, rbf_exp_c(0x3FE62E42FEFA39EFull), x);
+  r = fma(-n, rbf_exp_c(0x3C7ABC9E3B39803Full), r);
+  double p = fma(r, rbf_exp_c(0x3E5ADE156A5DCB37ull), rbf_exp_c(0x3E928AF3FCA7AB0Cull));
+  p = fma(r, p, rbf_exp_c(0x3EC71DEE623FDE64ull));
+  p = fma(r, p, rbf_exp_c(0x3EFA01997C89E6B0ull));
+  p = fma(r, p, rbf_exp_c(0x3F2A01A014761F6Eull));
+  p = fma(r, p, rbf_exp_c(0x3F56C16C1852B7B0ull));
+  p = fma(r, p, rbf_exp_c(0x3F81111111122322ull));
+  p = fma(r, p, rbf_exp_c(0x3FA55555555502A1ull));
+  p = fma(r, p, rbf_exp_c(0x3FC5555555555511ull));
+  p = fma(r, p, rbf_exp_c(0x3FE000000000000Bull));
+  p = fma(r, p, 1.0);
+  p = fma(r, p, 1.0);
+  return __builtin_ldexp(p, (int)n);
+}
 __device__ __forceinline__ double rbf_value(const double (&xi)[8], const double *__restrict__ Xs,
                                             int64_t g, int d) {
   double s = 0.0;
@@ -617,6 +642,8 @@
   DevState *st = nullptr;
   long long it = 0;
 };
+void launch_rbf_exp_probe(const double *s, int64_t n, double *lib_out, double *lean_out,
+                          hipStream_t st);
 void launch_symv(const SymPack &sp, const double *v_full, double *P, const int *status,
                  hipStream_t s, PGather pg = PGather{});
 void launch_sym_reduce(const SymPack &sp, int64_t n_out, double *y, bool epilogue, double sigma,
diff --git a/mlff-preconditioner_amd/csrc/kernels_sym.hip b/mlff-preconditioner_amd/csrc/kernels_sym.hip
--- a/mlff-preconditioner_amd/csrc/kernels_sym.hip
+++ b/mlff-preconditioner_amd/csrc/kernels_sym.hip
@@ -15,6 +15,7 @@
 constexpr int kBatches = B / kRB;
 constexpr int kTileRed = 6 * B;
 constexpr int kTileLds = kTileRed + 4 * kRB * 64;
+constexpr int kGenRowLds = kSymGenMaxD * B + B / 64;
 
 __device__ __forceinline__ void decode_unit(long long u, int nwhole, int lsub, int &tile, int &h,
                                             int &gb0, int &gb1) {
@@ -135,15 +136,24 @@
     for (int t = 0; t < kSymGenMaxD; ++t) gc.x[j][t] = (ok && t < gs.d) ? gs.Xs[g * gs.d + t] : 0.0;
   }
 }
+__device__ __forceinline__ bool gen_row_inside(const double *xrow, int r) {
+  const unsigned *mask = reinterpret_cast<const unsigned *>(xrow + kSymGenMaxD * B);
+  return ((mask[r >> 5] >> (r & 31)) & 1u) != 0u;
+}
 __device__ __forceinline__ void gen_stage_rows(const SymGen &gs, int I, int r0, int nr,
                                                double *__restrict__ xrow) {
+  unsigned *mask = reinterpret_cast<unsigned *>(xrow + kSymGenMaxD * B);
   for (int i = threadIdx.x; i < nr; i += 256) {
     int64_t g;
     const bool ok = gen_index(gs, (int64_t)I * B + r0 + i, g);
 #pragma unroll
     for (int t = 0; t < kSymGenMaxD; ++t)
-      xrow[4 * (r0 + i) + t] = (ok && t < gs.d) ? gs.Xs[g * gs.d + t] : 0.0;
-    xrow[4 * (r0 + i) + 3] = ok ? 1.0 : 0.0;
+      xrow[kSymGenMaxD * (r0 + i) + t] = (ok && t < gs.d) ? gs.Xs[g * gs.d + t] : 0.0;
+    const unsigned long long m = __ballot(ok);
+    if ((threadIdx.x & 63) == 0) {
+      mask[(r0 + i) >> 5] = (unsigned)m;
+      if (nr - i > 32) mask[((r0 + i) >> 5) + 1] = (unsigned)(m >> 32);
+    }
   }
 }
 __device__ __forceinline__ bool gen_block_full(const SymGen &gs, int Jb) {
@@ -151,10 +161,12 @@
   const int64_t p0 = (int64_t)Jb * B, p1 = p0 + B - 1;
   return p0 / gs.blk == p1 / gs.blk && gen_index(gs, p0, g) && gen_index(gs, p1, g);
 }
+template <bool PLAIN, bool DIAG>
 __device__ __forceinline__ void gen_row(const SymGen &gs, const GenCols &gc,
-                                        const double *__restrict__ xrow, int r, int lane, bool plain,
-                                        bool diag, d2 (&ar)[4]) {
-  const double *xr = xrow + 4 * r;
+                                        const double *__restrict__ xrow, int r, int lane,
+                                        d2 (&ar)[4]) {
+  static_assert(!(PLAIN && DIAG), "a diagonal tile is not plain");
+  const double *xr = xrow + kSymGenMaxD * r;
   double x[kSymGenMaxD];
 #pragma unroll
   for (int t = 0; t < kSymGenMaxD; ++t) x[t] = xr[t];
@@ -164,14 +176,14 @@
     double s = 0.0;
 #pragma unroll
     for (int t = 0; t < kSymGenMaxD; ++t) s = rbf_sqdist_step(s, __dsub_rn(gc.x[j][t], x[t]), t == 0);
-    v[j] = rbf_of_sqdist(s);
-  }
-  if (!plain) {
-    const bool rv = xr[3] != 0.0;
+    v[j] = rbf_of_sqdist_lean(s);
+  }
+  if constexpr (!PLAIN) {
+    const bool rv = gen_row_inside(xrow, r);
 #pragma unroll
     for (int j = 0; j < 8; ++j) {
       const int c = 2 * (lane + 64 * (j >> 1)) + (j & 1);
-      if (diag && c == r) v[j] = 1.0 + gs.jitter;
+      if (DIAG && c == r) v[j] = 1.0 + gs.jitter;
       if (!(rv && ((gc.valid >> j) & 1u))) v[j] = 0.0;
     }
   }
@@ -180,30 +192,35 @@
 }
 
 
+template <int RB>
 __device__ __forceinline__ void tile_load_batch(const double *A, int64_t rbase, int lane,
-                                                d2 (&a)[kRB][4]) {
+                                                d2 (&a)[RB][4]) {
   const d2 *rowp = reinterpret_cast<const d2 *>(A + rbase * B) + lane;
 #pragma unroll
-  for (int rr = 0; rr < kRB; ++rr)
+  for (int rr = 0; rr < RB; ++rr)
 #pragma unroll
     for (int q = 0; q < 4; ++q) a[rr][q] = __builtin_nontemporal_load(rowp + rr * (B / 2) + 64 * q);
 }
 
-template <bool GEN>
-__device__ __forceinline__ void tile_batch(const d2 (&a)[GEN ? 1 : kRB][4], const SymGen &gs,
+template <bool GEN, bool PLAIN, bool DIAG, int RB>
+__device__ __forceinline__ void tile_batch(d2 (&a)[GEN ? 1 : RB][4], const double *A,
+                                           const SymGen &gs,
                                            const GenCols &gc, const double *xrow,
-                                           bool plain, bool diag, const d2 (&pc)[4],
+                                           bool diag_rt, const d2 (&pc)[4],
                                            const double *vrow, int rbase, int lane,
                                            double *red, double *rows,
                                            d2 (&acc)[4]) {
+  const bool diag = GEN ? DIAG : diag_rt;
 #pragma unroll(GEN ? 2 : kRB)
   for (int rr = 0; rr < kRB; ++rr) {
     d2 ar[4];
     if constexpr (GEN) {
-      gen_row(gs, gc, xrow, rbase + rr, lane, plain, diag, ar);
+      gen_row<PLAIN, DIAG>(gs, gc, xrow, rbase + rr, lane, ar);
     } else {
-#pragma unroll
-      for (int q = 0; q < 4; ++q) ar[q] = a[rr][q];
+      if constexpr (RB < kRB)
+        if (rr == RB) tile_load_batch<RB>(A, rbase + RB, lane, a);
+#pragma unroll
+      for (int q = 0; q < 4; ++q) ar[q] = a[rr % RB][q];
     }
     double s0 = ar[0].x * pc[0].x;
     double s1 = ar[0].y * pc[0].y;
@@ -235,6 +252,34 @@
   __builtin_amdgcn_fence(__ATOMIC_RELEASE, "wavefront");
   __builtin_amdgcn_wave_barrier();
   __builtin_amdgcn_fence(__ATOMIC_ACQUIRE, "wavefront");
+}
+
+template <bool GEN, bool PLAIN, bool DIAG, int RB>
+__device__ __forceinline__ void tile_batches(d2 (&a)[GEN ? 1 : RB][4], const double *A,
+                                             const SymGen &gs, const GenCols &gc, const double *xrow,
+                                             bool diag_rt, const d2 (&pc)[4], const double *vrow,
+                                             int gb0, int gb1, int w, int lane, double *red,
+                                             double *rows, d2 (&acc)[4]) {
+#pragma unroll 1
+  for (int g = gb0 + w; g < gb1; g += 4) {
+    if constexpr (!GEN)
+      if (g != gb0 + w) tile_load_batch<RB>(A, g * kRB, lane, a);
+    tile_batch<GEN, PLAIN, DIAG, RB>(a, A, gs, gc, xrow, diag_rt, pc, vrow, g * kRB, lane, red, rows,
+                                     acc);
+  }
+}
+template <bool GEN, int RB>
+__device__ __forceinline__ void tile_unit(d2 (&a)[GEN ? 1 : RB][4], const double *A,
+                                          const SymGen &gs, const GenCols &gc, const double *xrow,
+                                          bool plain, bool diag, const d2 (&pc)[4],
+                                          const double *vrow, int gb0, int gb1, int w, int lane,
+                                          double *red, double *rows, d2 (&acc)[4]) {
+  if (GEN && plain)
+    tile_batches<GEN, GEN, false, RB>(a, A, gs, gc, xrow, diag, pc, vrow, gb0, gb1, w, lane, red, rows, acc);
+  else if (GEN && diag)
+    tile_batches<GEN, false, GEN, RB>(a, A, gs, gc, xrow, diag, pc, vrow, gb0, gb1, w, lane, red, rows, acc);
+  else
+    tile_batches<GEN, false, false, RB>(a, A, gs, gc, xrow, diag, pc, vrow, gb0, gb1, w, lane, red, rows, acc);
 }
 
 __device__ __forceinline__ void tile_stage_cols(const d2 (&acc)[4], double *cs, int w, int lane) {
@@ -276,7 +321,7 @@
 #pragma unroll
   for (int q = 0; q < 4; ++q)
     pc[q] = *reinterpret_cast<const d2 *>(v + (int64_t)t.y * B + 2 * (lane + 64 * q));
-  tile_load_batch(A, (int64_t)(gb0 + w) * kRB, lane, a);
+  tile_load_batch<kRB>(A, (int64_t)(gb0 + w) * kRB, lane, a);
   for (int i = gb0 * kRB + threadIdx.x; i < gb1 * kRB; i += 256) sh[i] = v[(int64_t)t.x * B + i];
   __syncthreads();
   const bool diag = t.x == t.y;
@@ -284,12 +329,8 @@
   d2 acc[4];
 #pragma unroll
   for (int q = 0; q < 4; ++q) acc[q] = d2{0.0, 0.0};
-#pragma unroll 1
-  for (int g = gb0 + w; g < gb1; g += 4) {
-    if (g != gb0 + w) tile_load_batch(A, g * kRB, lane, a);
-    tile_batch<false>(a, SymGen{}, none, nullptr, false, diag, pc, sh, g * kRB, lane,
-                      sh + kTileRed + w * kRB * 64, sh + B, acc);
-  }
+  tile_unit<false, kRB>(a, A, SymGen{}, none, nullptr, false, diag, pc, sh, gb0, gb1, w, lane,
+                   sh + kTileRed + w * kRB * 64, sh + B, acc);
   if (!diag) tile_stage_cols(acc, sh + 2 * B, w, lane);
   __syncthreads();
   tile_store_slots(P, Pq, Np, nb, t, h, gb0, gb1, diag, sh);
@@ -308,7 +349,7 @@
   double beta;
 };
 
-template <bool GEN>
+template <bool GEN, int RB>
 __device__ __forceinline__ long long symv_units(const SymvArgs &k, const SymGen &gs, long long u,
                                                 UnitQueue q, double *__restrict__ sh,
                                                 long long *s_next) {
@@ -324,11 +365,11 @@
   decode_unit(u, k.nwhole, k.lsub, tile, h, gb0, gb1);
   int2 t = k.list[tile];
   const double *A = k.tiles + (int64_t)tile * B * B;
-  d2 pc[4], a[GEN ? 1 : kRB][4];
+  d2 pc[4], a[GEN ? 1 : RB][4];
   GenCols gc;
 #pragma unroll
   for (int q = 0; q < 4; ++q) pc[q] = pg_val2(pg, v, (int64_t)t.y * B + 2 * (lane + 64 * q), beta);
-  if constexpr (!GEN) tile_load_batch(A, (int64_t)(gb0 + w) * kRB, lane, a);
+  if constexpr (!GEN) tile_load_batch<RB>(A, (int64_t)(gb0 + w) * kRB, lane, a);
   if (threadIdx.x == 0) *s_next = next_unit(q, k.nunits);
   for (int i = threadIdx.x; i < (gb1 - gb0) * kRB; i += 256) {
     const int64_t gi = (int64_t)t.x * B + gb0 * kRB + i;
@@ -345,12 +386,7 @@
     d2 acc[4];
 #pragma unroll
     for (int q = 0; q < 4; ++q) acc[q] = d2{0.0, 0.0};
-#pragma unroll 1
-    for (int g = gb0 + w; g < gb1; g += 4) {
-      if constexpr (!GEN)
-        if (g != gb0 + w) tile_load_batch(A, g * kRB, lane, a);
-      tile_batch<GEN>(a, gs, gc, xrow, plain, diag, pc, vrow, g * kRB, lane, red, rows, acc);
-    }
+    tile_unit<GEN, RB>(a, A, gs, gc, xrow, plain, diag, pc, vrow, gb0, gb1, w, lane, red, rows, acc);
     if (!diag) tile_stage_cols(acc, cs, w, lane);
     __syncthreads();
     const long long un = *s_next;
@@ -367,7 +403,7 @@
       if constexpr (GEN)
         gen_load_cols(gs, t2.y, lane, gc);
       else
-        tile_load_batch(A2, (int64_t)(gb02 + w) * kRB, lane, a);
+        tile_load_batch<RB>(A2, (int64_t)(gb02 + w) * kRB, lane, a);
     }
     tile_store_slots(k.P, k.Pq, k.Np, k.nb, t, h, gb0, gb1, diag, sh);
     __syncthreads();
@@ -399,8 +435,8 @@
 
 constexpr int kTraceWords = 4;
 
-template <bool ROLES>
-__global__ __launch_bounds__(256) void k_symv_dyn(const double *__restrict__ tiles,
+template <bool ROLES, int RB = kRB>
+__global__ __launch_bounds__(256, RB < kRB ? 3 : 1) void k_symv_dyn(const double *__restrict__ tiles,
                                                   const int2 *__restrict__ list,
                                                   const double *__restrict__ v,
                                                   double *__restrict__ P,
@@ -414,14 +450,15 @@
   if (status != nullptr && *status != ST_RUNNING) return;
   unsigned long long *tr = wgtrace != nullptr ? wgtrace + kTraceWords * blockIdx.x : nullptr;
   if (tr != nullptr && threadIdx.x == 0) tr[0] = wall_clock64();
-  __shared__ double sh[kTileLds + (ROLES ? 4 * B : 0)];
+  __shared__ double sh[kTileLds + (ROLES ? kGenRowLds : 0)];
   __shared__ long long s_next;
   __shared__ int s_role;
   if (!ROLES && (long long)blockIdx.x >= nunits) return;
   if (ROLES && threadIdx.x == 0) {
     int r = gs.roles == kSymRolesGen ? 1 : 0;
-    if (gs.roles == kSymRolesIndex) r = (int)(blockIdx.x & 1u);
-    if (gs.roles == kSymRolesCu) r = (int)(atomicAdd(ticket + kTicketWords + cu_key(), 1ull) & 1ull);
+    const unsigned wgs = (unsigned)gs.wgs;
+    if (gs.roles == kSymRolesIndex) r = blockIdx.x % wgs != 0u;
+    if (gs.roles == kSymRolesCu) r = atomicAdd(ticket + kTicketWords + cu_key(), 1ull) % wgs != 0ull;
     s_role = r;
   }
   if (!ROLES && tr != nullptr && threadIdx.x == 0) tr[3] = 1ull | (unsigned long long)cu_key() << 2;
@@ -462,11 +499,11 @@
   long long units_done;
   if constexpr (ROLES) {
     if (gen)
-      units_done = symv_units<true>(k, gs, u, q, sh, &s_next);
+      units_done = symv_units<true, RB>(k, gs, u, q, sh, &s_next);
     else
-      units_done = symv_units<false>(k, gs, u, q, sh, &s_next);
+      units_done = symv_units<false, RB>(k, gs, u, q, sh, &s_next);
   } else {
-    units_done = symv_units<false>(k, gs, u, q, sh, &s_next);
+    units_done = symv_units<false, RB>(k, gs, u, q, sh, &s_next);
   }
   if (tr != nullptr && threadIdx.x == 0) {
     tr[1] = wall_clock64();
@@ -893,6 +930,22 @@
   }
 }
 
+__global__ __launch_bounds__(256) void k_rbf_exp_probe(const double *__restrict__ s, int64_t n,
+                                                       double *__restrict__ lib_out,
+                                                       double *__restrict__ lean_out) {
+  for (int64_t i = (int64_t)blockIdx.x * 256 + threadIdx.x; i < n; i += (int64_t)gridDim.x * 256) {
+    lib_out[i] = rbf_of_sqdist(s[i]);
+    lean_out[i] = rbf_of_sqdist_lean(s[i]);
+  }
+}
+
+}
+
+void launch_rbf_exp_probe(const double *s, int64_t n, double *lib_out, double *lean_out,
+                          hipStream_t st) {
+  if (n <= 0) return;
+  const unsigned grid = (unsigned)std::min<int64_t>((n + 255) / 256, 4096);
+  hipLaunchKernelGGL(k_rbf_exp_probe, dim3(grid), dim3(256), 0, st, s, n, lib_out, lean_out);
 }
 
 struct SymKnobs {
@@ -904,6 +957,7 @@
   int gen_quarters = 0;
   int roles = kSymRolesCu;
   int pool_first = 0;
+  int wgs = 0;
   bool reduce_list = true;
   bool pq_ordered = false;
   long long trace_at = 0;
@@ -929,13 +983,18 @@
     if (std::strcmp(e, "gen") == 0) k.roles = kSymRolesGen;
   }
   if (const char *e = std::getenv("MLFF_SYM_STEAL")) k.pool_first = std::strcmp(e, "pool") == 0;
+  if (const char *e = std::getenv("MLFF_SYM_WGS")) {
+    const int v = std::atoi(e);
+    if (v == 2 || v == 3) k.wgs = v;
+  }
   if (const char *e = std::getenv("MLFF_SYM_REDUCE_LIST")) k.reduce_list = std::atoi(e) != 0;
   if (const char *e = std::getenv("MLFF_SYM_PQ_ORDERED")) k.pq_ordered = std::atoi(e) != 0;
   if (const char *e = std::getenv("MLFF_SYM_TRACE")) k.trace_at = std::atoll(e);
   return k;
 }
 
-static void print_symv_trace(const unsigned long long *tr, unsigned G, int64_t units, hipStream_t s) {
+static void print_symv_trace(const unsigned long long *tr, unsigned G, int64_t units, int wgs,
+                             hipStream_t s) {
   std::vector<unsigned long long> h((size_t)kTraceWords * G);
   if (hipStreamSynchronize(s) != hipSuccess ||
       hipMemcpy(h.data(), tr, sizeof(unsigned long long) * h.size(), hipMemcpyDeviceToHost) != hipSuccess)
@@ -983,11 +1042,11 @@
   for (int k = 0; k < kSymCuWords; ++k) {
     if (cu_s[k] + cu_g[k] == 0) continue;
     ++cus;
-    if (cu_s[k] == 1 && cu_g[k] == 1)
+    if (cu_s[k] == 1 && cu_g[k] == wgs - 1)
       ++paired;
-    else if (cu_s[k] == 2 && cu_g[k] == 0)
+    else if (cu_s[k] == wgs && cu_g[k] == 0)
       ++two_s;
-    else if (cu_s[k] == 0 && cu_g[k] == 2)
+    else if (cu_s[k] == 0 && cu_g[k] == wgs)
       ++two_g;
     else
       ++other;
@@ -997,9 +1056,11 @@
     if (xs[x] + xg[x] > 0)
       per_xcc += " " + std::to_string(x) + ":" + std::to_string(xs[x]) + "s+" + std::to_string(xg[x]) + "g";
   std::fprintf(stderr,
-               "[sym trace] roles: %d distinct CU keys; CUs holding {stream + gen} %d, {2 stream} %d, "
-               "{2 gen} %d, other %d; units taken stream / gen %.0f / %.0f; per XCC id%s\n",
-               cus, paired, two_s, two_g, other, un_s, un_g, per_xcc.c_str());
+               "[sym trace] roles: %d distinct CU keys; CUs holding {1 stream + %d gen} %d, {%d stream} "
+               "%d, {%d gen} %d, other %d; units taken stream / gen %.0f / %.0f (%.0f / %.0f per ms "
+               "of the span); per XCC id%s\n",
+               cus, wgs - 1, paired, wgs, two_s, wgs, two_g, other, un_s, un_g, 1e6 * un_s / span,
+               1e6 * un_g / span, per_xcc.c_str());
 }
 
 void launch_symv(const SymPack &sp, const double *v_full, double *P, const int *status,
@@ -1018,7 +1079,11 @@
   if (trace_at > 0 && ++launches == trace_at &&
       hipMalloc(&tr, sizeof(unsigned long long) * kTraceWords * G) == hipSuccess)
     (void)hipMemsetAsync(tr, 0, sizeof(unsigned long long) * kTraceWords * G, s);
-  if (sp.gen)
+  if (sp.gen && sp.rb4)
+    hipLaunchKernelGGL((k_symv_dyn<true, 4>), dim3(G), dim3(256), 0, s,
+                       sp.tiles, sp.list, v_full, P, sp.Pq, sp.Np, (int)sp.nwhole, (long long)grid,
+                       (int)sp.nb, sp.lsub, sp.ticket, status, pg, sp.gsrc, tr);
+  else if (sp.gen)
     hipLaunchKernelGGL(k_symv_dyn<true>, dim3(G), dim3(256), 0, s,
                        sp.tiles, sp.list, v_full, P, sp.Pq, sp.Np, (int)sp.nwhole, (long long)grid,
                        (int)sp.nb, sp.lsub, sp.ticket, status, pg, sp.gsrc, tr);
@@ -1027,7 +1092,7 @@
                        sp.tiles, sp.list, v_full, P, sp.Pq, sp.Np, (int)sp.nwhole, (long long)grid,
                        (int)sp.nb, sp.lsub, sp.ticket, status, pg, SymGen{}, tr);
   if (tr != nullptr) {
-    print_symv_trace(tr, G, grid, s);
+    print_symv_trace(tr, G, grid, sp.wgs, s);
     (void)hipFree(tr);
   }
 }
@@ -1118,6 +1183,8 @@
   int lsub = 2;
   int64_t nq = 3;
   int64_t dyn = 0;
+  int wgs = 2;
+  bool rb4 = false;
   bool gen = false;
   SymGen gsrc;
 };
@@ -1154,8 +1221,20 @@
     if (n_s == pl.nwhole && qmode == 1) on = false;
     if (on) {
       pl.gen = true;
+      if (kn.wgs != 2) {
+        int occ = 0;
+        if (hipOccupancyMaxActiveBlocksPerMultiprocessor(&occ, k_symv_dyn<true, 4>, 256, 0) != hipSuccess ||
+            occ < 1)
+          occ = 2;
+        const int64_t nunits = pl.nwhole + ((pl.nt - pl.nwhole) << pl.lsub);
+        pl.rb4 = kn.wgs == 3 || (occ > 2 && nunits >= kSymThreeWgMinUnits * occ * cus);
+        if (pl.rb4) {
+          pl.wgs = occ;
+          pl.dyn = (int64_t)occ * cus;
+        }
+      }
       pl.gsrc = SymGen{ctx->rbf.Xs, ctx->rbf.d, ctx->rbf.jitter, ctx->N, ctx->rows_per, ctx->blk,
-                       (int)n_s, qmode, kn.roles, kn.pool_first};
+                       (int)n_s, qmode, kn.roles, kn.pool_first, pl.wgs};
     }
   }
   return pl;
@@ -1197,6 +1276,8 @@
   sp.nwhole = pl.nwhole;
   sp.lsub = pl.lsub;
   sp.dyn = pl.dyn;
+  sp.wgs = pl.dyn > 0 ? pl.wgs : 0;
+  sp.rb4 = pl.rb4;
   sp.gen = pl.gen;
   sp.gsrc = pl.gsrc;
   sp.pq_ordered = kn.pq_ordered;
diff --git a/mlff-preconditioner_amd/sgdml_amd/_native.py b/mlff-preconditioner_amd/sgdml_amd/_native.py
--- a/mlff-preconditioner_amd/sgdml_amd/_native.py
+++ b/mlff-preconditioner_amd/sgdml_amd/_native.py
@@ -59,6 +59,7 @@
     "mlff_test_gram": (_int, [_c_ctx, _p_dbl, _i64, _i64, _int, _p_dbl]),
     "mlff_sgdml_energies": (_int, [_c_ctx, _p_dbl, _p_dbl, _p_i64, _p_i64]),
     "mlff_sgdml_descriptors": (_int, [_p_dbl, _i64, _int, _p_dbl, _p_dbl]),
+    "mlff_test_rbf_exp": (_int, [_c_ctx, _p_dbl, _i64, _p_dbl, _p_dbl]),
     "mlff_predict_set_model": (_int, [_c_ctx, _p_dbl, _p_dbl, _i64, _int, _p_i32, _int, _dbl, _dbl,
                                       _dbl]),
     "mlff_predict": (_int, [_c_ctx, _p_dbl, _i64, _p_dbl, _p_dbl]),
@@ -68,6 +69,7 @@
     "mlff_get_diag": (_int, [_c_ctx, _p_dbl]),
     "mlff_set_storage": (_int, [_c_ctx, _int]),
     "mlff_storage_info": (_int, [_c_ctx, _p_int, _p_dbl]),
+    "mlff_sym_launch_info": (_int, [_c_ctx, _p_int, _p_i64]),
     "mlff_operator_form": (_int, [_c_ctx, _p_int]),
     "mlff_precon_none": (_int, [_c_ctx]),
     "mlff_precon_pivchol": (_int, [_c_ctx, _i64, _int, _p_i64, _p_dbl]),
diff --git a/mlff-preconditioner_amd/sgdml_amd/solver.py b/mlff-preconditioner_amd/sgdml_amd/solver.py
--- a/mlff-preconditioner_amd/sgdml_amd/solver.py
+++ b/mlff-preconditioner_amd/sgdml_amd/solver.py
@@ -189,6 +189,12 @@
                                                                                 "dense")
         return name, nbytes.value
 
+    def sym_launch_info(self) -> tuple[int, int]:
+        wgs = ctypes.c_int()
+        grid = ctypes.c_int64()
+        self._call("mlff_sym_launch_info", ctypes.byref(wgs), ctypes.byref(grid))
+        return wgs.value, grid.value
+
     def operator_form(self) -> str | None:
         f = ctypes.c_int()
         self._call("mlff_operator_form", ctypes.byref(f))
```

New measurement: 624.8, median of 6. 12.1% higher.
